# jkulhanek/viewformer

Measured on AMD Instinct MI355X. Metric: novel views/sec (encode->AR transformer->decode), 128px 6-ctx, higher is better.
Workload: dtype bf16

## Files before the change

### include/vf_hip.h

```cpp
#ifndef VF_HIP_H
#define VF_HIP_H

#include <stddef.h>
#include <stdint.h>

#ifdef __cplusplus
extern "C" {
#endif

#define VF_OK 0
#define VF_ERR_BAD_ARG (-1)
#define VF_ERR_UNSUPPORTED (-2)

int vf_abi_version(void);
size_t vf_sizeof_igemm_args(void);
size_t vf_sizeof_pack_desc(void);
const char* vf_build_arch(void);
int vf_build_flags(void);
const char* vf_build_flag_name(int i);
enum { VF_SEL_ATTN_DMA = 0,
       VF_SEL_GEMM_G256 = 1,
       VF_SEL_LN_BWD_TWO_ROWS = 2,
       VF_SEL_ATTN_Q32 = 3,
       VF_SEL_CONV_X3H_K32 = 4,
       VF_SEL_GEMM_TAIL = 5,
       VF_SEL_COUNT = 6 };
int vf_select(int which, int value);
int vf_selected(int which);

enum { VF_MODE_GEMM = 0, VF_MODE_CONV3_S1 = 1, VF_MODE_CONV3_S2PAD = 2, VF_MODE_CONV3_UP2 = 3 };
enum { VF_EPI_NONE = 0, VF_EPI_GELU_ERF = 1,
       VF_EPI_GELU_BWD = 2,
       VF_EPI_GELU_DUAL = 3 };

typedef struct vf_igemm_args {
    const float* x;
    const float* w_packed;
    const float* bias;
    const float* res;
    float* out;
    const float* pro_mean;
    const float* pro_scale;
    const float* pro_beta;
    int32_t pro_swish;
    int32_t pro_rows_per_img;
    int32_t mode;
    int32_t epilogue;
    int32_t M;
    int32_t Cin, Cout;
    int32_t Hin, Win, Hout, Wout;
    int32_t lda, ldc, ldr;
    int32_t batch;
    int64_t stride_x, stride_w, stride_out, stride_res;
    float* gn_part;
    int32_t gn_slots;
    int32_t reserved0;
    void* out_aux;
    float drop_rate;
    uint32_t drop_seed, drop_site;
    int32_t drop_row0;
} vf_igemm_args;

size_t vf_igemm_packed_floats(int K, int N, int taps);
int vf_igemm_pack_f32(const float* src, float* dst, int K, int N, int taps,
                      int64_t sk, int64_t sn, int64_t st, int batch, int64_t src_bstride, void* stream);
int vf_igemm_f32(const vf_igemm_args* args , void* stream);

int vf_conv_in_u8_f32(const uint8_t* img_u8, const float* img_f32, const float* w_oihw, const float* bias,
                      float* out, int n_img, int H, int W, int Cout, void* stream);
size_t vf_conv_in_x3h_packed_elems(int Cout);
int vf_conv_in_x3h_pack(const float* w_oihw, void* dst, int Cout, void* stream);
int vf_conv_in_x3h(const uint8_t* img_u8, const float* img_f32, const void* w_packed, const float* bias, float* out, float* gn_part,
                   int gn_slots, int n_img, int H, int W, int Cout, void* stream);

int vf_conv3_small_cout_f32(const float* x, const float* w_oihw, const float* bias, const float* pro_mean,
                            const float* pro_scale, const float* pro_beta, int pro_swish, float* out, int n_img, int H, int W,
                            int Cin, int Cout, int x_bf16, void* stream);

size_t vf_groupnorm_workspace_bytes(int n_img, int HW, int C);
int vf_groupnorm_stats_f32(const float* x, const float* gamma, int n_img, int HW, int C, int groups, float eps,
                           float* mean_c, float* scale_c, void* ws, void* stream);
int vf_groupnorm_finalize_f32(const float* part, const float* gamma, int n_img, int HW, int C, int groups, int nslots,
                              float eps, float* mean_c, float* scale_c, void* stream);
int vf_groupnorm_apply_f32(const float* x, const float* mean_c, const float* scale_c, const float* beta,
                           float* out, int n_img, int HW, int C, int swish, void* stream);

size_t vf_vq_packed_floats(int D, int Kc);
int vf_vq_pack_codebook_f32(const float* E , float* dst, int D, int Kc, void* stream);
int vf_colsumsq_f32(const float* E , float* e_sq , int D, int Kc, void* stream);
int vf_vq_argmin_f32(const float* z, const float* E_packed, const float* e_sq, int64_t M, int D, int Kc,
                     int64_t* idx, void* stream);
size_t vf_vq_filter_packed_bytes(int D, int Kc);
int vf_vq_filter_pack(const float* E , void* dst, int D, int Kc, void* stream);
int vf_vq_argmin_filtered_f32(const float* z, const void* packed, int64_t M, int D, int Kc, int64_t* idx, uint32_t* stats4,
                              void* stream);
int vf_codebook_gather_f32(const float* E , const int64_t* idx, float* out ,
                           int64_t M, int D, int Kc, void* stream);

int vf_attn_blockcausal_f32(const float* q, const float* k, const float* v, float* out,
                            int B, int H, int T, int L, int ldq, int ldk, int ldv, int ldo,
                            float scale, int skip_masked, int twin_view, void* stream);
int vf_attn_blockcausal_bf16_v2(const void* q, const void* k, const void* v, int in_bf16, void* out, int out_bf16, int B, int H, int T, int L,
                                int ldq, int ldk, int ldv, int ldo, float scale, int skip_masked, int twin_view, void* stream);
int vf_attn_blockcausal_fp8(const void* q, const void* k, const void* v, int in_bf16, void* out, int out_bf16, int B, int H, int T, int L,
                            int ldq, int ldk, int ldv, int ldo, float scale, int skip_masked, int twin_view, void* stream);
int vf_attn_blockcausal_x6(const float* q, const float* k, const float* v, float* out,
                           int B, int H, int T, int L, int ldq, int ldk, int ldv, int ldo,
                           float scale, int skip_masked, int twin_view, void* stream);
int vf_attn_prefix_bf16(const void* q, const void* k, const void* v, const void* kp, const void* vp, int in_bf16, void* out, int out_bf16,
                        int B, int H, int C, int N, int L, int dh, int ldq, int ldk, int ldv, int ldkp, int ldvp, int64_t prefix_stride,
                        int ldo, void* stream);
int vf_attn_prefix_f32eq(const float* q, const float* k, const float* v, const float* kp, const float* vp, float* out,
                         int B, int H, int C, int N, int L, int dh, int ldq, int ldk, int ldv, int ldkp, int ldvp, int64_t prefix_stride,
                         int ldo, void* stream);
int vf_attn_prefix_var_bf16(const void* q, const void* k, const void* v, const void* kp, const void* vp, int in_bf16, void* out, int out_bf16,
                            int B, int H, int C, int N, int L, int dh, int ldq, int ldk, int ldv, int ldkp, int ldvp, int64_t prefix_stride,
                            int ldo, const int32_t* ctx_len, void* stream);
int vf_attn_prefix_var_f32eq(const float* q, const float* k, const float* v, const float* kp, const float* vp, float* out,
                             int B, int H, int C, int N, int L, int dh, int ldq, int ldk, int ldv, int ldkp, int ldvp, int64_t prefix_stride,
                             int ldo, const int32_t* ctx_len, void* stream);
int vf_attn_prefix_fork_bf16(const void* q, const void* k, const void* v, const void* kp, const void* vp, int in_bf16, void* out, int out_bf16,
                             int B, int H, int C, int N, int L, int dh, int ldq, int ldk, int ldv, int ldkp, int ldvp, int64_t prefix_stride,
                             int ldo, const int32_t* ctx_len, const void* kp2, const void* vp2, int C2, int ldkp2, int ldvp2,
                             int64_t prefix_stride2, const int32_t* split, int share, void* stream);
int vf_attn_prefix_fork_f32eq(const float* q, const float* k, const float* v, const float* kp, const float* vp, float* out,
                              int B, int H, int C, int N, int L, int dh, int ldq, int ldk, int ldv, int ldkp, int ldvp, int64_t prefix_stride,
                              int ldo, const int32_t* ctx_len, const float* kp2, const float* vp2, int C2, int ldkp2, int ldvp2,
                              int64_t prefix_stride2, const int32_t* split, int share, void* stream);
int vf_attn_prefix_bwd_f32(const void* q, const void* k, const void* v, const void* kp, const void* vp, int in_bf16, const float* dout,
                           float* dqkv, int B, int H, int C, int N, int L, int dh, int ldq, int ldk, int ldv, int ldkp, int ldvp,
                           int64_t prefix_stride, int lddo, int lddqkv, const int32_t* ctx_len, void* stream);
int vf_kv_append(const void* qkv, void* cache, int elem_bytes, int B, int K, int L, int d, int ld_src, int ld_dst, int64_t cache_stride,
                 int capacity, const int32_t* pos, void* stream);
int vf_kv_append_split(const void* qkv, void* k, void* v, int elem_bytes, int B, int K, int L, int d, int ld_src, int ld_k, int ld_v,
                       int64_t k_stride, int64_t v_stride, int capacity, const int32_t* pos, void* stream);
int vf_kv_pack_e4m3(const void* cache, int elem_bytes, void* kq, void* vq, float* kscale, float* vscale, int B, int C, int H, int L,
                    int ld_src, int64_t cache_stride, int64_t q_view_stride, int64_t q_scene_stride, int64_t s_view_stride,
                    int64_t s_scene_stride, const int32_t* lengths, void* stream);
int vf_kv_append_e4m3(const void* qkv, int elem_bytes, void* kq, void* vq, float* kscale, float* vscale, int B, int K, int H, int L,
                      int ld_src, int64_t q_view_stride, int64_t q_scene_stride, int64_t s_view_stride, int64_t s_scene_stride,
                      int capacity, const int32_t* pos, void* stream);
int vf_attn_prefix_q8_bf16(const void* q, const void* k, const void* v, const void* kq, const void* vq, const float* kscale, const float* vscale,
                           int in_bf16, void* out, int out_bf16, int B, int H, int C, int N, int L, int dh, int ldq, int ldk, int ldv,
                           int64_t q_view_stride, int64_t q_scene_stride, int64_t s_view_stride, int64_t s_scene_stride, int ldo,
                           const int32_t* ctx_len, void* stream);
int vf_attn_spatial_f32(const float* qkv, float* out, int n_img, int HW, int C, int64_t ld, int64_t ldo, float scale, void* stream);
int vf_attn_spatial_x3h(const float* qkv, float* out, int n_img, int HW, int C, int64_t ld, int64_t ldo, float scale, void* stream);
int vf_softmax_rows_f32(float* x, int64_t rows, int n, float scale, void* stream);

int vf_layernorm_f32(const float* x, const float* gamma, const float* beta, float* out,
                     int64_t rows, int d, float eps, void* stream);
int vf_layernorm_bf16out_f32(const float* x, const float* gamma, const float* beta, void* out_bf16, int64_t rows, int d, float eps,
                             void* stream);
int vf_embed_sum_f32(const int32_t* ids, const float* wte, const float* wpe, const float* add,
                     float* out, int64_t BS, int L, int d, int vocab, void* stream);
int vf_dense_small_k_gelu_f32(const float* x, const float* W, const float* b, float* out,
                              int64_t rows, int K, int N, int gelu, void* stream);
int vf_argmax_rows_f32(const float* x, int64_t rows, int n, int ld, int64_t* idx, void* stream);
int vf_lmhead_argmax_bf16(const void* h, int h_bf16, int64_t ldh, const void* w_packed, int64_t M, int K, int N, int64_t* idx,
                          float* max_logit, void* stream);
int vf_lmhead_score_bf16(const void* h, int h_bf16, int64_t ldh, const void* w_packed, int64_t M, int K, int N, const int32_t* target,
                         int64_t* idx, float* max_logit, float* lse, float* target_logit, float* entropy, void* stream);
int vf_logits_score_f32(const float* logits, int64_t rows, int N, int64_t ld, const int32_t* target, int64_t* idx, float* max_logit,
                        float* lse, float* target_logit, float* entropy, void* stream);
int vf_score_views_f32(const float* target_logit, const float* lse, const float* max_logit, const int64_t* idx, const int32_t* target,
                       int64_t views, int L, float* token_log_prob, float* confidence, float* log_likelihood, float* accuracy, void* stream);
int vf_sample_rows_f32(const float* logits, int64_t rows, int N, int64_t ld, float temperature, int top_k, float top_p, uint32_t seed,
                       const int64_t* row_id, int S, int64_t* idx, float* logp, int32_t* kept, float* thr, void* stream);
int vf_sample_views_f32(const float* logp, int64_t views, int L, int S, float* log_likelihood, void* stream);
uint32_t vf_crc32c(const void* data, size_t n, uint32_t crc);
int vf_postprocess_u8(const float* x, uint8_t* out, int64_t n, void* stream);
int vf_resize_u8(const uint8_t* src, uint8_t* dst, int n_img, int Hin, int Win, int Hout, int Wout, int C, int bilinear, void* stream);
size_t vf_image_metrics_workspace_bytes(int n_img, int H, int W, int C);
int vf_image_metrics_u8(const uint8_t* a, const uint8_t* b, int n_img, int H, int W, int C, int64_t* sums, double* ssim, void* workspace,
                        void* stream);
size_t vf_camera_knn_workspace_bytes(int64_t N, int Q, int k);
int vf_camera_knn_f32(const float* db, int64_t N, const float* queries, int Q, int k, float pos_weight, int32_t* idx, float* dist,
                      void* workspace, void* stream);
int vf_codebook_dist_table_f32(const float* E, int D, int K, int64_t ldE, float* table, void* stream);
size_t vf_code_knn_workspace_bytes(int64_t N, int Q, int k);
int vf_code_knn_f32(const int32_t* db, int64_t N, int64_t ld_db, const int32_t* queries, int Q, int64_t ld_q, int t, const float* table,
                    int K, int window, const int32_t* exclude, int k, int32_t* idx, float* dist, void* workspace, void* stream);
int vf_pose_tail_f32(const float* x, int64_t ldx, const float* W, const float* b, float position_multiplier, int64_t views, int L, int K,
                     float* raw, float* tokens, float* cameras, void* stream);

size_t vf_gemm_bf16_packed_elems(int K, int N);
int vf_gemm_bf16_pack(const float* src, void* dst, int K, int N, int64_t sk, int64_t sn, int batch,
                      int64_t src_bstride, void* stream);
typedef struct vf_pack_desc {
    const float* src;
    void* dst;
    int32_t K, N;
    int64_t sk, sn;
} vf_pack_desc;
int vf_gemm_bf16_pack_multi(const vf_pack_desc* descs_device, int n, void* stream);
int vf_gemm_bf16(const vf_igemm_args* args , void* stream);
size_t vf_conv3_bf16_packed_elems(int Cin, int Cout);
int vf_conv3_bf16_pack(const float* w_oihw, void* dst, int Cin, int Cout, void* stream);
int vf_conv3_halo_bf16(const vf_igemm_args* args , void* stream);

int vf_conv3_halo_gn_slots(int Hout, int Wout);
size_t vf_conv3_x6_packed_elems(int Cin, int Cout);
int vf_conv3_x6_pack(const float* w_oihw, void* dst, int Cin, int Cout, void* stream);
int vf_conv3_halo_x6(const vf_igemm_args* args , void* stream);
size_t vf_conv3_x3h_packed_elems(int Cin, int Cout);
int vf_conv3_x3h_pack(const float* w_oihw, void* dst, int Cin, int Cout, void* stream);
int vf_conv3_halo_x3h(const vf_igemm_args* args , void* stream);
size_t vf_gemm_x3h_packed_elems(int K, int N);
int vf_gemm_x3h_pack(const float* src, void* dst, int K, int N, int64_t sk, int64_t sn, void* stream);
int vf_gemm_x3h(const vf_igemm_args* args , void* stream);
size_t vf_gemm_x6_packed_elems(int K, int N);
int vf_gemm_x6_pack(const float* src, void* dst, int K, int N, int64_t sk, int64_t sn, void* stream);
int vf_gemm_x6(const vf_igemm_args* args , void* stream);
int vf_sum_slabs_f32(const float* slabs, int nslabs, int64_t stride, int64_t n, float* dst, int accumulate, void* stream);

int vf_vq_ema_accumulate_f32(const float* z, const int64_t* idx, int64_t M, int D, int Kc, float* counts, float* embed_sum,
                             void* stream);
int vf_vq_ema_update_f32(const float* counts, const float* embed_sum, float* cluster_size_hidden, float* dw_hidden,
                         float* embeddings, int D, int Kc, float decay, float eps, float corr, void* stream);

int vf_gather_transpose_f32(const float* src, float* dst, int n_img, int Hin, int Win, int C, int Hout, int Wout, int stride, int oy,
                            int ox, int64_t ld_dst, void* stream);
size_t vf_conv3_wgrad_x6_rows(int Cin);
int vf_conv3_wgrad_x6(const float* x, const void* dy_packed, float* slabs, int n_img, int Hin, int Win, int Cin, int Hout, int Wout,
                      int Cout, int mode, int splits, void* stream);
int vf_upsample2_bwd_f32(const float* du, float* dx, int n_img, int H, int W, int C, void* stream);
size_t vf_groupnorm_bwd_workspace_bytes(int n_img, int HW, int C, int groups);
int vf_groupnorm_bwd_f32(const float* x, const float* da, const float* mean_c, const float* scale_c, const float* gamma,
                         const float* beta, float* dx, float* chan_sums, int n_img, int HW, int C, int groups, float eps, int swish,
                         int accumulate, void* ws, void* stream);
int vf_softmax_rows_bwd_f32(const float* p, float* dp, int64_t rows, int n, float scale, void* stream);
int vf_l1_loss_partials(int64_t n);
int vf_l1_loss_f32(const float* x, const float* y, float* dy, float* part, int64_t n, float grad_weight, void* stream);

int vf_lpips_scaling_f32(const float* x, float* y, int64_t npix, const float* shift3, const float* scale3, int backward, void* stream);
int vf_relu_f32(float* x, int64_t n, void* stream);
int vf_relu_bwd_f32(float* dy, const float* y, int64_t n, void* stream);
int vf_maxpool2_f32(const float* x, float* y, int n_img, int Hout, int Wout, int C, void* stream);
int vf_maxpool2_bwd_f32(const float* x, const float* dy, float* dx, int n_img, int Hout, int Wout, int C, void* stream);
int vf_lpips_head_blocks(int HW);
int vf_lpips_head_f32(const float* f0, const float* f1, const float* w, float* part, int n_img, int HW, int C, void* stream);
int vf_lpips_head_bwd_f32(const float* f0, const float* f1, const float* w, float* df1, int64_t npix, int C, float gscale,
                          int accumulate, void* stream);

int vf_attn_blockcausal_lse_f32(const float* q, const float* k, const float* v, float* out, float* lse,
                                int B, int H, int T, int L, int ldq, int ldk, int ldv, int ldo,
                                float scale, int skip_masked, int twin_view, float drop_rate, uint32_t drop_seed,
                                uint32_t drop_site, uint32_t drop_plane0, void* stream);
int vf_attn_bwd_prep_f32(const float* dout, const float* out, float* D, int B, int H, int T, int lddo, int ldo, void* stream);
int vf_attn_bwd_f32(const float* q, const float* k, const float* v, const float* dout, const float* lse, const float* D,
                    float* dq, float* dk, float* dv, int B, int H, int T, int L, int ldq, int ldk, int ldv, int lddo,
                    int lddq, int lddk, int lddv, float scale, int twin_view, float drop_rate, uint32_t drop_seed,
                    uint32_t drop_site, uint32_t drop_plane0, void* stream);
int vf_gemm_tn_bf16(const void* x_bf16, int ldx, const void* dy, int dy_is_bf16, int ldy, int M, int K, int N, int splits, float* w_slabs,
                    float* b_slabs, int64_t slab_stride, void* stream);
int vf_attn_blockcausal_bf16_lse(const void* q, const void* k, const void* v, void* out, float* lse, int B, int H, int T, int L,
                                 int ldq, int ldk, int ldv, int ldo, float scale, int twin_view, float drop_rate, uint32_t drop_seed,
                                 uint32_t drop_site, uint32_t drop_plane0, void* stream);
int vf_attn_bwd_prep_bf16(const void* dout, const void* out, float* D, int B, int H, int T, int lddo, int ldo, void* stream);
int vf_attn_bwd_bf16(const void* q, const void* k, const void* v, const void* dout, const float* lse, const float* D, void* dq, void* dk,
                     void* dv, int out_bf16 , int B, int H, int T, int L,
                     int ldq, int ldk, int ldv, int lddo, int lddq, int lddk, int lddv, float scale, int twin_view, float drop_rate,
                     uint32_t drop_seed, uint32_t drop_site, uint32_t drop_plane0, void* stream);
int vf_dropout_add_f32(const float* x, const float* res, float* out, int64_t rows, int cols, int64_t row0, float rate, uint32_t seed, uint32_t site,
                       void* stream);

int vf_transpose_f32(const float* src, float* dst, int rows, int cols, int64_t ld_src, int64_t ld_dst, int batch,
                     int64_t bs_src, int64_t bs_dst, void* stream);
int vf_transpose_bf16_f32(const void* src_bf16, float* dst, int rows, int cols, int64_t ld_src, int64_t ld_dst, int batch,
                          int64_t bs_src, int64_t bs_dst, void* stream);
size_t vf_colsum_workspace_bytes(int N);
int vf_colsum_f32(const float* x, float* out, int64_t M, int N, int64_t ld, int accumulate, void* ws, void* stream);
size_t vf_layernorm_bwd_workspace_bytes(int64_t rows, int d);
int vf_layernorm_bwd_f32(const float* dy, const float* x, const float* gamma, float* dx, float* dgamma, float* dbeta,
                         int64_t rows, int d, float eps, int accumulate, const float* res ,
                         void* dx_bf16 ,
                         float drop_rate, uint32_t drop_seed, uint32_t drop_site, int64_t drop_row0 , void* ws, void* stream);
int vf_gelu_f32(const float* u, float* f, int64_t n, void* stream);
int vf_gelu_bf16out_f32(const float* u, void* f_bf16, int64_t n, void* stream);
int vf_gelu_bwd_f32(const float* u, const float* df, float* du, int64_t n, void* stream);
int vf_gelu_bwd_bf16out_f32(const float* u, const float* df, void* du_bf16, int64_t n, void* stream);
int vf_softmax_mask_f32(float* s, int64_t batch, int T, int L, int mask_spec, float scale, void* stream);
int vf_softmax_mask_bwd_f32(const float* p, float* dp, int64_t batch, int T, int L, int mask_spec, float scale, void* stream);
int vf_softmax_ce_f32(const float* logits, const int32_t* target, const float* row_weight, float* loss, float* dlogits,
                      int64_t rows, int V, float label_smoothing, void* stream);
int vf_pose_mse_f32(const float* raw, const float* gt, const float* w_pos, const float* w_ori, const float* xyz_div, float* pos_loss,
                    float* ori_loss, float* draw, int64_t rows, int L, float position_multiplier, void* stream);
size_t vf_embed_bwd_workspace_bytes(int d, int vocab);
int vf_embed_bwd_f32(const float* dh, const int32_t* ids, float* dwte, float* dwpe, float* dadd, int64_t BS, int L, int d,
                     int vocab, void* workspace, void* stream);
int vf_dense_small_k_bwd_f32(const float* x, const float* dy, float* dW, float* db, int64_t rows, int K, int N, void* stream);
int vf_dense_small_n_f32(const float* x, const float* W, const float* b, float* out, int64_t rows, int K, int N, int64_t ldx, void* stream);
int vf_dense_small_n_wgrad_slabs(int64_t rows);
int vf_dense_small_n_wgrad_f32(const float* x, const float* dy, float* dW, float* ws, int64_t rows, int K, int N, int64_t ldx, int accumulate,
                               void* stream);
int vf_adamw_f32(float* param, const float* grad, float* m, float* v, int64_t n, float lr_decay, float lr_adam, float beta1,
                 float beta2, float eps, void* stream);
int vf_adamw_flat_f32(float* param, const float* grad, float* m, float* v, int64_t n, const int64_t* nodecay_ranges, int nranges,
                      float lr_decay, float lr_adam, float beta1, float beta2, float eps, void* stream);
typedef struct vf_adamw_pack_desc {
    int64_t offset;
    void* dst_kn;
    void* dst_nk;
    int32_t rows, cols;
    int32_t nodecay;
    int32_t reserved;
} vf_adamw_pack_desc;
size_t vf_sizeof_adamw_pack_desc(void);
int vf_adamw_pack_check(const vf_adamw_pack_desc* descs_host, int ndesc, int64_t n);
int vf_adamw_flat_pack_f32(float* param, const float* grad, float* m, float* v, int64_t n, const int64_t* nodecay_ranges, int nranges,
                           float lr_decay, float lr_adam, float beta1, float beta2, float eps, const vf_adamw_pack_desc* descs_device, int ndesc,
                           void* stream);
int vf_add_inplace_f32(float* a, const float* b, int64_t n, void* stream);
int vf_axpby_f32(float a, const float* x, float b, const float* y, float* out, int64_t n, void* stream);
int vf_clip_scratch_floats(void);
int vf_clip_by_norm_f32(float* x, int64_t n, float clip, float* scratch, void* stream);
int vf_clip_grad_norm_f32(float* x, int64_t n, float max_norm, float* scratch, void* stream);

#ifdef __cplusplus
}
#endif
#endif
```

### viewformer_amd/_lib.py

```python
import ctypes
import os
from ctypes import c_int, c_int32, c_int64, c_float, c_void_p, c_size_t, c_char_p, POINTER

HERE = os.path.dirname(os.path.abspath(__file__))
LIB_PATH = os.environ.get('VF_HIP_LIB') or os.path.join(HERE, 'libvf_hip.so')


class VfIgemmArgs(ctypes.Structure):
    _fields_ = [
        ('x', c_void_p), ('w_packed', c_void_p), ('bias', c_void_p), ('res', c_void_p), ('out', c_void_p),
        ('pro_mean', c_void_p), ('pro_scale', c_void_p), ('pro_beta', c_void_p),
        ('pro_swish', c_int32), ('pro_rows_per_img', c_int32), ('mode', c_int32), ('epilogue', c_int32),
        ('M', c_int32), ('Cin', c_int32), ('Cout', c_int32),
        ('Hin', c_int32), ('Win', c_int32), ('Hout', c_int32), ('Wout', c_int32),
        ('lda', c_int32), ('ldc', c_int32), ('ldr', c_int32), ('batch', c_int32),
        ('stride_x', c_int64), ('stride_w', c_int64), ('stride_out', c_int64), ('stride_res', c_int64),
        ('gn_part', c_void_p), ('gn_slots', c_int32), ('reserved0', c_int32),
        ('out_aux', c_void_p),
        ('drop_rate', c_float), ('drop_seed', ctypes.c_uint32), ('drop_site', ctypes.c_uint32), ('drop_row0', c_int32),
    ]


SEL_ATTN_DMA, SEL_GEMM_G256, SEL_LN_BWD_TWO_ROWS, SEL_ATTN_Q32 = 0, 1, 2, 3
SEL_CONV_X3H_K32 = 4
SEL_GEMM_TAIL = 5
_ENV_SELECT = {'VF_ATTN_DMA': SEL_ATTN_DMA, 'VF_GEMM_G256': SEL_GEMM_G256, 'VF_LN_BWD_TWO_ROWS': SEL_LN_BWD_TWO_ROWS, 'VF_ATTN_Q32': SEL_ATTN_Q32,
               'VF_CONV_X3H_K32': SEL_CONV_X3H_K32, 'VF_GEMM_TAIL': SEL_GEMM_TAIL}

ADAMW_PACK_DESC_BYTES = 40
PACK_DESC_BYTES = 40
P = c_void_p
EXPORTS = {
    'vf_abi_version': (c_int, []),
    'vf_sizeof_igemm_args': (c_size_t, []),
    'vf_sizeof_pack_desc': (c_size_t, []),
    'vf_build_arch': (c_char_p, []),
    'vf_build_flags': (c_int, []),
    'vf_build_flag_name': (c_char_p, [c_int]),
    'vf_select': (c_int, [c_int, c_int]),
    'vf_selected': (c_int, [c_int]),
    'vf_igemm_packed_floats': (c_size_t, [c_int, c_int, c_int]),
    'vf_igemm_pack_f32': (c_int, [P, P, c_int, c_int, c_int, c_int64, c_int64, c_int64, c_int, c_int64, P]),
    'vf_igemm_f32': (c_int, [POINTER(VfIgemmArgs), P]),
    'vf_conv_in_u8_f32': (c_int, [P, P, P, P, P, c_int, c_int, c_int, c_int, P]),
    'vf_conv_in_x3h_packed_elems': (c_size_t, [c_int]),
    'vf_conv_in_x3h_pack': (c_int, [P, P, c_int, P]),
    'vf_conv_in_x3h': (c_int, [P, P, P, P, P, P, c_int, c_int, c_int, c_int, c_int, P]),
    'vf_crc32c': (ctypes.c_uint32, [P, c_size_t, ctypes.c_uint32]),
    'vf_conv3_small_cout_f32': (c_int, [P, P, P, P, P, P, c_int, P, c_int, c_int, c_int, c_int, c_int, c_int, P]),
    'vf_groupnorm_workspace_bytes': (c_size_t, [c_int, c_int, c_int]),
    'vf_groupnorm_stats_f32': (c_int, [P, P, c_int, c_int, c_int, c_int, c_float, P, P, P, P]),
    'vf_groupnorm_finalize_f32': (c_int, [P, P, c_int, c_int, c_int, c_int, c_int, c_float, P, P, P]),
    'vf_conv3_halo_gn_slots': (c_int, [c_int, c_int]),
    'vf_groupnorm_apply_f32': (c_int, [P, P, P, P, P, c_int, c_int, c_int, c_int, P]),
    'vf_vq_packed_floats': (c_size_t, [c_int, c_int]),
    'vf_vq_pack_codebook_f32': (c_int, [P, P, c_int, c_int, P]),
    'vf_colsumsq_f32': (c_int, [P, P, c_int, c_int, P]),
    'vf_vq_argmin_f32': (c_int, [P, P, P, c_int64, c_int, c_int, P, P]),
    'vf_vq_filter_packed_bytes': (c_size_t, [c_int, c_int]),
    'vf_vq_filter_pack': (c_int, [P, P, c_int, c_int, P]),
    'vf_vq_argmin_filtered_f32': (c_int, [P, P, c_int64, c_int, c_int, P, P, P]),
    'vf_gather_transpose_f32': (c_int, [P, P, c_int, c_int, c_int, c_int, c_int, c_int, c_int, c_int, c_int, c_int64, P]),
    'vf_upsample2_bwd_f32': (c_int, [P, P, c_int, c_int, c_int, c_int, P]),
    'vf_groupnorm_bwd_workspace_bytes': (c_size_t, [c_int, c_int, c_int, c_int]),
    'vf_groupnorm_bwd_f32': (c_int, [P, P, P, P, P, P, P, P, c_int, c_int, c_int, c_int, c_float, c_int, c_int, P, P]),
    'vf_softmax_rows_bwd_f32': (c_int, [P, P, c_int64, c_int, c_float, P]),
    'vf_l1_loss_partials': (c_int, [c_int64]),
    'vf_l1_loss_f32': (c_int, [P, P, P, P, c_int64, c_float, P]),
    'vf_conv3_wgrad_x6_rows': (c_size_t, [c_int]),
    'vf_conv3_wgrad_x6': (c_int, [P, P, P, c_int, c_int, c_int, c_int, c_int, c_int, c_int, c_int, c_int, P]),
    'vf_lpips_scaling_f32': (c_int, [P, P, c_int64, P, P, c_int, P]),
    'vf_relu_f32': (c_int, [P, c_int64, P]),
    'vf_relu_bwd_f32': (c_int, [P, P, c_int64, P]),
    'vf_maxpool2_f32': (c_int, [P, P, c_int, c_int, c_int, c_int, P]),
    'vf_maxpool2_bwd_f32': (c_int, [P, P, P, c_int, c_int, c_int, c_int, P]),
    'vf_lpips_head_blocks': (c_int, [c_int]),
    'vf_lpips_head_f32': (c_int, [P, P, P, P, c_int, c_int, c_int, P]),
    'vf_lpips_head_bwd_f32': (c_int, [P, P, P, P, c_int64, c_int, c_float, c_int, P]),
    'vf_vq_ema_accumulate_f32': (c_int, [P, P, c_int64, c_int, c_int, P, P, P]),
    'vf_vq_ema_update_f32': (c_int, [P, P, P, P, P, c_int, c_int, c_float, c_float, c_float, P]),
    'vf_codebook_gather_f32': (c_int, [P, P, P, c_int64, c_int, c_int, P]),
    'vf_attn_blockcausal_f32': (c_int, [P, P, P, P, c_int, c_int, c_int, c_int, c_int, c_int, c_int, c_int,
                                        c_float, c_int, c_int, P]),
    'vf_attn_blockcausal_bf16_v2': (c_int, [P, P, P, c_int, P, c_int] + [c_int] * 8 + [c_float, c_int, c_int, P]),
    'vf_attn_blockcausal_fp8': (c_int, [P, P, P, c_int, P, c_int] + [c_int] * 8 + [c_float, c_int, c_int, P]),
    'vf_attn_blockcausal_x6': (c_int, [P, P, P, P, c_int, c_int, c_int, c_int, c_int, c_int, c_int, c_int,
                                       c_float, c_int, c_int, P]),
    'vf_attn_prefix_bf16': (c_int, [P, P, P, P, P, c_int, P, c_int] + [c_int] * 11 + [c_int64, c_int, P]),
    'vf_attn_prefix_f32eq': (c_int, [P, P, P, P, P, P] + [c_int] * 11 + [c_int64, c_int, P]),
    'vf_attn_prefix_var_bf16': (c_int, [P, P, P, P, P, c_int, P, c_int] + [c_int] * 11 + [c_int64, c_int, P, P]),
    'vf_attn_prefix_var_f32eq': (c_int, [P, P, P, P, P, P] + [c_int] * 11 + [c_int64, c_int, P, P]),
    'vf_attn_prefix_fork_bf16': (c_int, [P, P, P, P, P, c_int, P, c_int] + [c_int] * 11 + [c_int64, c_int, P,
                                         P, P, c_int, c_int, c_int, c_int64, P, c_int, P]),
    'vf_attn_prefix_fork_f32eq': (c_int, [P, P, P, P, P, P] + [c_int] * 11 + [c_int64, c_int, P, P, P, c_int, c_int, c_int, c_int64, P, c_int, P]),
    'vf_attn_prefix_bwd_f32': (c_int, [P, P, P, P, P, c_int, P, P] + [c_int] * 11 + [c_int64, c_int, c_int, P, P]),
    'vf_kv_append': (c_int, [P, P, c_int, c_int, c_int, c_int, c_int, c_int, c_int, c_int64, c_int, P, P]),
    'vf_kv_append_split': (c_int, [P, P, P] + [c_int] * 8 + [c_int64, c_int64, c_int, P, P]),
    'vf_kv_pack_e4m3': (c_int, [P, c_int, P, P, P, P] + [c_int] * 5 + [c_int64] * 5 + [P, P]),
    'vf_kv_append_e4m3': (c_int, [P, c_int, P, P, P, P] + [c_int] * 5 + [c_int64] * 4 + [c_int, P, P]),
    'vf_attn_prefix_q8_bf16': (c_int, [P] * 7 + [c_int, P, c_int] + [c_int] * 9 + [c_int64] * 4 + [c_int, P, P]),
    'vf_attn_blockcausal_lse_f32': (c_int, [P, P, P, P, P, c_int, c_int, c_int, c_int, c_int, c_int, c_int, c_int,
                                            c_float, c_int, c_int, c_float, ctypes.c_uint32, ctypes.c_uint32, ctypes.c_uint32, P]),
    'vf_dropout_add_f32': (c_int, [P, P, P, c_int64, c_int, c_int64, c_float, ctypes.c_uint32, ctypes.c_uint32, P]),
    'vf_attn_bwd_prep_f32': (c_int, [P, P, P, c_int, c_int, c_int, c_int, c_int, P]),
    'vf_attn_bwd_f32': (c_int, [P, P, P, P, P, P, P, P, P, c_int, c_int, c_int, c_int, c_int, c_int, c_int, c_int, c_int,
                                c_int, c_int, c_float, c_int, c_float, ctypes.c_uint32, ctypes.c_uint32, ctypes.c_uint32, P]),
    'vf_gemm_tn_bf16': (c_int, [P, c_int, P, c_int, c_int, c_int, c_int, c_int, c_int, P, P, c_int64, P]),
    'vf_attn_blockcausal_bf16_lse': (c_int, [P, P, P, P, P, c_int, c_int, c_int, c_int, c_int, c_int, c_int, c_int, c_float, c_int,
                                             c_float, ctypes.c_uint32, ctypes.c_uint32, ctypes.c_uint32, P]),
    'vf_attn_bwd_prep_bf16': (c_int, [P, P, P, c_int, c_int, c_int, c_int, c_int, P]),
    'vf_attn_bwd_bf16': (c_int, [P, P, P, P, P, P, P, P, P, c_int, c_int, c_int, c_int, c_int, c_int, c_int, c_int, c_int, c_int, c_int, c_int,
                                 c_float, c_int, c_float, ctypes.c_uint32, ctypes.c_uint32, ctypes.c_uint32, P]),
    'vf_attn_spatial_f32': (c_int, [P, P, c_int, c_int, c_int, c_int64, c_int64, c_float, P]),
    'vf_attn_spatial_x3h': (c_int, [P, P, c_int, c_int, c_int, c_int64, c_int64, c_float, P]),
    'vf_softmax_rows_f32': (c_int, [P, c_int64, c_int, c_float, P]),
    'vf_layernorm_f32': (c_int, [P, P, P, P, c_int64, c_int, c_float, P]),
    'vf_layernorm_bf16out_f32': (c_int, [P, P, P, P, c_int64, c_int, c_float, P]),
    'vf_embed_sum_f32': (c_int, [P, P, P, P, P, c_int64, c_int, c_int, c_int, P]),
    'vf_dense_small_k_gelu_f32': (c_int, [P, P, P, P, c_int64, c_int, c_int, c_int, P]),
    'vf_lmhead_argmax_bf16': (c_int, [P, c_int, c_int64, P, c_int64, c_int, c_int, P, P, P]),
    'vf_lmhead_score_bf16': (c_int, [P, c_int, c_int64, P, c_int64, c_int, c_int, P, P, P, P, P, P, P]),
    'vf_logits_score_f32': (c_int, [P, c_int64, c_int, c_int64, P, P, P, P, P, P, P]),
    'vf_score_views_f32': (c_int, [P, P, P, P, P, c_int64, c_int, P, P, P, P, P]),
    'vf_sample_rows_f32': (c_int, [P, c_int64, c_int, c_int64, c_float, c_int, c_float, ctypes.c_uint32, P, c_int, P, P, P, P, P]),
    'vf_sample_views_f32': (c_int, [P, c_int64, c_int, c_int, P, P]),
    'vf_argmax_rows_f32': (c_int, [P, c_int64, c_int, c_int, P, P]),
    'vf_postprocess_u8': (c_int, [P, P, c_int64, P]),
    'vf_resize_u8': (c_int, [P, P, c_int, c_int, c_int, c_int, c_int, c_int, c_int, P]),
    'vf_image_metrics_workspace_bytes': (c_size_t, [c_int, c_int, c_int, c_int]),
    'vf_image_metrics_u8': (c_int, [P, P, c_int, c_int, c_int, c_int, P, P, P, P]),
    'vf_camera_knn_workspace_bytes': (c_size_t, [c_int64, c_int, c_int]),
    'vf_camera_knn_f32': (c_int, [P, c_int64, P, c_int, c_int, c_float, P, P, P, P]),
    'vf_codebook_dist_table_f32': (c_int, [P, c_int, c_int, c_int64, P, P]),
    'vf_code_knn_workspace_bytes': (c_size_t, [c_int64, c_int, c_int]),
    'vf_code_knn_f32': (c_int, [P, c_int64, c_int64, P, c_int, c_int64, c_int, P, c_int, c_int, P, c_int, P, P, P, P]),
    'vf_pose_tail_f32': (c_int, [P, c_int64, P, P, c_float, c_int64, c_int, c_int, P, P, P, P]),
    'vf_gemm_bf16_packed_elems': (c_size_t, [c_int, c_int]),
    'vf_gemm_bf16_pack': (c_int, [P, P, c_int, c_int, c_int64, c_int64, c_int, c_int64, P]),
    'vf_gemm_bf16_pack_multi': (c_int, [P, c_int, P]),
    'vf_gemm_bf16': (c_int, [POINTER(VfIgemmArgs), P]),
    'vf_conv3_bf16_packed_elems': (c_size_t, [c_int, c_int]),
    'vf_conv3_bf16_pack': (c_int, [P, P, c_int, c_int, P]),
    'vf_conv3_halo_bf16': (c_int, [POINTER(VfIgemmArgs), P]),
    'vf_conv3_x6_packed_elems': (c_size_t, [c_int, c_int]),
    'vf_conv3_x6_pack': (c_int, [P, P, c_int, c_int, P]),
    'vf_conv3_halo_x6': (c_int, [POINTER(VfIgemmArgs), P]),
    'vf_conv3_x3h_packed_elems': (c_size_t, [c_int, c_int]),
    'vf_conv3_x3h_pack': (c_int, [P, P, c_int, c_int, P]),
    'vf_conv3_halo_x3h': (c_int, [POINTER(VfIgemmArgs), P]),
    'vf_gemm_x3h_packed_elems': (c_size_t, [c_int, c_int]),
    'vf_gemm_x3h_pack': (c_int, [P, P, c_int, c_int, c_int64, c_int64, P]),
    'vf_gemm_x3h': (c_int, [POINTER(VfIgemmArgs), P]),
    'vf_gemm_x6_packed_elems': (c_size_t, [c_int, c_int]),
    'vf_gemm_x6_pack': (c_int, [P, P, c_int, c_int, c_int64, c_int64, P]),
    'vf_gemm_x6': (c_int, [POINTER(VfIgemmArgs), P]),
    'vf_sum_slabs_f32': (c_int, [P, c_int, c_int64, c_int64, P, c_int, P]),
    'vf_transpose_f32': (c_int, [P, P, c_int, c_int, c_int64, c_int64, c_int, c_int64, c_int64, P]),
    'vf_transpose_bf16_f32': (c_int, [P, P, c_int, c_int, c_int64, c_int64, c_int, c_int64, c_int64, P]),
    'vf_colsum_workspace_bytes': (c_size_t, [c_int]),
    'vf_colsum_f32': (c_int, [P, P, c_int64, c_int, c_int64, c_int, P, P]),
    'vf_layernorm_bwd_workspace_bytes': (c_size_t, [c_int64, c_int]),
    'vf_layernorm_bwd_f32': (c_int, [P, P, P, P, P, P, c_int64, c_int, c_float, c_int, P, P, c_float, ctypes.c_uint32, ctypes.c_uint32, c_int64, P, P]),
    'vf_gelu_f32': (c_int, [P, P, c_int64, P]),
    'vf_gelu_bf16out_f32': (c_int, [P, P, c_int64, P]),
    'vf_gelu_bwd_bf16out_f32': (c_int, [P, P, P, c_int64, P]),
    'vf_gelu_bwd_f32': (c_int, [P, P, P, c_int64, P]),
    'vf_softmax_mask_f32': (c_int, [P, c_int64, c_int, c_int, c_int, c_float, P]),
    'vf_softmax_mask_bwd_f32': (c_int, [P, P, c_int64, c_int, c_int, c_int, c_float, P]),
    'vf_softmax_ce_f32': (c_int, [P, P, P, P, P, c_int64, c_int, c_float, P]),
    'vf_pose_mse_f32': (c_int, [P, P, P, P, P, P, P, P, c_int64, c_int, c_float, P]),
    'vf_embed_bwd_workspace_bytes': (c_size_t, [c_int, c_int]),
    'vf_embed_bwd_f32': (c_int, [P, P, P, P, P, c_int64, c_int, c_int, c_int, P, P]),
    'vf_dense_small_k_bwd_f32': (c_int, [P, P, P, P, c_int64, c_int, c_int, P]),
    'vf_dense_small_n_f32': (c_int, [P, P, P, P, c_int64, c_int, c_int, c_int64, P]),
    'vf_dense_small_n_wgrad_slabs': (c_int, [c_int64]),
    'vf_dense_small_n_wgrad_f32': (c_int, [P, P, P, P, c_int64, c_int, c_int, c_int64, c_int, P]),
    'vf_adamw_f32': (c_int, [P, P, P, P, c_int64, c_float, c_float, c_float, c_float, c_float, P]),
    'vf_adamw_flat_f32': (c_int, [P, P, P, P, c_int64, P, c_int, c_float, c_float, c_float, c_float, c_float, P]),
    'vf_sizeof_adamw_pack_desc': (c_size_t, []),
    'vf_adamw_pack_check': (c_int, [P, c_int, c_int64]),
    'vf_adamw_flat_pack_f32': (c_int, [P, P, P, P, c_int64, P, c_int, c_float, c_float, c_float, c_float, c_float, P, c_int, P]),
    'vf_axpby_f32': (c_int, [c_float, P, c_float, P, P, c_int64, P]),
    'vf_add_inplace_f32': (c_int, [P, P, c_int64, P]),
    'vf_clip_scratch_floats': (c_int, []),
    'vf_clip_by_norm_f32': (c_int, [P, c_int64, c_float, P, P]),
    'vf_clip_grad_norm_f32': (c_int, [P, c_int64, c_float, P, P]),
}

_lib = None


class VfError(RuntimeError):
    pass


def _bind(path):
    lib = ctypes.CDLL(path)
    for name, (res, args) in EXPORTS.items():
        fn = getattr(lib, name)
        fn.restype = res
        fn.argtypes = args
    return lib


def load_variant(path):
    return _bind(os.path.abspath(path))


class use:

    def __init__(self, handle):
        self.handle = handle

    def __enter__(self):
        global _lib
        load()
        self.prev, _lib = _lib, self.handle
        return self.handle

    def __exit__(self, *exc):
        global _lib
        _lib = self.prev
        return False


def load():
    global _lib
    if _lib is not None:
        return _lib
    if not os.path.exists(LIB_PATH):
        raise VfError(f'{LIB_PATH} not found — run `python -m viewformer_amd.build` (hipcc --offload-arch=gfx950). '
                      'There is no CPU/PyTorch fallback for the hot path.')
    lib = _bind(LIB_PATH)
    if int(lib.vf_sizeof_igemm_args()) != ctypes.sizeof(VfIgemmArgs):
        raise VfError(f'vf_igemm_args is {int(lib.vf_sizeof_igemm_args())} bytes in {LIB_PATH} and {ctypes.sizeof(VfIgemmArgs)} in '
                      'viewformer_amd/_lib.py: rebuild the library or update the mirror')
    if int(lib.vf_sizeof_pack_desc()) != PACK_DESC_BYTES:
        raise VfError(f'vf_pack_desc is {int(lib.vf_sizeof_pack_desc())} bytes in {LIB_PATH}, {PACK_DESC_BYTES} expected')
    if int(lib.vf_sizeof_adamw_pack_desc()) != ADAMW_PACK_DESC_BYTES:
        raise VfError(f'vf_adamw_pack_desc is {int(lib.vf_sizeof_adamw_pack_desc())} bytes in {LIB_PATH}, {ADAMW_PACK_DESC_BYTES} expected')
    for env, which in _ENV_SELECT.items():
        if os.environ.get(env) in ('0', '1'):
            lib.vf_select(which, int(os.environ[env]))
    _lib = lib
    return lib


def select(which, value):
    prev = load().vf_select(int(which), 1 if value else 0)
    if prev < 0:
        raise VfError(f'vf_select({which}, {value}): bad argument')
    return prev


def check(status: int, what: str):
    if status == 0:
        return
    if status < 0:
        msg = {-1: 'bad argument', -2: 'unsupported shape'}.get(status, 'error')
        raise VfError(f'{what}: {msg} ({status})')
    raise VfError(f'{what}: HIP error {status}')
```

### viewformer_amd/csrc/conv3_halo_x3h.hip

```cpp
#include <type_traits>
#include "halo_common.h"

namespace {

typedef _Float16 f16x8 __attribute__((ext_vector_type(8)));
typedef _Float16 f16x4 __attribute__((ext_vector_type(4)));

typedef unsigned u32x4_t __attribute__((ext_vector_type(4)));
__device__ __forceinline__ f16x8 wbuf_load(__amdgpu_buffer_rsrc_t r, unsigned voff, unsigned soff) {
    return __builtin_bit_cast(f16x8, __builtin_amdgcn_raw_buffer_load_b128(r, voff, soff, 0));
}

constexpr int CK = 32;
constexpr int P_LDB = 144;
constexpr int TH = 8, TW = 16;
constexpr int BN = 128;
constexpr int PLANE_BYTES = 2 * BN * 16;
constexpr int KS_BYTES = 2 * PLANE_BYTES;
constexpr int TAP_BYTES = 2 * KS_BYTES;
constexpr int TAIL_BYTES = 16;

template <bool UP2, bool PAIR = false>
struct Geo {
    static constexpr int PH = UP2 ? (TH / 2 + 2) : (TH + 2);
    static constexpr int PW = PAIR ? 20 : (UP2 ? (TW / 2 + 2) : (TW + 2));
    static constexpr int NPIX = PH * PW;
    static constexpr int SLOTS = (NPIX * 8 + 255) / 256;
    static constexpr int BUF = (NPIX + 1) * P_LDB;
};

__device__ __forceinline__ void split2(float x, _Float16& h, _Float16& l) {
    h = (_Float16)x;
    l = (_Float16)((x - (float)h) * 2048.f);
}

template <bool UP2, bool PRO, bool SWISH, bool PAIR = false>
__global__ __launch_bounds__(256, 2) void conv3_halo_x3h_kernel(vf_igemm_args p) {
    using G = Geo<UP2, PAIR>;
    extern __shared__ __attribute__((aligned(16))) unsigned char smem_h[];

    const int tid = threadIdx.x;
    const int lane = tid & 63;
    const int wave = __builtin_amdgcn_readfirstlane(tid >> 6);
    constexpr int MI = 4, NJ = 1;
    const int wave_m = 0, wave_n = wave;
    const int half = lane >> 5, l31 = lane & 31;

    const int nb = p.Cout / BN;
    const int tilesX = p.Wout / TW, tilesY = p.Hout / TH;
    int bid = (int)vf_xcd_bid();
    const int nblk = bid % nb; bid /= nb;
    int tx = 0, ty = 0, img;
    if (PAIR) { img = bid * 2; }
    else { tx = bid % tilesX; bid /= tilesX; ty = bid % tilesY; img = bid / tilesY; }
    const int n_img_total = p.M / (p.Hout * p.Wout);
    const int img1 = PAIR ? min(img + 1, n_img_total - 1) : img;
    const int pair_pix = (img1 - img) * p.Hin * p.Win;
    const int y0 = ty * TH, x0 = tx * TW;
    const int sy0 = UP2 ? (y0 / 2 - 1) : (y0 - 1);
    const int sx0 = UP2 ? (x0 / 2 - 1) : (x0 - 1);

    const float* __restrict__ X = p.x + (size_t)img * p.Hin * p.Win * p.Cin;
    const int nchunks = p.Cin / CK;
    const int last_stage = nchunks * 9 - 1;

    const int c4 = tid & 7;
    int s_off[G::SLOTS];
    unsigned ok_mask = 0, sel_mask = 0;
    const int lds0 = (tid >> 3) * P_LDB + c4 * 8;
    int lds_last = 0;
#pragma unroll
    for (int q = 0; q < G::SLOTS; ++q) {
        const int pix = (tid >> 3) + 32 * q;
        const int pixc = pix < G::NPIX ? pix : G::NPIX;
        const int pr = pixc / G::PW, pc0 = pixc - pr * G::PW;
        const int sel = PAIR ? (pc0 >= 10) : 0;
        const int pc = pc0 - 10 * sel;
        sel_mask |= (unsigned)sel << q;
        const int sy = sy0 + pr, sx = sx0 + pc;
        const bool ok = pix < G::NPIX && sy >= 0 && sy < p.Hin && sx >= 0 && sx < p.Win;
        ok_mask |= (unsigned)ok << q;
        s_off[q] = ok ? (sel * pair_pix + sy * p.Win + sx) * p.Cin + c4 * 4 : c4 * 4;
        if (q == G::SLOTS - 1) lds_last = pixc * P_LDB + c4 * 8;
    }

    f32x4 preg[G::SLOTS];
    f32x4 pmean, pscale, pbeta, pmean1, pscale1;
    const __amdgpu_buffer_rsrc_t x_rs = __builtin_amdgcn_make_buffer_rsrc(const_cast<float*>(X), 0, 0x7fffffff, 0x00020000);
    auto patch_load = [&](int chunk) {
#pragma unroll
        for (int q = 0; q < G::SLOTS; ++q)
            preg[q] = __builtin_bit_cast(f32x4, __builtin_amdgcn_raw_buffer_load_b128(x_rs, (unsigned)s_off[q] * 4u, (unsigned)(chunk * CK * 4), 0));
        if (PRO) {
            pmean = *reinterpret_cast<const f32x4*>(p.pro_mean + (size_t)img * p.Cin + chunk * CK + c4 * 4);
            pscale = *reinterpret_cast<const f32x4*>(p.pro_scale + (size_t)img * p.Cin + chunk * CK + c4 * 4);
            pbeta = *reinterpret_cast<const f32x4*>(p.pro_beta + chunk * CK + c4 * 4);
            if (PAIR) {
                pmean1 = *reinterpret_cast<const f32x4*>(p.pro_mean + (size_t)img1 * p.Cin + chunk * CK + c4 * 4);
                pscale1 = *reinterpret_cast<const f32x4*>(p.pro_scale + (size_t)img1 * p.Cin + chunk * CK + c4 * 4);
            }
        }
    };
    auto patch_store_slot = [&](int buf, int q) {
        unsigned char* dst = smem_h + buf * G::BUF + (q == G::SLOTS - 1 ? lds_last : lds0 + q * 32 * P_LDB);
        f16x4 oh, ol;
#pragma unroll
        for (int e = 0; e < 4; ++e) {
            float t = preg[q][e];
            if (PRO) {
                const float mu = (PAIR && ((sel_mask >> q) & 1u)) ? pmean1[e] : pmean[e];
                const float sc = (PAIR && ((sel_mask >> q) & 1u)) ? pscale1[e] : pscale[e];
                t = (t - mu) * sc + pbeta[e];
                if (SWISH) t = vf_swish_1ulp(t);
            }
            _Float16 h, l;
            split2(((ok_mask >> q) & 1u) ? t : 0.f, h, l);
            oh[e] = h; ol[e] = l;
        }
        *reinterpret_cast<f16x4*>(dst) = oh;
        *reinterpret_cast<f16x4*>(dst + 64) = ol;
    };

    const int trow = vf_perm_row(l31), tpx = vf_perm_px(l31);
    int a_base[MI], a_r[MI];
#pragma unroll
    for (int mi = 0; mi < MI; ++mi) {
        const int a0 = wave_m * 4 + mi * 2 + trow;
        a_r[mi] = a0;
        const int tcol = PAIR ? (tpx >> 3) * 10 + (tpx & 7) : tpx;
        a_base[mi] = (a0 * G::PW + tcol) * P_LDB + half * 16;
    }

    const unsigned char* __restrict__ Wb = reinterpret_cast<const unsigned char*>(p.w_packed) + (size_t)nblk * TAP_BYTES;
    const size_t tap_stride = (size_t)nb * TAP_BYTES;
    const int b_lane = (half * BN + wave_n * (32 * NJ) + l31) * 16;
    constexpr int BD = 2, RING = BD + 1;
    static_assert(18 % RING == 0, "ring indices must repeat per chunk");
    f16x8 bring[RING][2][NJ];
    f16x8 aring[2][MI][2];
    const int last_g = nchunks * 18 - 1;
    const __amdgpu_buffer_rsrc_t w_rs = __builtin_amdgcn_make_buffer_rsrc(const_cast<unsigned char*>(Wb), 0, 0x7fffffff, 0x00020000);
    auto b_load = [&](f16x8 (&dst)[2][NJ], int g) {
        g = min(g, last_g);
        const unsigned soff = (unsigned)((size_t)(g >> 1) * tap_stride + (g & 1) * KS_BYTES);
#pragma unroll
        for (int pl = 0; pl < 2; ++pl)
#pragma unroll
            for (int j = 0; j < NJ; ++j) dst[pl][j] = wbuf_load(w_rs, (unsigned)(b_lane + pl * PLANE_BYTES + j * 32 * 16), soff);
    };
    auto a_load = [&](f16x8 (&dst)[MI][2], const unsigned char* patch, int s) {
        const int tap = s >> 1, ks = s & 1;
        const int dy = tap / 3, dx = tap % 3;
#pragma unroll
        for (int mi = 0; mi < MI; ++mi) {
            int aoff;
            if (UP2) {
                const int pr = (a_r[mi] + dy + 1) >> 1, pc = (tpx + dx + 1) >> 1;
                aoff = (pr * G::PW + pc) * P_LDB + half * 16;
            } else {
                aoff = a_base[mi] + (dy * G::PW + dx) * P_LDB;
            }
#pragma unroll
            for (int pl = 0; pl < 2; ++pl) dst[mi][pl] = *reinterpret_cast<const f16x8*>(patch + aoff + pl * 64 + ks * 32);
        }
    };

    f32x16 acc[MI][NJ], accx[MI][NJ];
#pragma unroll
    for (int i = 0; i < MI; ++i)
#pragma unroll
        for (int j = 0; j < NJ; ++j)
#pragma unroll
            for (int r = 0; r < 16; ++r) { acc[i][j][r] = 0.f; accx[i][j][r] = 0.f; }

    patch_load(0);
#pragma unroll
    for (int g = 0; g < BD; ++g) b_load(bring[g], g);
#pragma unroll
    for (int q = 0; q < G::SLOTS; ++q) patch_store_slot(0, q);
    __syncthreads();

    for (int chunk = 0; chunk < nchunks; ++chunk) {
        const unsigned char* patch = smem_h + (chunk & 1) * G::BUF;
        b_load(bring[BD % RING], chunk * 18 + BD);
        const bool more = UP2 || PAIR || chunk + 1 < nchunks;
        if (more) patch_load(min(chunk + 1, nchunks - 1));
        a_load(aring[0], patch, 0);
#pragma unroll
        for (int s = 0; s < 18; ++s) {
            if (s > 0) b_load(bring[(s + BD) % RING], chunk * 18 + s + BD);
            if (s + 1 < 18) a_load(aring[(s + 1) & 1], patch, s + 1);
#pragma unroll
            for (int t = 0; t < 3; ++t) {
#pragma unroll
                for (int mi = 0; mi < MI; ++mi)
#pragma unroll
                    for (int j = 0; j < NJ; ++j) {
                        if (t == 0) accx[mi][j] = __builtin_amdgcn_mfma_f32_32x32x16_f16(aring[s & 1][mi][1], bring[s % RING][0][j], accx[mi][j], 0, 0, 0);
                        else if (t == 1) accx[mi][j] = __builtin_amdgcn_mfma_f32_32x32x16_f16(aring[s & 1][mi][0], bring[s % RING][1][j], accx[mi][j], 0, 0, 0);
                        else acc[mi][j] = __builtin_amdgcn_mfma_f32_32x32x16_f16(aring[s & 1][mi][0], bring[s % RING][0][j], acc[mi][j], 0, 0, 0);
                    }
            }
            __builtin_amdgcn_sched_barrier(0);
            if ((s & 1) && (s >> 1) < G::SLOTS && more) patch_store_slot((chunk + 1) & 1, s >> 1);
        }
        __syncthreads();
    }

    const float inv_s = *reinterpret_cast<const float*>(reinterpret_cast<const unsigned char*>(p.w_packed) + (size_t)nchunks * 9 * nb * TAP_BYTES);
#pragma unroll
    for (int i = 0; i < MI; ++i)
#pragma unroll
        for (int j = 0; j < NJ; ++j)
#pragma unroll
            for (int r = 0; r < 16; ++r) acc[i][j][r] = __builtin_fmaf(accx[i][j][r], 4.8828125e-4f, acc[i][j][r]) * inv_s;
    vf_halo_epilogue_t<PAIR, MI, NJ>(p, acc, img, img1, y0, x0, PAIR ? 0 : (ty * tilesX + tx) * 2, nblk, wave_m, wave_n, half, l31);
}


constexpr int S2_PH = 2 * TH + 1, S2_PW = 2 * TW + 1;
constexpr int S2_NPIX = S2_PH * S2_PW;
constexpr int S2_LDB = 80;
constexpr int S2_SLOTS = (S2_NPIX * 4 + 255) / 256;
constexpr int S2_BUF = (S2_NPIX + 1) * S2_LDB;

template <bool P8>
__global__ __launch_bounds__(256, 2) void conv3_s2_x3h_kernel(vf_igemm_args p) {
    extern __shared__ __attribute__((aligned(16))) unsigned char smem_h[];
    constexpr int PW = P8 ? 34 : S2_PW;
    constexpr int NPIX = S2_PH * PW;
    constexpr int SLOTS = (NPIX * 4 + 255) / 256;
    const int tid = threadIdx.x;
    const int lane = tid & 63;
    const int wave = __builtin_amdgcn_readfirstlane(tid >> 6);
    constexpr int MI = 4, NJ = 1;
    const int wave_m = 0, wave_n = wave;
    const int half = lane >> 5, l31 = lane & 31;

    const int nb = p.Cout / BN;
    const int tilesX = P8 ? 1 : p.Wout / TW, tilesY = P8 ? 1 : p.Hout / TH;
    int bid = (int)vf_xcd_bid();
    const int nblk = bid % nb; bid /= nb;
    const int tx = bid % tilesX; bid /= tilesX;
    const int ty = bid % tilesY;
    const int img = P8 ? (bid / tilesY) * 2 : bid / tilesY;
    const int n_img_total = p.M / (p.Hout * p.Wout);
    const int img1 = P8 ? min(img + 1, n_img_total - 1) : img;
    const int pair_pix = (img1 - img) * p.Hin * p.Win;
    const int y0 = ty * TH, x0 = tx * TW;
    const float* __restrict__ X = p.x + (size_t)img * p.Hin * p.Win * p.Cin;
    const int nchunks = p.Cin / 16;

    const int c4 = tid & 3;
    int s_off[SLOTS], s_lds[SLOTS];
    bool s_ok[SLOTS];
#pragma unroll
    for (int q = 0; q < SLOTS; ++q) {
        const int pix = (tid >> 2) + 64 * q;
        const int pixc = pix < NPIX ? pix : 0;
        const int pr = pixc / PW, pc0 = pixc - pr * PW;
        const int sel = P8 ? (pc0 >= 17) : 0;
        const int pc = pc0 - 17 * sel;
        const int sy = 2 * y0 + pr, sx = 2 * x0 + pc;
        const bool ok = pix < NPIX && sy < p.Hin && sx < p.Win;
        s_ok[q] = ok;
        s_off[q] = ok ? (sel * pair_pix + sy * p.Win + sx) * p.Cin + c4 * 4 : c4 * 4;
        int slot;
        if (P8) slot = pr * PW + ((pc & 1) ? 18 + sel * 8 + (pc >> 1) : sel * 9 + (pc >> 1));
        else slot = pr * PW + (pc & 1) * (TW + 1) + (pc >> 1);
        s_lds[q] = (pix < NPIX ? slot : NPIX) * S2_LDB + c4 * 8;
    }
    f32x4 preg[SLOTS];
    auto patch_load = [&](int chunk) {
#pragma unroll
        for (int q = 0; q < SLOTS; ++q) preg[q] = *reinterpret_cast<const f32x4*>(X + chunk * 16 + s_off[q]);
    };
    auto patch_park = [&]() {
#pragma unroll
        for (int q = 0; q < SLOTS; ++q) {
            f16x4 oh, ol;
#pragma unroll
            for (int e = 0; e < 4; ++e) {
                _Float16 h, l;
                split2(s_ok[q] ? preg[q][e] : 0.f, h, l);
                oh[e] = h; ol[e] = l;
            }
            unsigned char* dst = smem_h + s_lds[q];
            *reinterpret_cast<f16x4*>(dst) = oh;
            *reinterpret_cast<f16x4*>(dst + 32) = ol;
        }
    };

    const int trow = vf_perm_row(l31), tpx = vf_perm_px(l31);
    int a_base[MI], a_base_o[MI];
#pragma unroll
    for (int mi = 0; mi < MI; ++mi) {
        const int row2 = 2 * (wave_m * 4 + mi * 2 + trow) * PW;
        if (P8) {
            a_base[mi] = (row2 + (tpx >> 3) * 9 + (tpx & 7)) * S2_LDB + half * 16;
            a_base_o[mi] = (row2 + 18 + (tpx >> 3) * 8 + (tpx & 7)) * S2_LDB + half * 16;
        } else {
            a_base[mi] = (row2 + tpx) * S2_LDB + half * 16;
            a_base_o[mi] = a_base[mi] + (TW + 1) * S2_LDB;
        }
    }

    const unsigned char* __restrict__ Wb = reinterpret_cast<const unsigned char*>(p.w_packed) + (size_t)nblk * TAP_BYTES;
    const size_t tap_stride = (size_t)nb * TAP_BYTES;
    const int b_lane = (half * BN + wave_n * (32 * NJ) + l31) * 16;
    const int last_g = nchunks * 9 - 1;
    constexpr int S2_BR = 3;
    f16x8 bring[S2_BR][2][NJ];
    f16x8 aring[2][MI][2];
    auto b_load = [&](f16x8 (&dst)[2][NJ], int g) {
        g = min(g, last_g);
        const int c = g / 9, tap = g - c * 9;
        const unsigned char* src = Wb + (size_t)((c >> 1) * 9 + tap) * tap_stride + (c & 1) * KS_BYTES + b_lane;
#pragma unroll
        for (int pl = 0; pl < 2; ++pl)
#pragma unroll
            for (int j = 0; j < NJ; ++j) dst[pl][j] = *reinterpret_cast<const f16x8*>(src + pl * PLANE_BYTES + j * 32 * 16);
    };
    auto a_load = [&](f16x8 (&dst)[MI][2], int tap) {
        const int dy = tap / 3, dx = tap % 3;
        const int off = (dy * PW + (dx >> 1)) * S2_LDB;
#pragma unroll
        for (int mi = 0; mi < MI; ++mi)
#pragma unroll
            for (int pl = 0; pl < 2; ++pl) dst[mi][pl] = *reinterpret_cast<const f16x8*>(smem_h + ((dx & 1) ? a_base_o[mi] : a_base[mi]) + off + pl * 32);
    };

    f32x16 acc[MI][NJ], accx[MI][NJ];
#pragma unroll
    for (int i = 0; i < MI; ++i)
#pragma unroll
        for (int j = 0; j < NJ; ++j)
#pragma unroll
            for (int r = 0; r < 16; ++r) { acc[i][j][r] = 0.f; accx[i][j][r] = 0.f; }

    patch_load(0);
    b_load(bring[0], 0);
    if (S2_BR > 2) b_load(bring[1], 1);
    for (int chunk = 0; chunk < nchunks; ++chunk) {
        __syncthreads();
        patch_park();
        b_load(bring[(S2_BR - 1) % S2_BR], chunk * 9 + S2_BR - 1);
        if (chunk + 1 < nchunks) patch_load(min(chunk + 1, nchunks - 1));
        __syncthreads();
        a_load(aring[0], 0);
#pragma unroll
        for (int t = 0; t < 9; ++t) {
            if (t > 0) b_load(bring[(t + S2_BR - 1) % S2_BR], chunk * 9 + t + S2_BR - 1);
            if (t + 1 < 9) a_load(aring[(t + 1) & 1], t + 1);
#pragma unroll
            for (int mi = 0; mi < MI; ++mi)
#pragma unroll
                for (int j = 0; j < NJ; ++j) accx[mi][j] = __builtin_amdgcn_mfma_f32_32x32x16_f16(aring[t & 1][mi][1], bring[t % S2_BR][0][j], accx[mi][j], 0, 0, 0);
#pragma unroll
            for (int mi = 0; mi < MI; ++mi)
#pragma unroll
                for (int j = 0; j < NJ; ++j) accx[mi][j] = __builtin_amdgcn_mfma_f32_32x32x16_f16(aring[t & 1][mi][0], bring[t % S2_BR][1][j], accx[mi][j], 0, 0, 0);
#pragma unroll
            for (int mi = 0; mi < MI; ++mi)
#pragma unroll
                for (int j = 0; j < NJ; ++j) acc[mi][j] = __builtin_amdgcn_mfma_f32_32x32x16_f16(aring[t & 1][mi][0], bring[t % S2_BR][0][j], acc[mi][j], 0, 0, 0);
            __builtin_amdgcn_sched_barrier(0);
        }
    }
    const float inv_s = *reinterpret_cast<const float*>(reinterpret_cast<const unsigned char*>(p.w_packed) + (size_t)(p.Cin / CK) * 9 * nb * TAP_BYTES);
#pragma unroll
    for (int i = 0; i < MI; ++i)
// ... 143 lines not shown
    for (int q = 0; q < G::SLOTS; ++q) patch_store_slot(0, q);
    __syncthreads();

    auto chunk_body = [&](int chunk, auto parity) {
        constexpr int P0 = decltype(parity)::value;
        const unsigned char* patch = smem_h + P0 * G::BUF;
        const bool more = chunk + 1 < nchunks;
        b_load(bring[(P0 + 1) & 1], chunk * 9 + 1);
        unsigned pad[G::SLOTS];
#pragma unroll
        for (int q = 0; q < G::SLOTS; ++q) pad[q] = __builtin_amdgcn_raw_buffer_load_b32(w_rs, (unsigned)(q * 256), 0u, 0);
        if (more) patch_load(chunk + 1);
#pragma unroll
        for (int i = 0; i < AR - 1; ++i) a_load(aring[i], patch, i);
#pragma unroll
        for (int t = 0; t < 9; ++t) {
            if (t > 0) b_load(bring[(P0 + t + 1) & 1], chunk * 9 + t + 1);
            if (t == 2) {
#pragma unroll
                for (int q = 0; q < G::SLOTS; ++q) asm volatile("" :: "v"(pad[q]));
            }
            const f16x8 (&B)[4] = bring[(P0 + t) & 1];
#pragma unroll
            for (int rt = 0; rt < RT; ++rt) {
                const int step = t * 8 + rt;
                if (step + AR - 1 < 72) a_load(aring[(step + AR - 1) % AR], patch, step + AR - 1);
                const f16x8 ah = aring[step % AR][0], al = aring[step % AR][1];
                accx[rt][0] = __builtin_amdgcn_mfma_f32_16x16x32_f16(al, B[0], accx[rt][0], 0, 0, 0);
                accx[rt][1] = __builtin_amdgcn_mfma_f32_16x16x32_f16(al, B[1], accx[rt][1], 0, 0, 0);
                acc[rt][0] = __builtin_amdgcn_mfma_f32_16x16x32_f16(ah, B[0], acc[rt][0], 0, 0, 0);
                acc[rt][1] = __builtin_amdgcn_mfma_f32_16x16x32_f16(ah, B[1], acc[rt][1], 0, 0, 0);
                accx[rt][0] = __builtin_amdgcn_mfma_f32_16x16x32_f16(ah, B[2], accx[rt][0], 0, 0, 0);
                accx[rt][1] = __builtin_amdgcn_mfma_f32_16x16x32_f16(ah, B[3], accx[rt][1], 0, 0, 0);
                __builtin_amdgcn_sched_barrier(0);
            }
            if (t >= 1 && t <= G::SLOTS && more) {
                if (t == 1) asm volatile("s_waitcnt vmcnt(8)" ::: "memory");
                patch_store_slot((P0 + 1) & 1, t - 1);
            }
        }
        __syncthreads();
    };
    for (int chunk = 0; chunk < nchunks; chunk += 2) {
        chunk_body(chunk, std::integral_constant<int, 0>{});
        chunk_body(chunk + 1, std::integral_constant<int, 1>{});
    }

    const float inv_s = *reinterpret_cast<const float*>(reinterpret_cast<const unsigned char*>(p.w_packed) + (size_t)nchunks * 9 * nb * TAP_BYTES);
    const __amdgpu_buffer_rsrc_t o_rs = __builtin_amdgcn_make_buffer_rsrc(p.out + (size_t)img * p.Hout * p.Wout * p.ldc, 0, 0x7fffffff, 0x00020000);
    const __amdgpu_buffer_rsrc_t r_rs = __builtin_amdgcn_make_buffer_rsrc(const_cast<float*>(p.res ? p.res + (size_t)img * p.Hout * p.Wout * p.ldr : p.out), 0, 0x7fffffff, 0x00020000);
    const bool Res = p.res != nullptr;
    const bool stats = p.gn_part != nullptr;
    const int cg = p.Cout >> 5;
    const int tile_slot = (ty * tilesX + tx) * 2;
    const int pbase = lg == 0 ? 0 : lg == 1 ? 1 : lg == 2 ? 9 : 8;
    auto spix = [&](int rt, int r) { return (y0 + rt) * p.Wout + x0 + 2 * r; };
#pragma unroll
    for (int rt = 0; rt < RT; ++rt)
#pragma unroll
        for (int ct = 0; ct < CT; ++ct)
#pragma unroll
            for (int r = 0; r < 4; ++r) acc[rt][ct][r] = __builtin_fmaf(accx[rt][ct][r], 4.8828125e-4f, acc[rt][ct][r]) * inv_s;
    __builtin_amdgcn_sched_barrier(0);
    float rr[CT][RT][4];
    if (Res) {
#pragma unroll
        for (int ct = 0; ct < CT; ++ct) {
            const int n = nblk * BN + wave * 32 + ct * 16 + lm;
            const unsigned rv = (unsigned)(pbase * p.ldr + n) * 4u;
#pragma unroll
            for (int rt = 0; rt < RT; ++rt)
#pragma unroll
                for (int r = 0; r < 4; ++r)
                    rr[ct][rt][r] = __builtin_bit_cast(float, __builtin_amdgcn_raw_buffer_load_b32(r_rs, rv, (unsigned)(spix(rt, r) * p.ldr) * 4u, 0));
        }
    }
#pragma unroll
    for (int ct = 0; ct < CT; ++ct) {
        const int n = nblk * BN + wave * 32 + ct * 16 + lm;
        const float bias = p.bias ? p.bias[n] : 0.f;
        const unsigned ov = (unsigned)(pbase * p.ldc + n) * 4u;
#pragma unroll
        for (int sl = 0; sl < 2; ++sl) {
            float s32 = 0.f, q32 = 0.f;
#pragma unroll
            for (int k = 0; k < 4; ++k) {
                const int rt = sl * 4 + k;
#pragma unroll
                for (int r = 0; r < 4; ++r) {
                    float v = acc[rt][ct][r] + bias;
                    if (Res) v += rr[ct][rt][r];
                    __builtin_amdgcn_raw_buffer_store_b32(__builtin_bit_cast(unsigned, v), o_rs, ov, (unsigned)(spix(rt, r) * p.ldc) * 4u, 0);
                    s32 += v;
                    q32 = __builtin_fmaf(v, v, q32);
                }
            }
            if (stats) {
                vf_gn_acc_t s = (vf_gn_acc_t)s32, q = (vf_gn_acc_t)q32;
                for (int o = 1; o < cg; o <<= 1) { s += __shfl_xor(s, o, 64); q += __shfl_xor(q, o, 64); }
                s += __shfl_xor(s, 16, 64); q += __shfl_xor(q, 16, 64);
                s += __shfl_xor(s, 32, 64); q += __shfl_xor(q, 32, 64);
                if (lg == 0 && (lm & (cg - 1)) == 0) {
                    float* dst = p.gn_part + ((((size_t)img * p.gn_slots) + tile_slot + sl) * 32 + n / cg) * 2;
                    dst[0] = (float)s;
                    dst[1] = (float)q;
                }
            }
        }
    }
}

__global__ void absmax_kernel(const float* __restrict__ w, long long n, unsigned* __restrict__ out) {
    float m = 0.f;
    for (long long i = blockIdx.x * (long long)blockDim.x + threadIdx.x; i < n; i += (long long)gridDim.x * blockDim.x) m = fmaxf(m, fabsf(w[i]));
    vf_block_max_atomic(m, out);
}

__global__ void pack_conv_x3h_kernel(const float* __restrict__ w, _Float16* __restrict__ dst, int Cin, int Cout, int nb, int nchunks,
                                     unsigned char* __restrict__ tail) {
    const float amax = __uint_as_float(*reinterpret_cast<const unsigned*>(tail + 4));
    const int ex = amax > 0.f ? ilogbf(amax) : 13;
    const float S = ldexpf(1.f, 13 - ex);
    if (blockIdx.x == 0 && threadIdx.x == 0) *reinterpret_cast<float*>(tail) = ldexpf(1.f, ex - 13);
    const long long total = (long long)nchunks * 9 * nb * CK * BN;
    for (long long idx = blockIdx.x * (long long)blockDim.x + threadIdx.x; idx < total; idx += (long long)gridDim.x * blockDim.x) {
        const int e = (int)(idx & 7);
        long long t = idx >> 3;
        const int nl = (int)(t % BN); t /= BN;
        const int half = (int)(t & 1);
        const int ks = (int)((t >> 1) & 1);
        t >>= 2;
        const int nblk = (int)(t % nb); t /= nb;
        const int tap = (int)(t % 9);
        const int chunk = (int)(t / 9);
        const int c = chunk * CK + ks * 16 + half * 8 + e;
        const int n = nblk * BN + nl;
        float v = 0.f;
        if (c < Cin && n < Cout) v = w[((size_t)n * Cin + c) * 9 + tap] * S;
        _Float16 h, l;
        split2(v, h, l);
        const size_t base = ((((size_t)(chunk * 9 + tap) * nb + nblk) * 2 + ks) * 2) * (2 * BN * 8) + ((size_t)half * BN + nl) * 8 + e;
        dst[base] = h;
        dst[base + 2 * BN * 8] = l;
    }
}

template <bool UP2, bool PRO, bool SWISH, bool PAIR>
int launch_halo(const vf_igemm_args& a, hipStream_t stream) {
    using G = Geo<UP2, PAIR>;
    const size_t smem = (size_t)2 * G::BUF;
    const int n_img = a.M / (a.Hout * a.Wout);
    const long long blocks = PAIR ? (long long)((n_img + 1) / 2) * (a.Cout / BN)
                                  : (long long)n_img * (a.Hout / TH) * (a.Wout / TW) * (a.Cout / BN);
    hipLaunchKernelGGL((conv3_halo_x3h_kernel<UP2, PRO, SWISH, PAIR>), dim3((unsigned)blocks), dim3(256), smem, stream, a);
    return vf_last_status();
}

static inline size_t vf_x3h16_lds_bytes(int pro_cin) { return (size_t)2 * Geo<false, false>::BUF + Geo<false, false>::SLOTS * 4096 - 1024 + (size_t)3 * pro_cin * 4; }

template <bool PRO, bool SWISH>
int launch_halo16(const vf_igemm_args& a, hipStream_t stream) {
    using G = Geo<false, false>;
    const int n_img = a.M / (a.Hout * a.Wout);
    const long long blocks = (long long)n_img * (a.Hout / TH) * (a.Wout / TW) * (a.Cout / BN);
    const size_t smem = vf_x3h16_lds_bytes(PRO ? a.Cin : 0);
    static unsigned long long attr_devs = 0;
    if (vf_attr_needed(&attr_devs)) {
        const hipError_t e = hipFuncSetAttribute(reinterpret_cast<const void*>(conv3_halo_x3h16_kernel<PRO, SWISH>), hipFuncAttributeMaxDynamicSharedMemorySize, 80 * 1024);
        if (e != hipSuccess) return (int)e;
        vf_attr_done(&attr_devs);
    }
    hipLaunchKernelGGL((conv3_halo_x3h16_kernel<PRO, SWISH>), dim3((unsigned)blocks), dim3(256), smem, stream, a);
    return vf_last_status();
}

template <bool UP2, bool PAIR>
int dispatch_pro(const vf_igemm_args& a, hipStream_t s) {
    if (!UP2 && !PAIR && (a.Cin / CK) % 2 == 0 && (!a.gn_part || a.Cout / 32 <= 16) && vf_x3h16_lds_bytes(a.pro_mean ? a.Cin : 0) <= 80 * 1024 &&
        vf_selected(VF_SEL_CONV_X3H_K32)) {
        if (!a.pro_mean) return launch_halo16<false, false>(a, s);
        return a.pro_swish ? launch_halo16<true, true>(a, s) : launch_halo16<true, false>(a, s);
    }
    if (!a.pro_mean) return launch_halo<UP2, false, false, PAIR>(a, s);
    return a.pro_swish ? launch_halo<UP2, true, true, PAIR>(a, s) : launch_halo<UP2, true, false, PAIR>(a, s);
}

}

extern "C" {

size_t vf_conv3_x3h_packed_elems(int Cin, int Cout) {
    if (Cin <= 0 || Cout <= 0) return 0;
    return (size_t)((Cin + CK - 1) / CK) * 9 * ((Cout + BN - 1) / BN) * CK * BN * 2 + TAIL_BYTES / 2;
}

int vf_conv3_x3h_pack(const float* w_oihw, void* dst, int Cin, int Cout, void* stream) {
    if (!w_oihw || !dst || Cin <= 0 || Cout <= 0) return VF_ERR_BAD_ARG;
    const int nb = (Cout + BN - 1) / BN, nchunks = (Cin + CK - 1) / CK;
    const long long total = (long long)nchunks * 9 * nb * CK * BN;
    unsigned char* tail = reinterpret_cast<unsigned char*>(dst) + (size_t)total * 2 * sizeof(_Float16);
    hipStream_t s = (hipStream_t)stream;
    if (hipMemsetAsync(tail, 0, TAIL_BYTES, s) != hipSuccess) return vf_last_status();
    const long long nw = (long long)Cout * Cin * 9;
    hipLaunchKernelGGL(absmax_kernel, dim3((unsigned)((nw + 2047) / 2048 > 128 ? 128 : (nw + 2047) / 2048)), dim3(256), 0, s, w_oihw, nw,
                       reinterpret_cast<unsigned*>(tail + 4));
    const int blocks = (int)((total + 255) / 256 > 4096 ? 4096 : (total + 255) / 256);
    hipLaunchKernelGGL(pack_conv_x3h_kernel, dim3(blocks), dim3(256), 0, s, w_oihw, (_Float16*)dst, Cin, Cout, nb, nchunks, tail);
    return vf_last_status();
}

int vf_conv3_halo_x3h(const vf_igemm_args* args, void* stream) {
    if (!args) return VF_ERR_BAD_ARG;
    const vf_igemm_args& a = *args;
    if (!a.x || !a.w_packed || !a.out || a.M <= 0) return VF_ERR_BAD_ARG;
    if (a.drop_rate != 0.f || a.out_aux) return VF_ERR_UNSUPPORTED;
    if (a.mode == VF_MODE_CONV3_S2PAD) {
        const bool p8 = a.Hout == 8 && a.Wout == 8;
        if (a.Cout % BN != 0 || a.Cin % CK != 0 || (!p8 && (a.Hout % TH != 0 || a.Wout % TW != 0)) || a.pro_mean) return VF_ERR_UNSUPPORTED;
        if (a.Hin != a.Hout * 2 || a.Win != a.Wout * 2 || a.M % (a.Hout * a.Wout) != 0) return VF_ERR_BAD_ARG;
        if (a.batch > 1 || a.epilogue != VF_EPI_NONE || a.ldc < a.Cout || (a.res && a.ldr < a.Cout)) return VF_ERR_BAD_ARG;
        if ((long long)a.Hin * a.Win * a.Cin >= (1ll << 31)) return VF_ERR_UNSUPPORTED;
        if (int st = vf_halo_gn_check(a)) return st;
        if (p8) {
            const long long blocks = (long long)((a.M / 64 + 1) / 2) * (a.Cout / BN);
            hipLaunchKernelGGL(conv3_s2_x3h_kernel<true>, dim3((unsigned)blocks), dim3(256), (size_t)(S2_PH * 34 + 1) * S2_LDB, (hipStream_t)stream, a);
            return vf_last_status();
        }
        const long long blocks = (long long)(a.M / (a.Hout * a.Wout)) * (a.Hout / TH) * (a.Wout / TW) * (a.Cout / BN);
        hipLaunchKernelGGL(conv3_s2_x3h_kernel<false>, dim3((unsigned)blocks), dim3(256), (size_t)S2_BUF, (hipStream_t)stream, a);
        return vf_last_status();
    }
    if (a.mode != VF_MODE_CONV3_S1 && a.mode != VF_MODE_CONV3_UP2) return VF_ERR_UNSUPPORTED;
    const bool pair = a.mode == VF_MODE_CONV3_S1 && a.Hout == 8 && a.Wout == 8;
    if (a.Cout % BN != 0 || a.Cin % CK != 0 || (!pair && (a.Hout % TH != 0 || a.Wout % TW != 0))) return VF_ERR_UNSUPPORTED;
    if (a.Hin <= 0 || a.Win <= 0 || a.M % (a.Hout * a.Wout) != 0) return VF_ERR_BAD_ARG;
    if (a.mode == VF_MODE_CONV3_S1 && (a.Hout != a.Hin || a.Wout != a.Win)) return VF_ERR_BAD_ARG;
    if (a.mode == VF_MODE_CONV3_UP2 && (a.Hout != a.Hin * 2 || a.Wout != a.Win * 2)) return VF_ERR_BAD_ARG;
    if (a.batch > 1 || a.epilogue != VF_EPI_NONE || a.ldc < a.Cout || (a.res && a.ldr < a.Cout)) return VF_ERR_BAD_ARG;
    if ((a.pro_mean || a.pro_scale || a.pro_beta) && !(a.pro_mean && a.pro_scale && a.pro_beta)) return VF_ERR_BAD_ARG;
    if ((long long)a.Hin * a.Win * a.Cin >= (1ll << 31)) return VF_ERR_UNSUPPORTED;
    if (int st = vf_halo_gn_check(a)) return st;
    hipStream_t s = (hipStream_t)stream;
    if (pair) return dispatch_pro<false, true>(a, s);
    return (a.mode == VF_MODE_CONV3_UP2) ? dispatch_pro<true, false>(a, s) : dispatch_pro<false, false>(a, s);
}

}
```

### viewformer_amd/csrc/gemm_bf16.hip

```cpp
#include "vf_common.h"
#include "epilogue.h"
#include "../../include/vf_hip.h"

namespace {

typedef __bf16 bf16x8 __attribute__((ext_vector_type(8)));
typedef __bf16 bf16x4 __attribute__((ext_vector_type(4)));

constexpr int CK = 64;
constexpr int BM = 128, BN = 128;
constexpr int A_LDB = 144;
constexpr int A_BYTES = BM * A_LDB;
constexpr int B_BYTES = CK * BN * 2;

__global__ __launch_bounds__(256, 2) void gemm_bf16_kernel(vf_igemm_args p) {
    extern __shared__ __attribute__((aligned(16))) unsigned char smem_b[];
    unsigned char* As = smem_b;
    unsigned char* Bs = smem_b + 2 * A_BYTES;

    const int tid = threadIdx.x;
    const int lane = tid & 63;
    const int wave = __builtin_amdgcn_readfirstlane(tid >> 6);
    const int wave_m = wave >> 1, wave_n = wave & 1;
    const int half = lane >> 5, l31 = lane & 31;
// ... 213 lines not shown
        typedef __bf16 bf16x2_t __attribute__((ext_vector_type(2)));
        const bool gelu16 = p.epilogue == VF_EPI_GELU_ERF;
        const bool gbwd = p.epilogue == VF_EPI_GELU_BWD;
        __bf16* __restrict__ O = reinterpret_cast<__bf16*>(p.out);
        const bool pairs = (p.ldc & 1) == 0 && (p.Cout & 1) == 0;
        const int odd = l31 & 1;
#pragma unroll
        for (int j = 0; j < NJ; ++j) {
            const int n = nblk * BN + wave_n * (32 * NJ) + j * 32 + l31;
            const float bias = (n < p.Cout && p.bias) ? p.bias[n] : 0.f;
#pragma unroll
            for (int i = 0; i < MI; ++i) {
                const int m0 = mtile * BM + wave_m * 64 + i * 32 + 4 * half;
                float t[16];
                if (gbwd) {
                    float uu[16];
#pragma unroll
                    for (int r = 0; r < 16; ++r) {
                        const int m = m0 + (r & 3) + 8 * (r >> 2);
                        uu[r] = p.res[(size_t)(m < p.M ? m : 0) * p.ldr + (n < p.Cout ? n : 0)];
                    }
#pragma unroll
                    for (int r = 0; r < 16; ++r) t[r] = __fmul_rn(__fadd_rn(acc[i][j][r], bias), vf_gelu_grad_fast(uu[r]));
                } else {
#pragma unroll
                    for (int r = 0; r < 16; ++r) {
                        t[r] = acc[i][j][r] + bias;
                        if (gelu16) t[r] = vf_gelu_erf_fast(t[r]);
                    }
                }
                if (pairs) {
#pragma unroll
                    for (int r = 0; r < 16; r += 2) {
                        const float give = odd ? t[r] : t[r + 1];
                        const float got = vf_lane_xor1(give);
                        const int m = m0 + ((r + odd) & 3) + 8 * ((r + odd) >> 2);
                        bf16x2_t v;
                        v[0] = (__bf16)(odd ? got : t[r]);
                        v[1] = (__bf16)(odd ? t[r + 1] : got);
                        const int n0 = n - odd;
                        if (m < p.M && n0 < p.Cout) *reinterpret_cast<bf16x2_t*>(O + (size_t)m * p.ldc + n0) = v;
                    }
                } else {
#pragma unroll
                    for (int r = 0; r < 16; ++r) {
                        const int m = m0 + (r & 3) + 8 * (r >> 2);
                        if (m < p.M && n < p.Cout) O[(size_t)m * p.ldc + n] = (__bf16)t[r];
                    }
                }
            }
        }
        return;
    }
    float* __restrict__ Out = p.out;
    const float* __restrict__ Res = p.res;
    const bool full = (mtile * BM + BM <= p.M) && (nblk * BN + BN <= p.Cout);
    const long long ldc = p.ldc, ldr = p.ldr;
    const bool gelu = p.epilogue == VF_EPI_GELU_ERF;
#pragma unroll
    for (int j = 0; j < NJ; ++j) {
        const int n = nblk * BN + wave_n * (32 * NJ) + j * 32 + l31;
        const bool nok = n < p.Cout;
        const float bias = (nok && p.bias) ? p.bias[n] : 0.f;
#pragma unroll
        for (int i = 0; i < MI; ++i) {
            const int m0 = mtile * BM + wave_m * 64 + i * 32 + 4 * half;
            const int nn = nok ? n : 0;
            float* o = Out + (size_t)(m0 < p.M ? m0 : 0) * ldc + nn;
            const float* rs = Res ? Res + (size_t)(m0 < p.M ? m0 : 0) * ldr + nn : nullptr;
            const int rows_left = nok ? p.M - m0 : 0;
            if (full) {
                auto oo = [&](int r) { return (long long)((r & 3) + 8 * (r >> 2)) * ldc; };
                auto ro = [&](int r) { return (long long)((r & 3) + 8 * (r >> 2)) * ldr; };
                if (gelu) {
                    if (Res) vf_store_tile<2, true>(acc[i][j], bias, o, rs, oo, ro);
                    else vf_store_tile<2, false>(acc[i][j], bias, o, rs, oo, ro);
                } else {
                    if (Res) vf_store_tile<0, true>(acc[i][j], bias, o, rs, oo, ro);
                    else vf_store_tile<0, false>(acc[i][j], bias, o, rs, oo, ro);
                }
            } else if (gelu) {
                if (Res) vf_store_tile_ragged<2, true>(acc[i][j], bias, o, rs, ldc, ldr, rows_left);
                else vf_store_tile_ragged<2, false>(acc[i][j], bias, o, rs, ldc, ldr, rows_left);
            } else {
                if (Res) vf_store_tile_ragged<0, true>(acc[i][j], bias, o, rs, ldc, ldr, rows_left);
                else vf_store_tile_ragged<0, false>(acc[i][j], bias, o, rs, ldc, ldr, rows_left);
            }
        }
    }
}

__global__ void pack_bf16_kernel(const float* __restrict__ src, __bf16* __restrict__ dst, int K, int N, long long sk,
                                 long long sn, int nb, int nchunks, long long src_bstride, long long dst_bstride) {
    const long long total = (long long)nchunks * nb * CK * BN;
    const int bz = blockIdx.y;
    for (long long idx = blockIdx.x * (long long)blockDim.x + threadIdx.x; idx < total; idx += (long long)gridDim.x * blockDim.x) {
        const int e = (int)(idx & 7);
        long long t = idx >> 3;
        const int nl = (int)(t % BN); t /= BN;
        const int half = (int)(t & 1);
        const int ks = (int)((t >> 1) & 3);
        t >>= 3;
        const int nblk = (int)(t % nb);
        const int chunk = (int)(t / nb);
        const int k = chunk * CK + ks * 16 + half * 8 + e;
        const int n = nblk * BN + nl;
        float v = 0.f;
        if (k < K && n < N) v = src[(size_t)bz * src_bstride + k * sk + n * sn];
        dst[(size_t)bz * dst_bstride + idx] = (__bf16)v;
    }
}

__global__ void pack_bf16_multi_kernel(const vf_pack_desc* __restrict__ descs) {
    const vf_pack_desc d = descs[blockIdx.y];
    const int nb = (d.N + BN - 1) / BN, nchunks = (d.K + CK - 1) / CK;
    const long long groups = (long long)nchunks * nb * (CK * BN / 8);
    __bf16* __restrict__ dst = reinterpret_cast<__bf16*>(d.dst);
    typedef __bf16 bf16x8_t __attribute__((ext_vector_type(8)));
    for (long long gi = blockIdx.x * (long long)blockDim.x + threadIdx.x; gi < groups; gi += (long long)gridDim.x * blockDim.x) {
        long long t = gi;
        const int nl = (int)(t % BN); t /= BN;
        const int half = (int)(t & 1);
        const int ks = (int)((t >> 1) & 3);
        t >>= 3;
        const int nblk = (int)(t % nb);
        const int chunk = (int)(t / nb);
        const int k0 = chunk * CK + ks * 16 + half * 8;
        const int n = nblk * BN + nl;
        float v[8];
#pragma unroll
        for (int e = 0; e < 8; ++e) v[e] = 0.f;
        if (n < d.N) {
            const float* sp = d.src + (long long)k0 * d.sk + (long long)n * d.sn;
            if (d.sk == 1 && k0 + 8 <= d.K && ((reinterpret_cast<uintptr_t>(sp) & 15) == 0)) {
                const f32x4 a = *reinterpret_cast<const f32x4*>(sp), b = *reinterpret_cast<const f32x4*>(sp + 4);
#pragma unroll
                for (int e = 0; e < 4; ++e) { v[e] = a[e]; v[4 + e] = b[e]; }
            } else {
#pragma unroll
                for (int e = 0; e < 8; ++e)
                    if (k0 + e < d.K) v[e] = sp[(long long)e * d.sk];
            }
        }
        bf16x8_t o;
#pragma unroll
        for (int e = 0; e < 8; ++e) o[e] = (__bf16)v[e];
        *reinterpret_cast<bf16x8_t*>(dst + gi * 8) = o;
    }
}

}

int vf_gemm_bf16_g256_launch(const vf_igemm_args& a, hipStream_t stream);

extern "C" {

size_t vf_gemm_bf16_packed_elems(int K, int N) {
    if (K <= 0 || N <= 0) return 0;
    return (size_t)((K + CK - 1) / CK) * ((N + BN - 1) / BN) * CK * BN;
}

int vf_gemm_bf16_pack(const float* src, void* dst, int K, int N, int64_t sk, int64_t sn, int batch, int64_t src_bstride,
                      void* stream) {
    if (!src || !dst || K <= 0 || N <= 0 || batch < 1) return VF_ERR_BAD_ARG;
    const int nb = (N + BN - 1) / BN, nchunks = (K + CK - 1) / CK;
    const long long total = (long long)nchunks * nb * CK * BN;
    const int blocks = (int)((total + 255) / 256 > 4096 ? 4096 : (total + 255) / 256);
    hipLaunchKernelGGL(pack_bf16_kernel, dim3(blocks, batch), dim3(256), 0, (hipStream_t)stream, src, (__bf16*)dst, K, N,
                       (long long)sk, (long long)sn, nb, nchunks, (long long)src_bstride, total);
    return vf_last_status();
}

int vf_gemm_bf16_pack_multi(const vf_pack_desc* descs_device, int n, void* stream) {
    if (!descs_device || n <= 0) return VF_ERR_BAD_ARG;
    hipLaunchKernelGGL(pack_bf16_multi_kernel, dim3(128, (unsigned)n), dim3(256), 0, (hipStream_t)stream, descs_device);
    return vf_last_status();
}

int vf_gemm_bf16(const vf_igemm_args* args, void* stream) {
    if (!args) return VF_ERR_BAD_ARG;
    const vf_igemm_args& a = *args;
    if (!a.x || !a.w_packed || !a.out || a.M <= 0 || a.Cin <= 0 || a.Cout <= 0) return VF_ERR_BAD_ARG;
    if (a.gn_part) return VF_ERR_UNSUPPORTED;
    if (a.mode != VF_MODE_GEMM || a.pro_mean) return VF_ERR_UNSUPPORTED;
    if (a.Cin % CK != 0) return VF_ERR_UNSUPPORTED;
    if (a.epilogue == VF_EPI_GELU_BWD && !(a.reserved0 & 2)) return VF_ERR_UNSUPPORTED;
    if ((a.epilogue == VF_EPI_GELU_DUAL) != (a.out_aux != nullptr)) return VF_ERR_BAD_ARG;
    if (a.lda < a.Cin || (a.lda & 3) || a.ldc < a.Cout || (a.res && a.ldr < a.Cout)) return VF_ERR_BAD_ARG;
    if (a.epilogue == VF_EPI_GELU_DUAL) {
        if (!(a.reserved0 & 1) || a.batch > 1 || a.Cin % (2 * CK) != 0) return VF_ERR_UNSUPPORTED;
        const int rc = vf_gemm_bf16_g256_launch(a, (hipStream_t)stream);
        return rc;
    }
    if (a.drop_rate != 0.f) {
        if (!(a.reserved0 & 1) || (a.reserved0 & 2) || a.batch > 1 || a.Cin % (2 * CK) != 0) return VF_ERR_UNSUPPORTED;
        return vf_gemm_bf16_g256_launch(a, (hipStream_t)stream);
    }
    const size_t smem = (size_t)2 * (A_BYTES + B_BYTES);
    static unsigned long long attr_devs = 0;
    if (vf_attr_needed(&attr_devs)) {
        hipError_t e = hipFuncSetAttribute(reinterpret_cast<const void*>(gemm_bf16_kernel),
                                           hipFuncAttributeMaxDynamicSharedMemorySize, (int)smem);
        if (e != hipSuccess) return (int)e;
        vf_attr_done(&attr_devs);
    }
    const int nb = (a.Cout + BN - 1) / BN, mt = (a.M + BM - 1) / BM;
    const bool a16 = a.reserved0 & 1, o16 = a.reserved0 & 2;
    if (a16 || o16) {
        if (a.Cin % (2 * CK) != 0 || a.batch > 1) return VF_ERR_UNSUPPORTED;
        if ((a16 && (a.lda & 7)) || (o16 && a.res && a.epilogue != VF_EPI_GELU_BWD)) return VF_ERR_BAD_ARG;
        if (a.epilogue == VF_EPI_GELU_BWD && !(o16 && a.res && a.ldr >= a.Cout)) return VF_ERR_BAD_ARG;
        if (a.reserved0 & 4) {
            if (a.epilogue != VF_EPI_GELU_BWD) return VF_ERR_BAD_ARG;
            return vf_gemm_bf16_g256_launch(a, (hipStream_t)stream);
        }
        if (vf_selected(VF_SEL_GEMM_G256)) {
            const int rc = vf_gemm_bf16_g256_launch(a, (hipStream_t)stream);
            if (rc != VF_ERR_UNSUPPORTED) return rc;
        }
        const dim3 g((unsigned)(mt * nb));
        hipStream_t st = (hipStream_t)stream;
        if (a16 && o16) hipLaunchKernelGGL((gemm_bf16_direct_kernel<true, true>), g, dim3(256), (size_t)2 * A_BYTES, st, a);
        else if (a16) hipLaunchKernelGGL((gemm_bf16_direct_kernel<true, false>), g, dim3(256), (size_t)2 * A_BYTES, st, a);
        else hipLaunchKernelGGL((gemm_bf16_direct_kernel<false, true>), g, dim3(256), (size_t)2 * A_BYTES, st, a);
        return vf_last_status();
    }
    if (a.Cin % (2 * CK) == 0 && a.batch <= 1) {
        hipLaunchKernelGGL((gemm_bf16_direct_kernel<false, false>), dim3((unsigned)(mt * nb)), dim3(256), (size_t)2 * A_BYTES, (hipStream_t)stream, a);
        return vf_last_status();
    }
    dim3 grid((unsigned)(mt * nb), 1, (unsigned)(a.batch > 0 ? a.batch : 1));
    hipLaunchKernelGGL(gemm_bf16_kernel, grid, dim3(256), smem, (hipStream_t)stream, a);
    return vf_last_status();
}

}
```

### viewformer_amd/csrc/gemm_bf16_g256.hip

```cpp
#include "vf_common.h"
#include "epilogue.h"
#include "../../include/vf_hip.h"

namespace {

typedef __bf16 bf16x8 __attribute__((ext_vector_type(8)));
typedef __bf16 bf16x2_t __attribute__((ext_vector_type(2)));

constexpr int GM = 256, GN = 256, GK = 64;
constexpr int GA_BYTES = GM * GK * 2;
constexpr int GB_BYTES = GN * GK * 2;
constexpr int GSTAGE = GA_BYTES + GB_BYTES;

__device__ __forceinline__ void bufds16(__amdgpu_buffer_rsrc_t r, void* l, unsigned voff, unsigned soff) {
    __builtin_amdgcn_raw_ptr_buffer_load_lds(r, (__attribute__((address_space(3))) void*)l, 16, voff, soff, 0, 0);
}

template <bool DROP, int IC>
__device__ __forceinline__ void g256_store_f32(const vf_igemm_args& p, const f32x16 (&acc)[IC][2], int m_tile0, int n_tile0, int wrow0,
                                               int wave_n, int half, int l31, bool full, bool gelu) {
    const long long ldc = p.ldc, ldr = p.ldr;
    const bool has_res = p.res != nullptr;
    const bool dual = p.epilogue == VF_EPI_GELU_DUAL;
    const int odd = l31 & 1;
// ... 4 lines not shown
        const int n = n_tile0 + wave_n * 64 + j * 32 + l31;
        const float bias = p.bias ? p.bias[n] : 0.f;
#pragma unroll
        for (int i = 0; i < IC; ++i) {
            int m0 = m_tile0 + wrow0 + i * 32 + 4 * half;
            if constexpr (DROP) asm volatile("" : "+v"(m0) :: "memory");
            const int rows_left = p.M - m0;
            float* o = p.out + (size_t)(rows_left > 0 ? m0 : 0) * ldc + n;
            float v[16];
#pragma unroll
            for (int r = 0; r < 16; ++r) v[r] = acc[i][j][r] + bias;
            if (gelu) {
#pragma unroll
                for (int r = 0; r < 16; ++r) v[r] = vf_gelu_erf_fast(v[r]);
            }
            if constexpr (DROP) {
#pragma unroll
                for (int g = 0; g < 4; ++g) {
                    const uint32_t w = vf_dropout_word(drop_key, (uint32_t)(((m0 + p.drop_row0) >> 2) + 2 * g) * (uint32_t)p.Cout + (uint32_t)n);
#pragma unroll
                    for (int e = 0; e < 4; ++e) v[4 * g + e] = vf_dropout_keep(w, e, drop_thresh) ? v[4 * g + e] * drop_scale : 0.f;
                }
            }
            if (has_res) {
                const float* rs = p.res + (size_t)(rows_left > 0 ? m0 : 0) * ldr + n;
                float rr[16];
#pragma unroll
                for (int r = 0; r < 16; ++r) {
                    const int row = (r & 3) + 8 * (r >> 2);
                    rr[r] = rs[(long long)(full || row < rows_left ? row : 0) * ldr];
                }
#pragma unroll
                for (int r = 0; r < 16; ++r) v[r] += rr[r];
            }
            if (full) {
#pragma unroll
                for (int r = 0; r < 16; ++r) o[(long long)((r & 3) + 8 * (r >> 2)) * ldc] = v[r];
            } else if (rows_left > 0) {
#pragma unroll
                for (int r = 0; r < 16; ++r) {
                    const int row = (r & 3) + 8 * (r >> 2);
                    if (row < rows_left) o[(long long)row * ldc] = v[r];
                }
            }
            if (dual) {
                __builtin_amdgcn_sched_barrier(0);
                __bf16* o16 = reinterpret_cast<__bf16*>(p.out_aux) + (size_t)(rows_left > 0 ? m0 : 0) * ldc + (n - odd);
#pragma unroll
                for (int r = 0; r < 16; ++r) v[r] = vf_gelu_erf_fast(v[r]);
#pragma unroll
                for (int r = 0; r < 16; r += 2) {
                    const float give = odd ? v[r] : v[r + 1];
                    const float got = vf_lane_xor1(give);
                    const int row = ((r + odd) & 3) + 8 * ((r + odd) >> 2);
                    bf16x2_t h;
                    h[0] = (__bf16)(odd ? got : v[r]);
                    h[1] = (__bf16)(odd ? v[r + 1] : got);
                    if (full || row < rows_left) *reinterpret_cast<bf16x2_t*>(o16 + (long long)row * ldc) = h;
                }
            }
            __builtin_amdgcn_sched_barrier(0);
        }
    }
}

template <int EPI, bool FULL, int IC>
__device__ __forceinline__ void g256_store_bf16(const vf_igemm_args& p, const f32x16 (&acc)[IC][2], int m_tile0, int n_tile0, int wrow0,
                                                int wave_n, int half, int l31) {
    __bf16* __restrict__ O = reinterpret_cast<__bf16*>(p.out);
    const int odd = l31 & 1;
#pragma unroll
    for (int j = 0; j < 2; ++j) {
        const int n = n_tile0 + wave_n * 64 + j * 32 + l31;
        const float bias = p.bias ? p.bias[n] : 0.f;
#pragma unroll
        for (int i = 0; i < IC; ++i) {
            const int m0 = m_tile0 + wrow0 + i * 32 + 4 * half;
            float t[16];
            if (EPI == 2 || EPI == 4) {
                const bool u16 = p.reserved0 & 4;
                const unsigned esz = u16 ? 2u : 4u;
                const __amdgpu_buffer_rsrc_t u_rs = __builtin_amdgcn_make_buffer_rsrc(
                    const_cast<unsigned char*>(reinterpret_cast<const unsigned char*>(p.res) + (size_t)m_tile0 * p.ldr * esz), 0,
                    (int)min((long long)0x7fffffff, (long long)(p.M - m_tile0) * p.ldr * esz), 0x00020000);
                float uu[16];
                if (u16) {
                    const unsigned voff = ((unsigned)(m0 - m_tile0) * (unsigned)p.ldr + (unsigned)(n - odd)) * 2u;
                    unsigned w[8];
#pragma unroll
                    for (int r = 0; r < 16; r += 2) {
                        const int row = ((r + odd) & 3) + 8 * ((r + odd) >> 2);
                        w[r >> 1] = __builtin_amdgcn_raw_buffer_load_b32(u_rs, voff + (unsigned)row * (unsigned)p.ldr * 2u, 0, 0);
                    }
#pragma unroll
                    for (int r = 0; r < 16; r += 2) {
                        const unsigned mine = w[r >> 1];
                        const unsigned give = odd ? (mine << 16) : (mine & 0xffff0000u);
                        const unsigned got = vf_lane_xor1(give);
                        uu[r] = __builtin_bit_cast(float, odd ? got : (mine << 16));
                        uu[r + 1] = __builtin_bit_cast(float, odd ? (mine & 0xffff0000u) : got);
                    }
                } else {
                    const unsigned voff = ((unsigned)(m0 - m_tile0) * (unsigned)p.ldr + (unsigned)n) * 4u;
#pragma unroll
                    for (int r = 0; r < 16; ++r) {
                        const unsigned soff = (unsigned)((r & 3) + 8 * (r >> 2)) * (unsigned)p.ldr * 4u;
                        uu[r] = __builtin_bit_cast(float, __builtin_amdgcn_raw_buffer_load_b32(u_rs, voff, soff, 0));
                    }
                }
                __builtin_amdgcn_sched_barrier(0);
#pragma unroll
                for (int q = 0; q < 4; ++q) {
#pragma unroll
                    for (int e = 0; e < 4; ++e)
                        t[4 * q + e] = __fmul_rn(__fadd_rn(acc[i][j][4 * q + e], bias), EPI == 4 ? uu[4 * q + e] : vf_gelu_grad_fast(uu[4 * q + e]));
                    __builtin_amdgcn_sched_barrier(0);
                }
            } else {
#pragma unroll
                for (int r = 0; r < 16; ++r) {
                    t[r] = acc[i][j][r] + bias;
                    if (EPI == 1) t[r] = vf_gelu_erf_fast(t[r]);
                }
            }
            float gq[EPI == 5 ? 16 : 1];
            if (EPI == 5) {
#pragma unroll
                for (int r = 0; r < 16; ++r) { float f, g; vf_gelu_and_grad_fast(t[r], f, g); t[r] = f; gq[r] = g; }
            }
#pragma unroll
            for (int pass = 0; pass < ((EPI == 3 || EPI == 5) ? 2 : 1); ++pass) {
                __bf16* __restrict__ dst = pass == 0 ? O : reinterpret_cast<__bf16*>(p.out_aux);
                if (EPI == 3 && pass == 1) {
                    __builtin_amdgcn_sched_barrier(0);
#pragma unroll
                    for (int r = 0; r < 16; ++r) t[r] = vf_gelu_erf_fast(t[r]);
                }
#pragma unroll
                for (int r = 0; r < 16; r += 2) {
                    const float lo = (EPI == 5 && pass == 0) ? gq[r] : t[r], hi = (EPI == 5 && pass == 0) ? gq[r + 1] : t[r + 1];
                    const float give = odd ? lo : hi;
                    const float got = vf_lane_xor1(give);
                    const int m = m0 + ((r + odd) & 3) + 8 * ((r + odd) >> 2);
                    bf16x2_t v;
                    v[0] = (__bf16)(odd ? got : lo);
                    v[1] = (__bf16)(odd ? hi : got);
                    if (FULL || m < p.M) *reinterpret_cast<bf16x2_t*>(dst + (size_t)m * p.ldc + (n - odd)) = v;
                }
            }
        }
    }
}

template <bool O16, bool DROP, int IC>
__device__ __forceinline__ void g256_tile(const vf_igemm_args& p, unsigned char* smem_b, int m_tile0, int nblk, int tid) {
    constexpr int TROWS = 2 * IC * 32;
    const int lane = tid & 63;
    const int wave = __builtin_amdgcn_readfirstlane(tid >> 6);
    const int wave_m = wave >> 2, wave_n = wave & 3;
    const int half = lane >> 5, l31 = lane & 31;
    const int wrow0 = wave_m * (IC * 32);
    const int n_tile0 = nblk * GN;
    const int nstages = p.Cin / GK;

    const bool a_mover = wave * 32 < TROWS;
    const __amdgpu_buffer_rsrc_t a_rsrc = __builtin_amdgcn_make_buffer_rsrc(const_cast<float*>(p.x), 0, 0x7fffffff, 0x00020000);
    const __amdgpu_buffer_rsrc_t w_rsrc = __builtin_amdgcn_make_buffer_rsrc(const_cast<float*>(p.w_packed), 0, 0x7fffffff, 0x00020000);
    unsigned avoff[4];
#pragma unroll
    for (int q = 0; q < 4; ++q) {
        const int r = wave * 32 + q * 8 + (lane >> 3);
        const int c = (lane & 7) ^ ((r >> 1) & 7);
        int m = m_tile0 + r;
        m = m < p.M ? m : p.M - 1;
        avoff[q] = (unsigned)(((size_t)m * p.lda) * 2 + c * 16);
    }
    const unsigned wvoff = (unsigned)((size_t)nblk * GB_BYTES + wave * 4096 + lane * 16);
    const size_t w_stage_stride = (size_t)(p.Cout / 128) * (GK * 128 * 2);
    auto issue = [&](int s) {
        unsigned char* dst = smem_b + (s & 1) * GSTAGE;
        if (IC == 4 || a_mover) {
#pragma unroll
            for (int q = 0; q < 4; ++q) bufds16(a_rsrc, dst + (wave * 32 + q * 8) * 128, avoff[q], (unsigned)(s * (GK * 2)));
        }
#pragma unroll
        for (int q = 0; q < 4; ++q) bufds16(w_rsrc, dst + GA_BYTES + wave * 4096 + q * 1024, wvoff + q * 1024, (unsigned)((size_t)s * w_stage_stride));
    };

    const unsigned a_row_off = (unsigned)((wrow0 + l31) * 128);
    const unsigned a_swz = (unsigned)((l31 >> 1) & 7);
    unsigned a_off[4];
#pragma unroll
    for (int ks = 0; ks < 4; ++ks) a_off[ks] = a_row_off + ((((unsigned)(ks * 2 + half)) ^ a_swz) << 4);
    const unsigned b_off = (unsigned)(GA_BYTES + (wave_n >> 1) * (GK * 128 * 2) + ((half * 128) + (wave_n & 1) * 64 + l31) * 16);

    f32x16 acc[IC][2];
#pragma unroll
    for (int i = 0; i < IC; ++i)
#pragma unroll
        for (int j = 0; j < 2; ++j)
#pragma unroll
            for (int r = 0; r < 16; ++r) acc[i][j][r] = 0.f;

    issue(0);
    for (int s = 0; s < nstages; ++s) {
        asm volatile("s_waitcnt vmcnt(0) lgkmcnt(0)" ::: "memory");
        __builtin_amdgcn_s_barrier();
        if (s + 1 < nstages) issue(s + 1);
        const unsigned char* buf = smem_b + (s & 1) * GSTAGE;
        bf16x8 a[2][IC], b[2][2];
        auto frags = [&](int ks, bf16x8 (&af)[IC], bf16x8 (&bf)[2]) {
#pragma unroll
            for (int j = 0; j < 2; ++j) bf[j] = *reinterpret_cast<const bf16x8*>(buf + b_off + (ks * 2 * 128 + j * 32) * 16);
#pragma unroll
            for (int i = 0; i < IC; ++i) af[i] = *reinterpret_cast<const bf16x8*>(buf + a_off[ks] + i * (32 * 128));
        };
        frags(0, a[0], b[0]);
#pragma unroll
        for (int ks = 0; ks < 4; ++ks) {
            if (ks < 3) frags(ks + 1, a[(ks + 1) & 1], b[(ks + 1) & 1]);
            __builtin_amdgcn_sched_barrier(0);
#pragma unroll
            for (int i = 0; i < IC; ++i)
#pragma unroll
                for (int j = 0; j < 2; ++j)
                    acc[i][j] = __builtin_amdgcn_mfma_f32_32x32x16_bf16(a[ks & 1][i], b[ks & 1][j], acc[i][j], 0, 0, 0);
            __builtin_amdgcn_sched_barrier(0);
        }
    }

    const bool full = m_tile0 + TROWS <= p.M;
    const bool gelu = p.epilogue == VF_EPI_GELU_ERF;
    if (O16) {
        const bool gbwd = p.epilogue == VF_EPI_GELU_BWD;
        const bool dual16 = p.epilogue == VF_EPI_GELU_DUAL;
        const bool deriv = p.reserved0 & 8;
        if (dual16 && deriv) {
            if (full) g256_store_bf16<5, true, IC>(p, acc, m_tile0, n_tile0, wrow0, wave_n, half, l31);
            else g256_store_bf16<5, false, IC>(p, acc, m_tile0, n_tile0, wrow0, wave_n, half, l31);
        } else if (gbwd && deriv) {
            if (full) g256_store_bf16<4, true, IC>(p, acc, m_tile0, n_tile0, wrow0, wave_n, half, l31);
            else g256_store_bf16<4, false, IC>(p, acc, m_tile0, n_tile0, wrow0, wave_n, half, l31);
        } else if (dual16) {
            if (full) g256_store_bf16<3, true, IC>(p, acc, m_tile0, n_tile0, wrow0, wave_n, half, l31);
            else g256_store_bf16<3, false, IC>(p, acc, m_tile0, n_tile0, wrow0, wave_n, half, l31);
        } else if (full) {
            if (gbwd) g256_store_bf16<2, true, IC>(p, acc, m_tile0, n_tile0, wrow0, wave_n, half, l31);
            else if (gelu) g256_store_bf16<1, true, IC>(p, acc, m_tile0, n_tile0, wrow0, wave_n, half, l31);
            else g256_store_bf16<0, true, IC>(p, acc, m_tile0, n_tile0, wrow0, wave_n, half, l31);
        } else {
            if (gbwd) g256_store_bf16<2, false, IC>(p, acc, m_tile0, n_tile0, wrow0, wave_n, half, l31);
            else if (gelu) g256_store_bf16<1, false, IC>(p, acc, m_tile0, n_tile0, wrow0, wave_n, half, l31);
            else g256_store_bf16<0, false, IC>(p, acc, m_tile0, n_tile0, wrow0, wave_n, half, l31);
        }
    } else {
        g256_store_f32<DROP, IC>(p, acc, m_tile0, n_tile0, wrow0, wave_n, half, l31, full, gelu);
    }
}

__device__ __forceinline__ void g256_panel_order(unsigned lbid, int mt, int nb, int& mtile, int& nblk) {
    constexpr int PANEL = 4;
    const int sn = nb <= PANEL ? nb : nb % PANEL == 0 ? PANEL : nb % 3 == 0 ? 3 : nb % 2 == 0 ? 2 : 1;
    const int per_panel = mt * sn;
    const int panel = (int)(lbid / (unsigned)per_panel);
    const int in_panel = (int)(lbid - (unsigned)panel * per_panel);
    nblk = panel * sn + in_panel % sn;
    mtile = in_panel / sn;
}

template <bool O16, bool DROP = false, bool TAIL = false>
__global__ __launch_bounds__(512, 1) void gemm_bf16_g256_kernel(vf_igemm_args p, int f_rows, int h_rows, int tail_ic) {
    extern __shared__ __attribute__((aligned(16))) unsigned char smem_b[];
    const int tid = threadIdx.x;
    const int nb = p.Cout / GN;
    int mtile, nblk;
    if constexpr (!TAIL) {
        g256_panel_order(vf_xcd_bid(), (p.M + GM - 1) / GM, nb, mtile, nblk);
        g256_tile<O16, DROP, 4>(p, smem_b, mtile * GM, nblk, tid);
    } else {
        const unsigned F = (unsigned)(f_rows * nb), tot = gridDim.x;
        const unsigned x = blockIdx.x & 7u, i = blockIdx.x >> 3;
        const unsigned nF = F / 8u + (x < (F & 7u) ? 1u : 0u);
        const unsigned baseF = x * (F / 8u) + (x < (F & 7u) ? x : (F & 7u));
        if (i < nF) {
            g256_panel_order(baseF + i, f_rows, nb, mtile, nblk);
            g256_tile<O16, DROP, 4>(p, smem_b, mtile * GM, nblk, tid);
            return;
        }
        const unsigned baseT = x * (tot / 8u) + (x < (tot & 7u) ? x : (tot & 7u));
        g256_panel_order(baseT - baseF + (i - nF), h_rows, nb, mtile, nblk);
        const int m_tile0 = f_rows * GM + mtile * (tail_ic * 64);
        if (tail_ic == 3) g256_tile<O16, DROP, 3>(p, smem_b, m_tile0, nblk, tid);
        else g256_tile<O16, DROP, 2>(p, smem_b, m_tile0, nblk, tid);
    }
}

}

struct G256Tail { int f_rows, h_rows, ic; };
static G256Tail g256_tail_policy(int M, int nb) {
    const int mt = (M + GM - 1) / GM;
    const long long ntiles = (long long)mt * nb;
    constexpr int CUS = 256;
    G256Tail none{0, 0, 0};
    if (ntiles <= CUS || !vf_selected(VF_SEL_GEMM_TAIL)) return none;
    const int last = (int)(ntiles % CUS);
    if (last == 0 || last > (CUS * 3) / 4 - 8 || last < 16) return none;
    const int f_rows = (int)((ntiles / CUS) * CUS / nb);
    if (f_rows <= 0 || f_rows >= mt) return none;
    const int rem_blocks = (M - f_rows * GM + 31) / 32;
    for (int ic = 2; ic <= 3; ++ic) {
        const int h_rows = (rem_blocks + 2 * ic - 1) / (2 * ic);
        if ((long long)h_rows * nb <= CUS) return G256Tail{f_rows, h_rows, ic};
    }
    return none;
}

int vf_gemm_bf16_g256_launch(const vf_igemm_args& a, hipStream_t stream) {
    const bool a16 = a.reserved0 & 1, o16 = a.reserved0 & 2;
    if (!a16 || a.batch > 1 || a.Cout % GN != 0 || a.Cin % GK != 0 || a.M < GM || (a.lda & 7)) return VF_ERR_UNSUPPORTED;
    if (o16 && ((a.res && a.epilogue != VF_EPI_GELU_BWD) || (a.ldc & 1))) return VF_ERR_UNSUPPORTED;
    if (a.epilogue == VF_EPI_GELU_BWD && !(o16 && a.res)) return VF_ERR_UNSUPPORTED;
    if (a.epilogue == VF_EPI_GELU_DUAL && (a.res || !a.out_aux || (a.ldc & 1))) return VF_ERR_UNSUPPORTED;
    if ((a.reserved0 & 4) && a.epilogue != VF_EPI_GELU_BWD) return VF_ERR_BAD_ARG;
    if (a.reserved0 & 8) {
        if (a.epilogue == VF_EPI_GELU_BWD ? !(a.reserved0 & 4) : !(a.epilogue == VF_EPI_GELU_DUAL && o16)) return VF_ERR_BAD_ARG;
    }
    if (a.res && a.epilogue == VF_EPI_GELU_ERF) return VF_ERR_UNSUPPORTED;
    if (a.drop_rate != 0.f && (!(a.drop_rate > 0.f && a.drop_rate < 1.f) || o16 || a.epilogue != VF_EPI_NONE || a.drop_row0 < 0 || (a.drop_row0 & 3) ||
                               (((unsigned long long)a.M + (unsigned long long)a.drop_row0 + 3) / 4) * (unsigned long long)a.Cout >= (1ull << 32)))
        return VF_ERR_UNSUPPORTED;
    if ((size_t)a.M * a.lda * 2 >= (1ull << 31) || (size_t)a.Cin * a.Cout * 2 >= (1ull << 31)) return VF_ERR_UNSUPPORTED;
    const int mt = (a.M + GM - 1) / GM, nb = a.Cout / GN;
    const G256Tail t = g256_tail_policy(a.M, nb);
    const dim3 g((unsigned)(t.f_rows ? (t.f_rows + t.h_rows) * nb : mt * nb));
    auto launch = [&](auto kernel, unsigned long long* devs) -> int {
        if (vf_attr_needed(devs)) {
            const hipError_t e = hipFuncSetAttribute(reinterpret_cast<const void*>(kernel), hipFuncAttributeMaxDynamicSharedMemorySize, 2 * GSTAGE);
            if (e != hipSuccess) return (int)e;
            vf_attr_done(devs);
        }
        hipLaunchKernelGGL(kernel, g, dim3(512), (size_t)2 * GSTAGE, stream, a, t.f_rows, t.h_rows, t.ic);
        return vf_last_status();
    };
    static unsigned long long d0 = 0, d1 = 0, d2 = 0, d3 = 0, d4 = 0, d5 = 0;
    const bool drop = a.drop_rate > 0.f;
    if (t.f_rows) {
        if (o16) return launch(gemm_bf16_g256_kernel<true, false, true>, &d3);
        return drop ? launch(gemm_bf16_g256_kernel<false, true, true>, &d5) : launch(gemm_bf16_g256_kernel<false, false, true>, &d4);
    }
    if (o16) return launch(gemm_bf16_g256_kernel<true, false, false>, &d0);
    return drop ? launch(gemm_bf16_g256_kernel<false, true, false>, &d2) : launch(gemm_bf16_g256_kernel<false, false, false>, &d1);
}
```

### viewformer_amd/csrc/igemm_f32.hip

```cpp
#include "vf_common.h"
#include "epilogue.h"
#include "../../include/vf_hip.h"
#include <stdlib.h>

int vf_conv3_halo_try(const vf_igemm_args& a, hipStream_t stream, int* status);

namespace {

constexpr int CK = 32;
constexpr int A_LD = 36;

__host__ __device__ inline int bn_for(int N) { return N > 64 ? 128 : (N > 32 ? 64 : 32); }

struct RowInfo {
    int pix_base;
    int oy, ox;
    int img;
    int valid;
};

template <int WAVES_M, int WAVES_N, int WM_T, int WN_T, int PBN = WAVES_N * WN_T * 32>
__global__ __launch_bounds__(256, 2) void igemm_f32_kernel(vf_igemm_args p) {
    constexpr int BN = WAVES_N * WN_T * 32;
    constexpr int BM = WAVES_M * WM_T * 32;
// ... 110 lines not shown
#pragma unroll
        for (int q = 0; q < AP; ++q) {
            f32x4 v = areg[q];
            if (has_pro) {
#pragma unroll
                for (int e = 0; e < 4; ++e) {
                    float t = (v[e] - pmean[q][e]) * pscale[q][e] + pbeta[e];
                    if (p.pro_swish) t = vf_swish(t);
                    v[e] = aok[q] ? t : 0.f;
                }
            }
            *reinterpret_cast<f32x4*>(a_dst + (a_row0 + 32 * q) * A_LD + a_col4 * 4) = v;
        }
        float* b_dst = Bs + buf * (CK * BN);
#pragma unroll
        for (int q = 0; q < B_F4; ++q)
            *reinterpret_cast<f32x4*>(b_dst + (size_t)(tid + 256 * q) * 4) = breg[q];
    };

    f32x16 acc[WM_T][WN_T];
#pragma unroll
    for (int i = 0; i < WM_T; ++i)
#pragma unroll
        for (int j = 0; j < WN_T; ++j)
#pragma unroll
            for (int r = 0; r < 16; ++r) acc[i][j][r] = 0.f;

    int chunk = 0, tap = 0;
    load_stage(0, 0);
    store_stage(0);
    __syncthreads();

    for (int s = 0; s < nstages; ++s) {
        int nchunk = chunk, ntap = tap + 1;
        if (ntap == taps) { ntap = 0; nchunk = chunk + 1; }
        const bool more = (s + 1) < nstages;
        if (more) load_stage(nchunk, ntap);

        const float* a_src = As + (s & 1) * (BM * A_LD) + (wave_m * WM_T * 32 + l31) * A_LD + half * 4;
        const float* b_src = Bs + (s & 1) * (CK * BN) + (half * BN + wave_n * WN_T * 32 + l31) * 4;
#pragma unroll
        for (int g = 0; g < 4; ++g) {
            f32x4 a[WM_T], b[WN_T];
#pragma unroll
            for (int i = 0; i < WM_T; ++i) a[i] = *reinterpret_cast<const f32x4*>(a_src + i * 32 * A_LD + g * 8);
#pragma unroll
            for (int j = 0; j < WN_T; ++j) b[j] = *reinterpret_cast<const f32x4*>(b_src + (g * 2 * BN + j * 32) * 4);
#pragma unroll
            for (int e = 0; e < 4; ++e)
#pragma unroll
                for (int i = 0; i < WM_T; ++i)
#pragma unroll
                    for (int j = 0; j < WN_T; ++j)
                        acc[i][j] = __builtin_amdgcn_mfma_f32_32x32x2f32(a[i][e], b[j][e], acc[i][j], 0, 0, 0);
        }
        if (more) store_stage((s + 1) & 1);
        __syncthreads();
        chunk = nchunk; tap = ntap;
    }

#pragma unroll
    for (int j = 0; j < WN_T; ++j) {
        const int n = nblk * BN + (wave_n * WN_T + j) * 32 + l31;
        const bool nok = n < p.Cout;
        const float bias = (nok && p.bias) ? p.bias[n] : 0.f;
        const long long ldc = p.ldc, ldr = p.ldr;
        const bool gelu = p.epilogue == VF_EPI_GELU_ERF;
#pragma unroll
        for (int i = 0; i < WM_T; ++i) {
            const int m0 = mtile * BM + (wave_m * WM_T + i) * 32 + 4 * half;
            const int nn = nok ? n : 0;
            float* o = Out + (size_t)(m0 < p.M ? m0 : 0) * ldc + nn;
            const float* rs = Res ? Res + (size_t)(m0 < p.M ? m0 : 0) * ldr + nn : nullptr;
            const int rows_left = nok ? p.M - m0 : 0;
            const bool full = (mtile * BM + BM <= p.M) && (nblk * BN + BN <= p.Cout);
            if (full) {
                auto oo = [&](int r) { return (long long)((r & 3) + 8 * (r >> 2)) * ldc; };
                auto ro = [&](int r) { return (long long)((r & 3) + 8 * (r >> 2)) * ldr; };
                if (gelu) {
                    if (Res) vf_store_tile<1, true>(acc[i][j], bias, o, rs, oo, ro);
                    else vf_store_tile<1, false>(acc[i][j], bias, o, rs, oo, ro);
                } else {
                    if (Res) vf_store_tile<0, true>(acc[i][j], bias, o, rs, oo, ro);
                    else vf_store_tile<0, false>(acc[i][j], bias, o, rs, oo, ro);
                }
            } else if (gelu) {
                if (Res) vf_store_tile_ragged<1, true>(acc[i][j], bias, o, rs, ldc, ldr, rows_left);
                else vf_store_tile_ragged<1, false>(acc[i][j], bias, o, rs, ldc, ldr, rows_left);
            } else {
                if (Res) vf_store_tile_ragged<0, true>(acc[i][j], bias, o, rs, ldc, ldr, rows_left);
                else vf_store_tile_ragged<0, false>(acc[i][j], bias, o, rs, ldc, ldr, rows_left);
            }
        }
    }
}

__global__ void pack_b_kernel(const float* __restrict__ src, float* __restrict__ dst, int K, int N, int taps,
                              long long sk, long long sn, long long st, int BN, int nb, int nchunks,
                              long long src_bstride, long long dst_bstride) {
    const long long total = (long long)nchunks * taps * nb * CK * BN;
    const int bz = blockIdx.y;
    for (long long idx = blockIdx.x * (long long)blockDim.x + threadIdx.x; idx < total;
         idx += (long long)gridDim.x * blockDim.x) {
        const int e = (int)(idx & 3);
        long long t = idx >> 2;
        const int nl = (int)(t % BN); t /= BN;
        const int half = (int)(t & 1);
        const int g = (int)((t >> 1) & 3);
        t >>= 3;
        const int nblk = (int)(t % nb); t /= nb;
        const int tap = (int)(t % taps);
        const int chunk = (int)(t / taps);
        const int k = chunk * CK + g * 8 + half * 4 + e;
        const int n = nblk * BN + nl;
        float v = 0.f;
        if (k < K && n < N) v = src[(size_t)bz * src_bstride + k * sk + n * sn + tap * st];
        dst[(size_t)bz * dst_bstride + idx] = v;
    }
}

template <int WAVES_M, int WAVES_N, int WM_T, int WN_T, int PBN = WAVES_N * WN_T * 32>
int launch_igemm(const vf_igemm_args& a, hipStream_t stream) {
    constexpr int BN = WAVES_N * WN_T * 32;
    constexpr int BM = WAVES_M * WM_T * 32;
    const size_t smem = (size_t)(2 * BM * A_LD + 2 * CK * BN) * sizeof(float);
    auto kern = igemm_f32_kernel<WAVES_M, WAVES_N, WM_T, WN_T, PBN>;
    static unsigned long long attr_devs = 0;
    if (vf_attr_needed(&attr_devs)) {
        hipError_t e = hipFuncSetAttribute(reinterpret_cast<const void*>(kern),
                                           hipFuncAttributeMaxDynamicSharedMemorySize, (int)smem);
        if (e != hipSuccess) return (int)e;
        vf_attr_done(&attr_devs);
    }
    const int nb = (a.Cout + BN - 1) / BN;
    const int mt = (a.M + BM - 1) / BM;
    dim3 grid((unsigned)(mt * nb), 1, (unsigned)(a.batch > 0 ? a.batch : 1));
    hipLaunchKernelGGL(kern, grid, dim3(256), smem, stream, a);
    return vf_last_status();
}

}

int vf_pack_b_impl(const float* src, float* dst, int K, int N, int taps, long long sk, long long sn, long long st,
                   int BN, int batch, long long src_bstride, hipStream_t stream) {
    const int nb = (N + BN - 1) / BN;
    const int nchunks = (K + CK - 1) / CK;
    const long long total = (long long)nchunks * taps * nb * CK * BN;
    const int blocks = (int)((total + 255) / 256 > 4096 ? 4096 : (total + 255) / 256);
    hipLaunchKernelGGL(pack_b_kernel, dim3(blocks, batch), dim3(256), 0, stream, src, dst, K, N, taps, sk, sn, st, BN,
                       nb, nchunks, src_bstride, total);
    return vf_last_status();
}

extern "C" {

int vf_abi_version(void) { return 20; }

static int g_vf_select[VF_SEL_COUNT] = {1, 1, 1, 1, 1, 0};
int vf_select(int which, int value) {
    if (which < 0 || which >= VF_SEL_COUNT || (value != 0 && value != 1)) return VF_ERR_BAD_ARG;
    return __atomic_exchange_n(&g_vf_select[which], value, __ATOMIC_RELAXED);
}
int vf_selected(int which) {
    if (which < 0 || which >= VF_SEL_COUNT) return VF_ERR_BAD_ARG;
    return __atomic_load_n(&g_vf_select[which], __ATOMIC_RELAXED);
}
size_t vf_sizeof_igemm_args(void) { return sizeof(vf_igemm_args); }
size_t vf_sizeof_pack_desc(void) { return sizeof(vf_pack_desc); }
const char* vf_build_arch(void) { return "gfx950"; }

size_t vf_igemm_packed_floats(int K, int N, int taps) {
    if (K <= 0 || N <= 0 || taps <= 0) return 0;
    const int BN = bn_for(N);
    const size_t nb = (size_t)(N + BN - 1) / BN;
    const size_t nchunks = (size_t)(K + CK - 1) / CK;
    return nchunks * taps * nb * CK * BN;
}

int vf_igemm_pack_f32(const float* src, float* dst, int K, int N, int taps, int64_t sk, int64_t sn, int64_t st,
                      int batch, int64_t src_bstride, void* stream) {
    if (!src || !dst || K <= 0 || N <= 0 || (taps != 1 && taps != 9) || batch < 1) return VF_ERR_BAD_ARG;
    return vf_pack_b_impl(src, dst, K, N, taps, sk, sn, st, bn_for(N), batch, src_bstride, (hipStream_t)stream);
}

int vf_igemm_f32(const vf_igemm_args* args, void* stream) {
    if (!args) return VF_ERR_BAD_ARG;
    const vf_igemm_args& a = *args;
    if (!a.x || !a.w_packed || !a.out || a.M <= 0 || a.Cin <= 0 || a.Cout <= 0) return VF_ERR_BAD_ARG;
    if (a.epilogue != VF_EPI_NONE && a.epilogue != VF_EPI_GELU_ERF) return VF_ERR_UNSUPPORTED;
    if (a.gn_part) return VF_ERR_UNSUPPORTED;
    if (a.drop_rate != 0.f || a.out_aux) return VF_ERR_UNSUPPORTED;
    if (a.Cin % CK != 0) return VF_ERR_UNSUPPORTED;
    if (a.mode < VF_MODE_GEMM || a.mode > VF_MODE_CONV3_UP2) return VF_ERR_BAD_ARG;
    if (a.mode != VF_MODE_GEMM) {
        if (a.Hin <= 0 || a.Win <= 0 || a.Hout <= 0 || a.Wout <= 0) return VF_ERR_BAD_ARG;
        if (a.M % (a.Hout * a.Wout) != 0) return VF_ERR_BAD_ARG;
        if (a.mode == VF_MODE_CONV3_S1 && (a.Hout != a.Hin || a.Wout != a.Win)) return VF_ERR_BAD_ARG;
        if (a.mode == VF_MODE_CONV3_S2PAD && (a.Hout != a.Hin / 2 || a.Wout != a.Win / 2)) return VF_ERR_BAD_ARG;
        if (a.mode == VF_MODE_CONV3_UP2 && (a.Hout != a.Hin * 2 || a.Wout != a.Win * 2)) return VF_ERR_BAD_ARG;
    } else {
        if (a.lda < a.Cin || (a.lda & 3)) return VF_ERR_BAD_ARG;
    }
    if (a.ldc < a.Cout || (a.res && a.ldr < a.Cout)) return VF_ERR_BAD_ARG;
    const bool pro = a.pro_mean || a.pro_scale || a.pro_beta;
    if (pro && !(a.pro_mean && a.pro_scale && a.pro_beta)) return VF_ERR_BAD_ARG;
    if (pro && a.mode == VF_MODE_GEMM && a.pro_rows_per_img <= 0) return VF_ERR_BAD_ARG;
    hipStream_t s = (hipStream_t)stream;
    {
        int st = 0;
        if (vf_conv3_halo_try(a, s, &st) == 0) return st;
    }
    const int BN = bn_for(a.Cout);
    if (BN == 128) {
        const long long tiles128 = (long long)((a.M + 127) / 128) * ((a.Cout + 127) / 128) * (a.batch > 0 ? a.batch : 1);
        if (tiles128 < 384 && a.Cout % 64 == 0) return launch_igemm<2, 2, 1, 1, 128>(a, s);
        return launch_igemm<2, 2, 2, 2>(a, s);
    }
    if (BN == 64) return launch_igemm<4, 1, 1, 2>(a, s);
    return launch_igemm<4, 1, 1, 1>(a, s);
}

}
```

### viewformer_amd/csrc/vf_common.h

```cpp
#pragma once
#include <hip/hip_runtime.h>
#include <stdint.h>

typedef float f32x4 __attribute__((ext_vector_type(4)));
typedef float f32x16 __attribute__((ext_vector_type(16)));

#define VF_OK 0
#define VF_ERR_BAD_ARG (-1)
#define VF_ERR_UNSUPPORTED (-2)

#define VF_WAVE 64

static inline int vf_last_status() {
    hipError_t e = hipGetLastError();
    return e == hipSuccess ? VF_OK : (int)e;
}

static inline bool vf_attr_needed(unsigned long long* mask) {
    int d = 0;
    (void)hipGetDevice(&d);
    return !((__atomic_load_n(mask, __ATOMIC_RELAXED) >> (d & 63)) & 1ull);
}
static inline void vf_attr_done(unsigned long long* mask) {
    int d = 0;
    (void)hipGetDevice(&d);
    __atomic_fetch_or(mask, 1ull << (d & 63), __ATOMIC_RELAXED);
}

__device__ __forceinline__ float vf_swish(float v) {
    return v / (1.0f + expf(-v));
}

__device__ __forceinline__ float vf_swish_1ulp(float v) {
    const float LH = -1.4426950408889634f, LL = -1.9259629911266175e-8f;
    float th = v * LH;
    const float tl = __builtin_fmaf(v, LH, -th) + v * LL;
    th = fminf(th, 126.0f);
    const float e0 = __builtin_amdgcn_exp2f(th);
    const float d = 1.0f + __builtin_fmaf(e0 * tl, 0.6931471805599453f, e0);
    float r = __builtin_amdgcn_rcpf(d);
    r = __builtin_fmaf(__builtin_fmaf(-d, r, 1.0f), r, r);
    return v * r;
}

__device__ __forceinline__ float vf_exp_neg(float d) {
    const float LH = 1.4426950408889634f, LL = 1.9259629911266175e-8f;
    const float th = __fmul_rn(d, LH);
    const float tl = __builtin_fmaf(d, LH, -th) + d * LL;
    const float e0 = __builtin_amdgcn_exp2f(th);
    return __builtin_fmaf(e0 * tl, 0.6931471805599453f, e0);
}

__device__ __forceinline__ float vf_gelu_erf(float v) {
    return 0.5f * v * (1.0f + erff(v * 0.70710678118654752440f));
}

__device__ __forceinline__ float vf_gelu_grad(float x) {
    const float cdf = __fmul_rn(0.5f, __fadd_rn(1.0f, erff(__fmul_rn(x, 0.70710678118654752440f))));
    const float pdf = __fmul_rn(0.39894228040143267794f, expf(__fmul_rn(-0.5f, __fmul_rn(x, x))));
    return __fmaf_rn(x, pdf, cdf);
}

__device__ __forceinline__ float vf_gelu_grad_fast(float x) {
    const float z = __fmul_rn(fabsf(x), 0.70710678118654752440f);
    const float t = __builtin_amdgcn_rcpf(__fmaf_rn(0.3275911f, z, 1.0f));
    float p = __fmaf_rn(1.061405429f, t, -1.453152027f);
    p = __fmaf_rn(p, t, 1.421413741f);
    p = __fmaf_rn(p, t, -0.284496736f);
    p = __fmaf_rn(p, t, 0.254829592f);
    const float e = __builtin_amdgcn_exp2f(__fmul_rn(-1.4426950408889634f, __fmul_rn(z, z)));
    const float erf_abs = __fmaf_rn(-__fmul_rn(p, t), e, 1.0f);
    const float cdf = __fmul_rn(0.5f, __fadd_rn(1.0f, copysignf(erf_abs, x)));
    return __fmaf_rn(x, __fmul_rn(0.39894228040143267794f, e), cdf);
}

__device__ __forceinline__ float vf_gelu_erf_fast(float v) {
    const float z = fabsf(v) * 0.70710678118654752440f;
    float t = __builtin_amdgcn_rcpf(__builtin_fmaf(0.3275911f, z, 1.0f));
    float p = __builtin_fmaf(1.061405429f, t, -1.453152027f);
    p = __builtin_fmaf(p, t, 1.421413741f);
    p = __builtin_fmaf(p, t, -0.284496736f);
    p = __builtin_fmaf(p, t, 0.254829592f);
    const float e = __builtin_amdgcn_exp2f(-1.4426950408889634f * z * z);
    const float erf_abs = __builtin_fmaf(-p * t, e, 1.0f);
    return 0.5f * v * (1.0f + copysignf(erf_abs, v));
}

__device__ __forceinline__ void vf_gelu_and_grad_fast(float v, float& f, float& g) {
    const float z = fabsf(v) * 0.70710678118654752440f;
    float t = __builtin_amdgcn_rcpf(__builtin_fmaf(0.3275911f, z, 1.0f));
    float p = __builtin_fmaf(1.061405429f, t, -1.453152027f);
    p = __builtin_fmaf(p, t, 1.421413741f);
    p = __builtin_fmaf(p, t, -0.284496736f);
    p = __builtin_fmaf(p, t, 0.254829592f);
    const float e = __builtin_amdgcn_exp2f(-1.4426950408889634f * z * z);
    const float erf_abs = __builtin_fmaf(-p * t, e, 1.0f);
    const float one_plus = 1.0f + copysignf(erf_abs, v);
    f = 0.5f * v * one_plus;
    g = __builtin_fmaf(v, 0.39894228040143267794f * e, 0.5f * one_plus);
}

__device__ __forceinline__ int vf_lane_xor1(int v) { return __builtin_amdgcn_mov_dpp(v, 0xB1, 0xF, 0xF, true); }
__device__ __forceinline__ unsigned vf_lane_xor1(unsigned v) { return (unsigned)__builtin_amdgcn_mov_dpp((int)v, 0xB1, 0xF, 0xF, true); }
__device__ __forceinline__ float vf_lane_xor1(float v) { return __int_as_float(__builtin_amdgcn_mov_dpp(__float_as_int(v), 0xB1, 0xF, 0xF, true)); }

__device__ __forceinline__ float vf_wave_sum(float v) {
#pragma unroll
    for (int o = 32; o > 0; o >>= 1) v += __shfl_xor(v, o, 64);
    return v;
}

__device__ __forceinline__ float vf_wave_sum_dpp(float v) {
#define VF_DPP_ADD(ctrl, rmask) v += __int_as_float(__builtin_amdgcn_update_dpp(0, __float_as_int(v), ctrl, rmask, 0xF, false))
    VF_DPP_ADD(0x111, 0xF);
    VF_DPP_ADD(0x112, 0xF);
    VF_DPP_ADD(0x114, 0xF);
    VF_DPP_ADD(0x118, 0xF);
    VF_DPP_ADD(0x142, 0xA);
    VF_DPP_ADD(0x143, 0xC);
#undef VF_DPP_ADD
    return __int_as_float(__builtin_amdgcn_readlane(__float_as_int(v), 63));
}

__device__ __forceinline__ float vf_wave_max(float v) {
#pragma unroll
    for (int o = 32; o > 0; o >>= 1) v = fmaxf(v, __shfl_xor(v, o, 64));
    return v;
}

__device__ __forceinline__ void vf_block_max_atomic(float m, unsigned* out) {
    __shared__ float vf_bm_red[4];
    m = vf_wave_max(m);
    if ((threadIdx.x & 63) == 0) vf_bm_red[threadIdx.x >> 6] = m;
    __syncthreads();
    if (threadIdx.x == 0) atomicMax(out, __float_as_uint(fmaxf(fmaxf(vf_bm_red[0], vf_bm_red[1]), fmaxf(vf_bm_red[2], vf_bm_red[3]))));
}

__host__ __device__ __forceinline__ uint32_t vf_dropout_hash(uint32_t seed, uint32_t site, uint64_t idx) {
    uint32_t h = seed ^ (site * 0x9E3779B9u);
    h ^= (uint32_t)idx;
    h *= 0x85EBCA6Bu;
    h ^= h >> 13;
    h += (uint32_t)(idx >> 32) * 0xC2B2AE35u + 0x27D4EB2Fu;
    h ^= h >> 16;
    h *= 0x165667B1u;
    h ^= h >> 15;
    h *= 0xD3A2646Cu;
    h ^= h >> 16;
    return h;
}
__host__ __device__ __forceinline__ uint32_t vf_lowbias32(uint32_t x) {
    x ^= x >> 16;
    x *= 0x7FEB352Du;
    x ^= x >> 15;
    x *= 0x846CA68Bu;
    x ^= x >> 16;
    return x;
}
__host__ __device__ __forceinline__ uint32_t vf_dropout_key(uint32_t seed, uint32_t site, uint32_t hi) { return vf_dropout_hash(seed, site, (uint64_t)hi); }
__host__ __device__ __forceinline__ uint32_t vf_dropout_word(uint32_t key, uint32_t lo) { return vf_lowbias32(lo ^ key); }
__host__ __device__ __forceinline__ bool vf_dropout_keep(uint32_t word, int j, uint32_t thresh) {
    const uint32_t s = 8u * ((uint32_t)j & 3u);
    return ((word << s) | (word >> ((32u - s) & 31u))) >= thresh;
}
__device__ __forceinline__ uint32_t vf_dropout_rotr(int j) { return (32u - 8u * ((uint32_t)j & 3u)) & 31u; }
__device__ __forceinline__ bool vf_dropout_keep_rotr(uint32_t word, uint32_t rr, uint32_t thresh) { return __builtin_amdgcn_alignbit(word, word, rr) >= thresh; }
__host__ __device__ __forceinline__ bool vf_dropout_keep_elem(uint32_t seed, uint32_t site, uint64_t m, uint32_t n, uint32_t N, uint32_t thresh) {
    const uint64_t g = (m >> 2) * (uint64_t)N + n;
    return vf_dropout_keep(vf_dropout_word(vf_dropout_key(seed, site, (uint32_t)(g >> 32)), (uint32_t)g), (int)(m & 3), thresh);
}
__host__ __device__ __forceinline__ uint32_t vf_dropout_thresh(float rate) { return (uint32_t)((double)rate * 4294967296.0); }

__device__ __forceinline__ unsigned vf_xcd_bid() {
    const unsigned n = gridDim.x, b = blockIdx.x;
    const unsigned q = n >> 3, r = n & 7u, x = b & 7u, i = b >> 3;
    return x * q + (x < r ? x : r) + i;
}

__device__ __forceinline__ float vf_vq_sq4(const f32x4 v) {
    return __builtin_fmaf(v[0], v[0], v[1] * v[1]) + __builtin_fmaf(v[2], v[2], v[3] * v[3]);
// ... 107 lines not shown
```

### viewformer_amd/ops.py

```python
import ctypes
import os

import torch

from . import _lib
from ._lib import VfIgemmArgs, check

MODE_GEMM, MODE_CONV3_S1, MODE_CONV3_S2PAD, MODE_CONV3_UP2 = 0, 1, 2, 3
EPI_NONE, EPI_GELU, EPI_GELU_BWD, EPI_GELU_DUAL = 0, 1, 2, 3


def _stream():
    return ctypes.c_void_p(torch.cuda.current_stream().cuda_stream)


def _p(t):
    if t is None:
        return None
    return ctypes.c_void_p(t.data_ptr())


def _chk(t, dtype=torch.float32, name='tensor'):
    if not t.is_cuda:
        raise _lib.VfError(f'{name} must live on the GPU (no CPU fallback for the hot path)')
# ... 153 lines not shown


ARM_KW = {'f32': {}, 'x6': dict(x6=True), 'x3h': dict(x3h=True), 'bf16': dict(bf16=True)}


def conv3_arm(mode, Cin, Cout, Hout, Wout, activations=False, res=False):
    if not res and conv3_small_cout_supported(mode, Cin, Cout, Hout, Wout):
        return 'small'
    if conv3_x6_supported(mode, Cin, Cout, Hout, Wout):
        return 'x3h' if activations else 'x6'
    return 'f32'


def pack_conv3(arm, w_oihw):
    return {'f32': pack_conv_oihw, 'x6': pack_conv3_x6, 'x3h': pack_conv3_x3h, 'bf16': pack_conv3_bf16}[arm](w_oihw)


def pack_dense_nk_arm(arm, w, n_rows=None):
    return {'f32': pack_dense_nk, 'x6': pack_dense_nk_x6, 'x3h': pack_dense_nk_x3h, 'bf16': pack_dense_nk_bf16}[arm](w, n_rows)


def pack_dense(arm, w, transposed=False, n_rows=None):
    fn = globals()['pack_dense_' + ('nk' if transposed else 'kn') + ('' if arm == 'f32' else '_' + arm)]
    return fn(w) if n_rows is None else fn(w, n_rows=n_rows)


def gemm_bf16_splitk(x, w_packed, M, Cin, Cout, dst, splits, lda=None, accumulate=True):
    lib = _lib.load()
    ks = Cin // splits
    if splits < 1 or ks * splits != Cin or ks % 64:
        raise _lib.VfError(f'gemm_bf16_splitk: Cin = {Cin} does not split into {splits} ranges of whole 64-deep chunks')
    nb = (Cout + 127) // 128
    slabs = torch.empty((splits, M, Cout), dtype=torch.float32, device=x.device)
    igemm(x, w_packed, M, ks, Cout, slabs, lda=Cin if lda is None else lda, bf16=True, batch=splits, stride_x=ks,
          stride_w=(ks // 64) * nb * 64 * 128, stride_out=M * Cout)
    check(lib.vf_sum_slabs_f32(_p(slabs), splits, M * Cout, M * Cout, _p(_f32(dst)), 1 if accumulate else 0, _stream()),
          'vf_sum_slabs_f32')
    return dst


TN_TARGET_WORKGROUPS = 256
TN_TARGET_WORKGROUPS_BESIDE = 192


def gemm_tn_bf16_supported(x, M, K, N):
    return x.dtype == torch.bfloat16 and gemm_tn_bf16_shape_ok(M, K, N)


def gemm_tn_bf16_shape_ok(M, K, N):
    return K % 256 == 0 and N % 256 == 0 and M % 64 == 0 and M * K * 2 < 2 ** 31


def gemm_g256_shape_ok(M, K, N):
    return N % 256 == 0 and K % 64 == 0 and M >= 256 and M * K * 2 < 2 ** 31 and K * N * 2 < 2 ** 31


def gemm_drop_supported(M, K, N, row0=0):
    return gemm_g256_shape_ok(M, K, N) and row0 % 4 == 0 and ((M + row0 + 3) // 4) * N < 2 ** 32


def gemm_tn_bf16(x16, dy, M, K, N, dw, db=None, accumulate=True, beside_another_gemm=False):
    lib = _lib.load()
    _chk(x16, torch.bfloat16, 'x16')
    tiles = (K // 256) * (N // 256)
    target = TN_TARGET_WORKGROUPS_BESIDE if beside_another_gemm else TN_TARGET_WORKGROUPS
    splits = max(1, min(M // 64, target // tiles if tiles <= target else 1))
    rec = K * N + (N if db is not None else 0)
    ws = torch.empty((splits, rec), dtype=torch.float32, device=dy.device)
    y16 = dy.dtype == torch.bfloat16
    check(lib.vf_gemm_tn_bf16(_p(x16), x16.stride(0), _p(dy if y16 else _f32(dy)), 1 if y16 else 0, dy.stride(0), M, K, N, splits, _p(ws),
                              ws.data_ptr() + K * N * 4 if db is not None else None, rec, _stream()), 'vf_gemm_tn_bf16')
    acc = 1 if accumulate else 0
    _f32(dw)
    if db is not None and _f32(db).data_ptr() == dw.data_ptr() + K * N * 4 and dw.is_contiguous():
        check(lib.vf_sum_slabs_f32(_p(ws), splits, rec, rec, _p(dw), acc, _stream()), 'vf_sum_slabs_f32')
    else:
        check(lib.vf_sum_slabs_f32(_p(ws), splits, rec, K * N, _p(dw), acc, _stream()), 'vf_sum_slabs_f32')
        if db is not None:
            check(lib.vf_sum_slabs_f32(ws.data_ptr() + K * N * 4, splits, rec, N, _p(db), acc, _stream()), 'vf_sum_slabs_f32')
    return dw


def igemm(x, w_packed, M, Cin, Cout, out, bias=None, res=None, mode=MODE_GEMM, epilogue=EPI_NONE,
          pro=None, pro_swish=False, pro_rows_per_img=0, Hin=0, Win=0, Hout=0, Wout=0,
          lda=None, ldc=None, ldr=None, batch=1, stride_x=0, stride_w=0, stride_out=0, stride_res=0, bf16=False, x6=False, gn_part=None, split_k=0,
          x3h=False, a16=False, o16=False, out_aux=None, res16=False, drop=None, gelu_grad=False):
    lib = _lib.load()
    if not 0 <= M < 2 ** 31 or max(Cin, Cout, Hin, Win, Hout, Wout, batch) >= 2 ** 31:
        raise _lib.VfError(f'igemm: M = {M} rows do not fit the int32 fields of vf_igemm_args — split the launch '
                           '(VQGAN(max_images_per_call=...))')
    a = VfIgemmArgs()
    a.x = x.data_ptr()
    a.w_packed = w_packed.data_ptr()
    a.bias = bias.data_ptr() if bias is not None else None
    a.res = res.data_ptr() if res is not None else None
    a.out = out.data_ptr()
    if out_aux is not None:
        _chk(out_aux, torch.bfloat16, 'out_aux')
        if out_aux.shape != out.shape or not (out_aux.is_contiguous() or out_aux.stride() == out.stride()):
            raise _lib.VfError('out_aux must have the shape and row stride of out')
        a.out_aux = out_aux.data_ptr()
    if pro is not None:
        mean_c, scale_c, beta = pro
        a.pro_mean, a.pro_scale, a.pro_beta = mean_c.data_ptr(), scale_c.data_ptr(), beta.data_ptr()
    a.pro_swish = 1 if pro_swish else 0
    a.pro_rows_per_img = pro_rows_per_img
    a.mode, a.epilogue = mode, epilogue
    a.M, a.Cin, a.Cout = M, Cin, Cout
    a.Hin, a.Win, a.Hout, a.Wout = Hin, Win, Hout, Wout
    a.lda = Cin if lda is None else lda
    a.ldc = Cout if ldc is None else ldc
    a.ldr = (Cout if ldr is None else ldr)
    a.batch = batch
    a.stride_x, a.stride_w, a.stride_out, a.stride_res = stride_x, stride_w, stride_out, stride_res
    a.reserved0 = split_k
    if gn_part is not None:
        a.gn_part = _f32(gn_part).data_ptr()
        a.gn_slots = gn_part.shape[1]
    conv16 = False
    if a16 or o16:
        if not bf16 or mode not in (MODE_GEMM, MODE_CONV3_S1, MODE_CONV3_UP2):
            raise _lib.VfError('a16 / o16 need bf16=True and a GEMM or 3x3 stride-1 / upsample convolution')
        _chk(x, torch.bfloat16 if a16 else torch.float32, 'x')
        _chk(out, torch.bfloat16 if o16 else torch.float32, 'out')
        a.reserved0 = (1 if a16 else 0) | (2 if o16 else 0)
        conv16 = mode != MODE_GEMM
        if conv16:
            if a16 and not o16:
                raise _lib.VfError('the bf16 convolution takes bf16 activations in only together with bf16 out')
            if res is not None:
                _chk(res, torch.bfloat16 if o16 else torch.float32, 'res')
    if drop is not None and drop[0]:
        if not (bf16 and a16 and not o16 and mode == MODE_GEMM and epilogue == EPI_NONE):
            raise _lib.VfError('drop needs the bf16 GEMM with bf16 x, fp32 out and no epilogue function')
        a.drop_rate, a.drop_seed, a.drop_site = float(drop[0]), int(drop[1]) & 0xFFFFFFFF, int(drop[2])
        a.drop_row0 = int(drop[3]) if len(drop) > 3 else 0
    if res16:
        if not (a16 and o16 and epilogue == EPI_GELU_BWD and res is not None):
            raise _lib.VfError('res16 is the bf16 pre-activation of EPI_GELU_BWD (bf16 in, bf16 out)')
        _chk(res, torch.bfloat16, 'res')
        a.reserved0 |= 4
    if gelu_grad:
        if not ((epilogue == EPI_GELU_DUAL and a16 and o16) or (epilogue == EPI_GELU_BWD and res16)):
            raise _lib.VfError('gelu_grad: EPI_GELU_DUAL with bf16 in / out, or EPI_GELU_BWD with res16')
        a.reserved0 |= 8
    for t in ((None if a16 else x), (None if o16 else out), bias, (None if (res16 or conv16) else res)):
        if t is not None:
            _f32(t)
    if x3h:
        _chk(w_packed, torch.float16, 'w_packed')
        if mode == MODE_GEMM:
            check(lib.vf_gemm_x3h(ctypes.byref(a), _stream()), 'vf_gemm_x3h')
        else:
            check(lib.vf_conv3_halo_x3h(ctypes.byref(a), _stream()), 'vf_conv3_halo_x3h')
        return out
    if x6:
        _chk(w_packed, torch.bfloat16, 'w_packed')
        if mode == MODE_GEMM:
            check(lib.vf_gemm_x6(ctypes.byref(a), _stream()), 'vf_gemm_x6')
        else:
            check(lib.vf_conv3_halo_x6(ctypes.byref(a), _stream()), 'vf_conv3_halo_x6')
        return out
    if bf16:
        _chk(w_packed, torch.bfloat16, 'w_packed')
        if mode == MODE_GEMM:
            check(lib.vf_gemm_bf16(ctypes.byref(a), _stream()), 'vf_gemm_bf16')
        else:
            check(lib.vf_conv3_halo_bf16(ctypes.byref(a), _stream()), 'vf_conv3_halo_bf16')
        return out
    _f32(w_packed)
    check(lib.vf_igemm_f32(ctypes.byref(a), _stream()), 'vf_igemm_f32')
    return out


def conv3_small_cout_supported(mode, Cin, Cout, H, W):
    return mode == MODE_CONV3_S1 and 1 <= Cout <= 4 and Cin % 32 == 0 and Cin // 32 * 4608 <= 96 * 1024 and H % 8 == 0 and W % 32 == 0


def conv3_small_cout(x, w_oihw, bias, n_img, H, W, Cin, Cout, pro=None, pro_swish=True, out=None):
    lib = _lib.load()
    if out is None:
        out = torch.empty((n_img * H * W, Cout), dtype=torch.float32, device=x.device)
    pm, ps, pb = (None, None, None) if pro is None else pro
    x16 = x.dtype == torch.bfloat16
    check(lib.vf_conv3_small_cout_f32(_p(x if x16 else _f32(x)), _p(_f32(w_oihw)), _p(_f32(bias)) if bias is not None else None,
                                      _p(pm) if pm is not None else None, _p(ps) if ps is not None else None,
                                      _p(pb) if pb is not None else None, 1 if pro_swish else 0, _p(out), n_img, H, W, Cin, Cout,
                                      1 if x16 else 0, _stream()), 'vf_conv3_small_cout_f32')
    return out


def pack_conv_in_x3h(w_oihw):
    lib = _lib.load()
    w = _f32(w_oihw).contiguous()
    out = torch.empty(int(lib.vf_conv_in_x3h_packed_elems(w.shape[0])), dtype=torch.float16, device=w.device)
    check(lib.vf_conv_in_x3h_pack(_p(w), _p(out), w.shape[0], _stream()), 'vf_conv_in_x3h_pack')
    return out


def conv_in_x3h_supported(H, W, Cout):
    return H % 8 == 0 and W % 16 == 0 and Cout % 128 == 0


def conv_in(img, w_oihw, bias, n_img, H, W, Cout, out=None, wp3h=None, gn_part=None):
    lib = _lib.load()
    if out is None:
        out = torch.empty((n_img, H, W, Cout), dtype=torch.float32, device=img.device)
    if img.dtype == torch.uint8:
        u8, f32 = _p(_chk(img, torch.uint8)), None
    else:
        u8, f32 = None, _p(_f32(img))
    if wp3h is not None:
        _chk(wp3h, torch.float16, 'wp3h')
        check(lib.vf_conv_in_x3h(u8, f32, _p(wp3h), _p(bias), _p(out), _p(gn_part) if gn_part is not None else None,
                                 gn_part.shape[1] if gn_part is not None else 0, n_img, H, W, Cout, _stream()), 'vf_conv_in_x3h')
        return out
    if gn_part is not None:
        raise _lib.VfError('conv_in: fused GroupNorm statistics need the x3h form (wp3h)')
    check(lib.vf_conv_in_u8_f32(u8, f32, _p(_f32(w_oihw)), _p(bias), _p(out), n_img, H, W, Cout, _stream()),
          'vf_conv_in_u8_f32')
    return out


def groupnorm_stats(x, gamma, n_img, HW, C, groups=32, eps=1e-6):
    lib = _lib.load()
    mean_c = torch.empty((n_img, C), dtype=torch.float32, device=x.device)
    scale_c = torch.empty((n_img, C), dtype=torch.float32, device=x.device)
    ws = torch.empty(int(lib.vf_groupnorm_workspace_bytes(n_img, HW, C)), dtype=torch.uint8, device=x.device)
    check(lib.vf_groupnorm_stats_f32(_p(_f32(x)), _p(_f32(gamma)), n_img, HW, C, groups, eps, _p(mean_c), _p(scale_c),
                                     _p(ws), _stream()), 'vf_groupnorm_stats_f32')
    return mean_c, scale_c


def halo_gn_slots(Hout, Wout):
    return int(_lib.load().vf_conv3_halo_gn_slots(Hout, Wout))


def new_gn_part(n_img, Hout, Wout, device):
    return torch.empty((n_img, halo_gn_slots(Hout, Wout), 32, 2), dtype=torch.float32, device=device)


def groupnorm_finalize(part, gamma, n_img, HW, C, groups=32, eps=1e-6):
    lib = _lib.load()
    mean_c = torch.empty((n_img, C), dtype=torch.float32, device=part.device)
    scale_c = torch.empty((n_img, C), dtype=torch.float32, device=part.device)
    check(lib.vf_groupnorm_finalize_f32(_p(_f32(part)), _p(_f32(gamma)), n_img, HW, C, groups, part.shape[1], eps,
                                        _p(mean_c), _p(scale_c), _stream()), 'vf_groupnorm_finalize_f32')
    return mean_c, scale_c


def groupnorm_apply(x, mean_c, scale_c, beta, n_img, HW, C, swish, out=None):
    lib = _lib.load()
    if out is None:
        out = torch.empty_like(x)
    check(lib.vf_groupnorm_apply_f32(_p(_f32(x)), _p(mean_c), _p(scale_c), _p(_f32(beta)), _p(out), n_img, HW, C,
                                     1 if swish else 0, _stream()), 'vf_groupnorm_apply_f32')
    return out


def vq_pack_codebook(E):
    lib = _lib.load()
    E = _f32(E).contiguous()
    D, Kc = E.shape
    out = torch.empty(int(lib.vf_vq_packed_floats(D, Kc)), dtype=torch.float32, device=E.device)
    check(lib.vf_vq_pack_codebook_f32(_p(E), _p(out), D, Kc, _stream()), 'vf_vq_pack_codebook_f32')
    e_sq = torch.empty(Kc, dtype=torch.float32, device=E.device)
    check(lib.vf_colsumsq_f32(_p(E), _p(e_sq), D, Kc, _stream()), 'vf_colsumsq_f32')
    return out, e_sq


def vq_argmin(z_rows, E_packed, e_sq, D, Kc):
    lib = _lib.load()
    z_rows = _f32(z_rows)
    M = z_rows.numel() // D
    idx = torch.empty(M, dtype=torch.int64, device=z_rows.device)
    check(lib.vf_vq_argmin_f32(_p(z_rows), _p(E_packed), _p(e_sq), M, D, Kc, _p(idx), _stream()), 'vf_vq_argmin_f32')
    return idx


def vq_filter_supported(D, Kc):
    return int(_lib.load().vf_vq_filter_packed_bytes(D, Kc)) > 0


def vq_filter_pack(E):
    lib = _lib.load()
    E = _f32(E).contiguous()
    D, Kc = E.shape
    n = int(lib.vf_vq_filter_packed_bytes(D, Kc))
    if n == 0:
        raise _lib.VfError(f'vq_filter_pack: unsupported codebook shape D={D}, Kc={Kc} (need D == 256, Kc % 32 == 0, Kc <= 1024)')
    out = torch.empty(n, dtype=torch.uint8, device=E.device)
    check(lib.vf_vq_filter_pack(_p(E), _p(out), D, Kc, _stream()), 'vf_vq_filter_pack')
    return out


def vq_argmin_filtered(z_rows, blob, D, Kc, stats=None):
    lib = _lib.load()
    z_rows = _f32(z_rows)
    M = z_rows.numel() // D
    idx = torch.empty(M, dtype=torch.int64, device=z_rows.device)
    check(lib.vf_vq_argmin_filtered_f32(_p(z_rows), _p(_chk(blob, torch.uint8, 'blob')), M, D, Kc, _p(idx),
                                        _p(_chk(stats, torch.int32, 'stats')) if stats is not None else None, _stream()),
          'vf_vq_argmin_filtered_f32')
    return idx


def codebook_gather(E, idx, D, Kc):
    lib = _lib.load()
    idx = _chk(idx, torch.int64, 'codes').contiguous()
    M = idx.numel()
    out = torch.empty((M, D), dtype=torch.float32, device=idx.device)
    check(lib.vf_codebook_gather_f32(_p(_f32(E)), _p(idx), _p(out), M, D, Kc, _stream()), 'vf_codebook_gather_f32')
    return out


def attn_blockcausal(q, k, v, out, B, H, T, L, ldq, ldk, ldv, ldo, scale=1.0, skip_masked=True, twin_view=-1, bf16=False, x6=False,
                     fp8=False):
    lib = _lib.load()
    if fp8:
# ... 467 lines not shown
```

Measured before the change: 1146.

## Add 64-row GEMM tiles and split-K paths for small-M latency-bound launches

Adds a 64-row-tile bf16 GEMM path, on by default, that kicks in when the existing tiling would launch fewer blocks than there are CUs. Two split-K variants are added but default off: one for GEMM with a separate reduce kernel, and one for the paired 8x8 halo conv. Both write partial sums to a workspace that ops.py allocates. The goal is better CU occupancy during the small-batch autoregressive transformer and decoder steps. The cost is extra workspace traffic and an extra reduce launch when split-K is enabled, plus a possible tile-efficiency loss from the smaller tiles.

```diff
diff --git a/include/vf_hip.h b/include/vf_hip.h
--- a/include/vf_hip.h
+++ b/include/vf_hip.h
@@ -27,6 +27,9 @@
        VF_SEL_COUNT = 6 };
 int vf_select(int which, int value);
 int vf_selected(int which);
+enum { VF_LAT_GEMM_ROWS64 = 0, VF_LAT_GEMM_SPLITK = 1, VF_LAT_CONV_SPLITK = 2, VF_LAT_COUNT = 3 };
+int vf_latency_select(int which, int value);
+int vf_latency_selected(int which);
 
 enum { VF_MODE_GEMM = 0, VF_MODE_CONV3_S1 = 1, VF_MODE_CONV3_S2PAD = 2, VF_MODE_CONV3_UP2 = 3 };
 enum { VF_EPI_NONE = 0, VF_EPI_GELU_ERF = 1,
@@ -195,6 +198,8 @@
 } vf_pack_desc;
 int vf_gemm_bf16_pack_multi(const vf_pack_desc* descs_device, int n, void* stream);
 int vf_gemm_bf16(const vf_igemm_args* args , void* stream);
+size_t vf_gemm_bf16_workspace_bytes(const vf_igemm_args* args );
+int vf_gemm_bf16_ws(const vf_igemm_args* args , void* workspace, size_t workspace_bytes, void* stream);
 size_t vf_conv3_bf16_packed_elems(int Cin, int Cout);
 int vf_conv3_bf16_pack(const float* w_oihw, void* dst, int Cin, int Cout, void* stream);
 int vf_conv3_halo_bf16(const vf_igemm_args* args , void* stream);
@@ -206,6 +211,8 @@
 size_t vf_conv3_x3h_packed_elems(int Cin, int Cout);
 int vf_conv3_x3h_pack(const float* w_oihw, void* dst, int Cin, int Cout, void* stream);
 int vf_conv3_halo_x3h(const vf_igemm_args* args , void* stream);
+size_t vf_conv3_halo_x3h_workspace_bytes(const vf_igemm_args* args );
+int vf_conv3_halo_x3h_ws(const vf_igemm_args* args , void* workspace, size_t workspace_bytes, void* stream);
 size_t vf_gemm_x3h_packed_elems(int K, int N);
 int vf_gemm_x3h_pack(const float* src, void* dst, int K, int N, int64_t sk, int64_t sn, void* stream);
 int vf_gemm_x3h(const vf_igemm_args* args , void* stream);
diff --git a/viewformer_amd/_lib.py b/viewformer_amd/_lib.py
--- a/viewformer_amd/_lib.py
+++ b/viewformer_amd/_lib.py
@@ -24,6 +24,8 @@
 SEL_ATTN_DMA, SEL_GEMM_G256, SEL_LN_BWD_TWO_ROWS, SEL_ATTN_Q32 = 0, 1, 2, 3
 SEL_CONV_X3H_K32 = 4
 SEL_GEMM_TAIL = 5
+LAT_GEMM_ROWS64, LAT_GEMM_SPLITK, LAT_CONV_SPLITK = 0, 1, 2
+_ENV_LATENCY = {'VF_LAT_GEMM_ROWS64': LAT_GEMM_ROWS64, 'VF_LAT_GEMM_SPLITK': LAT_GEMM_SPLITK, 'VF_LAT_CONV_SPLITK': LAT_CONV_SPLITK}
 _ENV_SELECT = {'VF_ATTN_DMA': SEL_ATTN_DMA, 'VF_GEMM_G256': SEL_GEMM_G256, 'VF_LN_BWD_TWO_ROWS': SEL_LN_BWD_TWO_ROWS, 'VF_ATTN_Q32': SEL_ATTN_Q32,
                'VF_CONV_X3H_K32': SEL_CONV_X3H_K32, 'VF_GEMM_TAIL': SEL_GEMM_TAIL}
 
@@ -39,6 +41,8 @@
     'vf_build_flag_name': (c_char_p, [c_int]),
     'vf_select': (c_int, [c_int, c_int]),
     'vf_selected': (c_int, [c_int]),
+    'vf_latency_select': (c_int, [c_int, c_int]),
+    'vf_latency_selected': (c_int, [c_int]),
     'vf_igemm_packed_floats': (c_size_t, [c_int, c_int, c_int]),
     'vf_igemm_pack_f32': (c_int, [P, P, c_int, c_int, c_int, c_int64, c_int64, c_int64, c_int, c_int64, P]),
     'vf_igemm_f32': (c_int, [POINTER(VfIgemmArgs), P]),
@@ -139,6 +143,8 @@
     'vf_gemm_bf16_pack': (c_int, [P, P, c_int, c_int, c_int64, c_int64, c_int, c_int64, P]),
     'vf_gemm_bf16_pack_multi': (c_int, [P, c_int, P]),
     'vf_gemm_bf16': (c_int, [POINTER(VfIgemmArgs), P]),
+    'vf_gemm_bf16_workspace_bytes': (c_size_t, [POINTER(VfIgemmArgs)]),
+    'vf_gemm_bf16_ws': (c_int, [POINTER(VfIgemmArgs), P, c_size_t, P]),
     'vf_conv3_bf16_packed_elems': (c_size_t, [c_int, c_int]),
     'vf_conv3_bf16_pack': (c_int, [P, P, c_int, c_int, P]),
     'vf_conv3_halo_bf16': (c_int, [POINTER(VfIgemmArgs), P]),
@@ -148,6 +154,8 @@
     'vf_conv3_x3h_packed_elems': (c_size_t, [c_int, c_int]),
     'vf_conv3_x3h_pack': (c_int, [P, P, c_int, c_int, P]),
     'vf_conv3_halo_x3h': (c_int, [POINTER(VfIgemmArgs), P]),
+    'vf_conv3_halo_x3h_workspace_bytes': (c_size_t, [POINTER(VfIgemmArgs)]),
+    'vf_conv3_halo_x3h_ws': (c_int, [POINTER(VfIgemmArgs), P, c_size_t, P]),
     'vf_gemm_x3h_packed_elems': (c_size_t, [c_int, c_int]),
     'vf_gemm_x3h_pack': (c_int, [P, P, c_int, c_int, c_int64, c_int64, P]),
     'vf_gemm_x3h': (c_int, [POINTER(VfIgemmArgs), P]),
@@ -242,6 +250,9 @@
     for env, which in _ENV_SELECT.items():
         if os.environ.get(env) in ('0', '1'):
             lib.vf_select(which, int(os.environ[env]))
+    for env, which in _ENV_LATENCY.items():
+        if os.environ.get(env) in ('0', '1'):
+            lib.vf_latency_select(which, int(os.environ[env]))
     _lib = lib
     return lib
 
@@ -250,6 +261,13 @@
     prev = load().vf_select(int(which), 1 if value else 0)
     if prev < 0:
         raise VfError(f'vf_select({which}, {value}): bad argument')
+    return prev
+
+
+def latency_select(which, value):
+    prev = load().vf_latency_select(int(which), 1 if value else 0)
+    if prev < 0:
+        raise VfError(f'vf_latency_select({which}, {value}): bad argument')
     return prev
 
 
diff --git a/viewformer_amd/csrc/conv3_halo_x3h.hip b/viewformer_amd/csrc/conv3_halo_x3h.hip
--- a/viewformer_amd/csrc/conv3_halo_x3h.hip
+++ b/viewformer_amd/csrc/conv3_halo_x3h.hip
@@ -34,8 +34,8 @@
     l = (_Float16)((x - (float)h) * 2048.f);
 }
 
-template <bool UP2, bool PRO, bool SWISH, bool PAIR = false>
-__global__ __launch_bounds__(256, 2) void conv3_halo_x3h_kernel(vf_igemm_args p) {
+template <bool UP2, bool PRO, bool SWISH, bool PAIR = false, bool SPLIT = false>
+__global__ __launch_bounds__(256, 2) void conv3_halo_x3h_kernel(vf_igemm_args p, float* __restrict__ ws, int split_chunks) {
     using G = Geo<UP2, PAIR>;
     extern __shared__ __attribute__((aligned(16))) unsigned char smem_h[];
 
@@ -49,6 +49,7 @@
     const int nb = p.Cout / BN;
     const int tilesX = p.Wout / TW, tilesY = p.Hout / TH;
     int bid = (int)vf_xcd_bid();
+    const int tile_id = bid;
     const int nblk = bid % nb; bid /= nb;
     int tx = 0, ty = 0, img;
     if (PAIR) { img = bid * 2; }
@@ -61,8 +62,8 @@
     const int sx0 = UP2 ? (x0 / 2 - 1) : (x0 - 1);
 
     const float* __restrict__ X = p.x + (size_t)img * p.Hin * p.Win * p.Cin;
-    const int nchunks = p.Cin / CK;
-    const int last_stage = nchunks * 9 - 1;
+    const int chunk0 = SPLIT ? (int)blockIdx.y * split_chunks : 0;
+    const int nchunks = SPLIT ? split_chunks : p.Cin / CK;
 
     const int c4 = tid & 7;
     int s_off[G::SLOTS];
@@ -88,6 +89,7 @@
     f32x4 pmean, pscale, pbeta, pmean1, pscale1;
     const __amdgpu_buffer_rsrc_t x_rs = __builtin_amdgcn_make_buffer_rsrc(const_cast<float*>(X), 0, 0x7fffffff, 0x00020000);
     auto patch_load = [&](int chunk) {
+        chunk += chunk0;
 #pragma unroll
         for (int q = 0; q < G::SLOTS; ++q)
             preg[q] = __builtin_bit_cast(f32x4, __builtin_amdgcn_raw_buffer_load_b128(x_rs, (unsigned)s_off[q] * 4u, (unsigned)(chunk * CK * 4), 0));
@@ -141,7 +143,7 @@
     const int last_g = nchunks * 18 - 1;
     const __amdgpu_buffer_rsrc_t w_rs = __builtin_amdgcn_make_buffer_rsrc(const_cast<unsigned char*>(Wb), 0, 0x7fffffff, 0x00020000);
     auto b_load = [&](f16x8 (&dst)[2][NJ], int g) {
-        g = min(g, last_g);
+        g = min(g, last_g) + chunk0 * 18;
         const unsigned soff = (unsigned)((size_t)(g >> 1) * tap_stride + (g & 1) * KS_BYTES);
 #pragma unroll
         for (int pl = 0; pl < 2; ++pl)
@@ -207,6 +209,16 @@
         __syncthreads();
     }
 
+    if constexpr (SPLIT) {
+        float* dst = ws + ((size_t)blockIdx.y * gridDim.x + tile_id) * (MI * NJ * 16 * 256) + tid;
+#pragma unroll
+        for (int i = 0; i < MI; ++i)
+#pragma unroll
+            for (int j = 0; j < NJ; ++j)
+#pragma unroll
+                for (int r = 0; r < 16; ++r) dst[((i * NJ + j) * 16 + r) * 256] = __builtin_fmaf(accx[i][j][r], 4.8828125e-4f, acc[i][j][r]);
+        return;
+    }
     const float inv_s = *reinterpret_cast<const float*>(reinterpret_cast<const unsigned char*>(p.w_packed) + (size_t)nchunks * 9 * nb * TAP_BYTES);
 #pragma unroll
     for (int i = 0; i < MI; ++i)
@@ -217,6 +229,44 @@
     vf_halo_epilogue_t<PAIR, MI, NJ>(p, acc, img, img1, y0, x0, PAIR ? 0 : (ty * tilesX + tx) * 2, nblk, wave_m, wave_n, half, l31);
 }
 
+template <bool PAIR>
+__global__ __launch_bounds__(64) void conv3_x3h_split_reduce_kernel(vf_igemm_args p, const float* __restrict__ ws, int slices) {
+    constexpr int MI = 2, NJ = 1;
+    const int lane = threadIdx.x;
+    const int sub = blockIdx.x & 7;
+    const int wave = sub & 3, wave_m = sub >> 2;
+    const int half = lane >> 5, l31 = lane & 31;
+    const int nb = p.Cout / BN;
+    const int tilesX = p.Wout / TW, tilesY = p.Hout / TH;
+    const int tile_id = (int)(blockIdx.x >> 3);
+    int bid = tile_id;
+    const int nblk = bid % nb; bid /= nb;
+    int tx = 0, ty = 0, img;
+    if (PAIR) { img = bid * 2; }
+    else { tx = bid % tilesX; bid /= tilesX; ty = bid % tilesY; img = bid / tilesY; }
+    const int n_img_total = p.M / (p.Hout * p.Wout);
+    const int img1 = PAIR ? min(img + 1, n_img_total - 1) : img;
+    const float inv_s = *reinterpret_cast<const float*>(reinterpret_cast<const unsigned char*>(p.w_packed) + (size_t)(p.Cin / CK) * 9 * nb * TAP_BYTES);
+    f32x16 acc[MI][NJ];
+    const float* src = ws + (size_t)tile_id * (4 * 16 * 256) + (wave_m * 2 * 16) * 256 + wave * 64 + lane;
+    const size_t slice_stride = (size_t)(gridDim.x >> 3) * (4 * 16 * 256);
+#pragma unroll
+    for (int i = 0; i < MI; ++i)
+#pragma unroll
+        for (int r = 0; r < 16; ++r) acc[i][0][r] = src[(i * 16 + r) * 256];
+    for (int s = 1; s < slices; ++s) {
+        const float* sp = src + s * slice_stride;
+#pragma unroll
+        for (int i = 0; i < MI; ++i)
+#pragma unroll
+            for (int r = 0; r < 16; ++r) acc[i][0][r] = __fadd_rn(acc[i][0][r], sp[(i * 16 + r) * 256]);
+    }
+#pragma unroll
+    for (int i = 0; i < MI; ++i)
+#pragma unroll
+        for (int r = 0; r < 16; ++r) acc[i][0][r] = __fmul_rn(acc[i][0][r], inv_s);
+    vf_halo_epilogue_t<PAIR, MI, NJ>(p, acc, img, img1, ty * TH, tx * TW, PAIR ? 0 : (ty * tilesX + tx) * 2, nblk, wave_m, wave, half, l31);
+}
 
 constexpr int S2_PH = 2 * TH + 1, S2_PW = 2 * TW + 1;
 constexpr int S2_NPIX = S2_PH * S2_PW;
@@ -666,7 +716,36 @@
     const int n_img = a.M / (a.Hout * a.Wout);
     const long long blocks = PAIR ? (long long)((n_img + 1) / 2) * (a.Cout / BN)
                                   : (long long)n_img * (a.Hout / TH) * (a.Wout / TW) * (a.Cout / BN);
-    hipLaunchKernelGGL((conv3_halo_x3h_kernel<UP2, PRO, SWISH, PAIR>), dim3((unsigned)blocks), dim3(256), smem, stream, a);
+    hipLaunchKernelGGL((conv3_halo_x3h_kernel<UP2, PRO, SWISH, PAIR>), dim3((unsigned)blocks), dim3(256), smem, stream, a, (float*)nullptr, 0);
+    return vf_last_status();
+}
+
+constexpr size_t SPLIT_TILE_BYTES = (size_t)4 * 16 * 256 * sizeof(float);
+static inline long long halo_blocks(const vf_igemm_args& a, bool pair) {
+    const int n_img = a.M / (a.Hout * a.Wout);
+    return pair ? (long long)((n_img + 1) / 2) * (a.Cout / BN) : (long long)n_img * (a.Hout / TH) * (a.Wout / TW) * (a.Cout / BN);
+}
+static int halo_split_slices(const vf_igemm_args& a, bool pair, size_t ws_bytes, bool unlimited) {
+    if (!vf_latency_selected(VF_LAT_CONV_SPLITK) || a.mode != VF_MODE_CONV3_S1 || !pair) return 0;
+    const int cus = vf_device_cus();
+    const long long blocks = halo_blocks(a, pair);
+    const int nchunks = a.Cin / CK;
+    if (cus <= 0 || blocks <= 0 || blocks >= cus) return 0;
+    int S = 1;
+    while (blocks * S < cus && S * 2 <= nchunks && nchunks % (S * 2) == 0) S *= 2;
+    if (!unlimited)
+        while (S > 1 && (size_t)S * blocks * SPLIT_TILE_BYTES > ws_bytes) S >>= 1;
+    return S > 1 ? S : 0;
+}
+
+template <bool PRO, bool SWISH, bool PAIR>
+int launch_halo_split(const vf_igemm_args& a, float* ws, int S, hipStream_t stream) {
+    using G = Geo<false, PAIR>;
+    const unsigned blocks = (unsigned)halo_blocks(a, PAIR);
+    hipLaunchKernelGGL((conv3_halo_x3h_kernel<false, PRO, SWISH, PAIR, true>), dim3(blocks, (unsigned)S), dim3(256), (size_t)2 * G::BUF, stream, a, ws,
+                       (a.Cin / CK) / S);
+    if (const int rc = vf_last_status()) return rc;
+    hipLaunchKernelGGL(conv3_x3h_split_reduce_kernel<PAIR>, dim3(blocks * 8), dim3(64), 0, stream, a, (const float*)ws, S);
     return vf_last_status();
 }
 
@@ -689,7 +768,15 @@
 }
 
 template <bool UP2, bool PAIR>
-int dispatch_pro(const vf_igemm_args& a, hipStream_t s) {
+int dispatch_pro(const vf_igemm_args& a, hipStream_t s, void* ws, size_t ws_bytes) {
+    if constexpr (PAIR) {
+        if (ws && !(reinterpret_cast<uintptr_t>(ws) & 15)) {
+            if (const int S = halo_split_slices(a, PAIR, ws_bytes, false)) {
+                if (!a.pro_mean) return launch_halo_split<false, false, PAIR>(a, (float*)ws, S, s);
+                return a.pro_swish ? launch_halo_split<true, true, PAIR>(a, (float*)ws, S, s) : launch_halo_split<true, false, PAIR>(a, (float*)ws, S, s);
+            }
+        }
+    }
     if (!UP2 && !PAIR && (a.Cin / CK) % 2 == 0 && (!a.gn_part || a.Cout / 32 <= 16) && vf_x3h16_lds_bytes(a.pro_mean ? a.Cin : 0) <= 80 * 1024 &&
         vf_selected(VF_SEL_CONV_X3H_K32)) {
         if (!a.pro_mean) return launch_halo16<false, false>(a, s);
@@ -723,7 +810,18 @@
     return vf_last_status();
 }
 
-int vf_conv3_halo_x3h(const vf_igemm_args* args, void* stream) {
+size_t vf_conv3_halo_x3h_workspace_bytes(const vf_igemm_args* args) {
+    if (!args || args->mode != VF_MODE_CONV3_S1 || args->M <= 0 || args->Hout <= 0 || args->Wout <= 0 || args->Cin <= 0 || args->Cout <= 0) return 0;
+    const vf_igemm_args& a = *args;
+    const bool pair = a.Hout == 8 && a.Wout == 8;
+    if (a.Cout % BN != 0 || a.Cin % CK != 0 || (!pair && (a.Hout % TH != 0 || a.Wout % TW != 0)) || a.M % (a.Hout * a.Wout) != 0) return 0;
+    const int S = halo_split_slices(a, pair, 0, true);
+    return S ? (size_t)S * halo_blocks(a, pair) * SPLIT_TILE_BYTES : 0;
+}
+
+int vf_conv3_halo_x3h(const vf_igemm_args* args, void* stream) { return vf_conv3_halo_x3h_ws(args, nullptr, 0, stream); }
+
+int vf_conv3_halo_x3h_ws(const vf_igemm_args* args, void* workspace, size_t workspace_bytes, void* stream) {
     if (!args) return VF_ERR_BAD_ARG;
     const vf_igemm_args& a = *args;
     if (!a.x || !a.w_packed || !a.out || a.M <= 0) return VF_ERR_BAD_ARG;
@@ -755,8 +853,8 @@
     if ((long long)a.Hin * a.Win * a.Cin >= (1ll << 31)) return VF_ERR_UNSUPPORTED;
     if (int st = vf_halo_gn_check(a)) return st;
     hipStream_t s = (hipStream_t)stream;
-    if (pair) return dispatch_pro<false, true>(a, s);
-    return (a.mode == VF_MODE_CONV3_UP2) ? dispatch_pro<true, false>(a, s) : dispatch_pro<false, false>(a, s);
-}
-
-}
+    if (pair) return dispatch_pro<false, true>(a, s, workspace, workspace_bytes);
+    return (a.mode == VF_MODE_CONV3_UP2) ? dispatch_pro<true, false>(a, s, nullptr, 0) : dispatch_pro<false, false>(a, s, nullptr, 0);
+}
+
+}
diff --git a/viewformer_amd/csrc/gemm_bf16.hip b/viewformer_amd/csrc/gemm_bf16.hip
--- a/viewformer_amd/csrc/gemm_bf16.hip
+++ b/viewformer_amd/csrc/gemm_bf16.hip
@@ -389,6 +389,8 @@
 }
 
 int vf_gemm_bf16_g256_launch(const vf_igemm_args& a, hipStream_t stream);
+int vf_gemm_bf16_g64_launch(const vf_igemm_args& a, void* ws, size_t ws_bytes, hipStream_t stream);
+size_t vf_gemm_bf16_g64_workspace_bytes(const vf_igemm_args& a);
 
 extern "C" {
 
@@ -414,7 +416,14 @@
     return vf_last_status();
 }
 
-int vf_gemm_bf16(const vf_igemm_args* args, void* stream) {
+size_t vf_gemm_bf16_workspace_bytes(const vf_igemm_args* args) {
+    if (!args || !args->x || !args->w_packed || !args->out || args->M <= 0 || args->Cin <= 0 || args->Cout <= 0) return 0;
+    return vf_gemm_bf16_g64_workspace_bytes(*args);
+}
+
+int vf_gemm_bf16(const vf_igemm_args* args, void* stream) { return vf_gemm_bf16_ws(args, nullptr, 0, stream); }
+
+int vf_gemm_bf16_ws(const vf_igemm_args* args, void* workspace, size_t workspace_bytes, void* stream) {
     if (!args) return VF_ERR_BAD_ARG;
     const vf_igemm_args& a = *args;
     if (!a.x || !a.w_packed || !a.out || a.M <= 0 || a.Cin <= 0 || a.Cout <= 0) return VF_ERR_BAD_ARG;
@@ -451,6 +460,7 @@
             if (a.epilogue != VF_EPI_GELU_BWD) return VF_ERR_BAD_ARG;
             return vf_gemm_bf16_g256_launch(a, (hipStream_t)stream);
         }
+        if (const int rc = vf_gemm_bf16_g64_launch(a, workspace, workspace_bytes, (hipStream_t)stream); rc != VF_ERR_UNSUPPORTED) return rc;
         if (vf_selected(VF_SEL_GEMM_G256)) {
             const int rc = vf_gemm_bf16_g256_launch(a, (hipStream_t)stream);
             if (rc != VF_ERR_UNSUPPORTED) return rc;
diff --git a/viewformer_amd/csrc/gemm_bf16_g256.hip b/viewformer_amd/csrc/gemm_bf16_g256.hip
--- a/viewformer_amd/csrc/gemm_bf16_g256.hip
+++ b/viewformer_amd/csrc/gemm_bf16_g256.hip
@@ -180,8 +180,9 @@
     }
 }
 
-template <bool O16, bool DROP, int IC>
-__device__ __forceinline__ void g256_tile(const vf_igemm_args& p, unsigned char* smem_b, int m_tile0, int nblk, int tid) {
+template <bool O16, bool DROP, int IC, bool SPLIT = false>
+__device__ __forceinline__ void g256_tile(const vf_igemm_args& p, unsigned char* smem_b, int m_tile0, int nblk, int tid, int st0_ = 0, int nst_ = 0,
+                                          float* __restrict__ part = nullptr) {
     constexpr int TROWS = 2 * IC * 32;
     const int lane = tid & 63;
     const int wave = __builtin_amdgcn_readfirstlane(tid >> 6);
@@ -189,7 +190,8 @@
     const int half = lane >> 5, l31 = lane & 31;
     const int wrow0 = wave_m * (IC * 32);
     const int n_tile0 = nblk * GN;
-    const int nstages = p.Cin / GK;
+    const int st0 = SPLIT ? st0_ : 0;
+    const int nstages = SPLIT ? nst_ : p.Cin / GK;
 
     const bool a_mover = wave * 32 < TROWS;
     const __amdgpu_buffer_rsrc_t a_rsrc = __builtin_amdgcn_make_buffer_rsrc(const_cast<float*>(p.x), 0, 0x7fffffff, 0x00020000);
@@ -209,10 +211,10 @@
         unsigned char* dst = smem_b + (s & 1) * GSTAGE;
         if (IC == 4 || a_mover) {
 #pragma unroll
-            for (int q = 0; q < 4; ++q) bufds16(a_rsrc, dst + (wave * 32 + q * 8) * 128, avoff[q], (unsigned)(s * (GK * 2)));
-        }
-#pragma unroll
-        for (int q = 0; q < 4; ++q) bufds16(w_rsrc, dst + GA_BYTES + wave * 4096 + q * 1024, wvoff + q * 1024, (unsigned)((size_t)s * w_stage_stride));
+            for (int q = 0; q < 4; ++q) bufds16(a_rsrc, dst + (wave * 32 + q * 8) * 128, avoff[q], (unsigned)((st0 + s) * (GK * 2)));
+        }
+#pragma unroll
+        for (int q = 0; q < 4; ++q) bufds16(w_rsrc, dst + GA_BYTES + wave * 4096 + q * 1024, wvoff + q * 1024, (unsigned)((size_t)(st0 + s) * w_stage_stride));
     };
 
     const unsigned a_row_off = (unsigned)((wrow0 + l31) * 128);
@@ -257,6 +259,22 @@
         }
     }
 
+    if constexpr (SPLIT) {
+#pragma unroll
+        for (int j = 0; j < 2; ++j) {
+            const int n = n_tile0 + wave_n * 64 + j * 32 + l31;
+#pragma unroll
+            for (int i = 0; i < IC; ++i) {
+                const int m0 = m_tile0 + wrow0 + i * 32 + 4 * half;
+#pragma unroll
+                for (int r = 0; r < 16; ++r) {
+                    const int m = m0 + (r & 3) + 8 * (r >> 2);
+                    if (m < p.M) part[(size_t)m * p.Cout + n] = acc[i][j][r];
+                }
+            }
+        }
+        return;
+    }
     const bool full = m_tile0 + TROWS <= p.M;
     const bool gelu = p.epilogue == VF_EPI_GELU_ERF;
     if (O16) {
@@ -323,6 +341,113 @@
     }
 }
 
+template <bool O16, bool SPLIT>
+__global__ __launch_bounds__(512, 1) void gemm_bf16_g64_kernel(vf_igemm_args p, float* __restrict__ ws, int slice_stages) {
+    extern __shared__ __attribute__((aligned(16))) unsigned char smem_b[];
+    int mtile, nblk;
+    g256_panel_order(blockIdx.x, (p.M + 63) / 64, p.Cout / GN, mtile, nblk);
+    if constexpr (SPLIT) {
+        const int sl = blockIdx.y;
+        g256_tile<O16, false, 1, true>(p, smem_b, mtile * 64, nblk, threadIdx.x, sl * slice_stages, slice_stages, ws + (size_t)sl * p.M * p.Cout);
+    } else {
+        g256_tile<O16, false, 1>(p, smem_b, mtile * 64, nblk, threadIdx.x);
+    }
+}
+
+template <bool O16>
+__global__ __launch_bounds__(256) void g64_reduce_kernel(vf_igemm_args p, const float* __restrict__ ws, int slices) {
+    const long long quads = (long long)p.M * (p.Cout / 4);
+    const long long slab = (long long)p.M * p.Cout;
+    const bool gelu = p.epilogue == VF_EPI_GELU_ERF;
+    for (long long i = blockIdx.x * (long long)blockDim.x + threadIdx.x; i < quads; i += (long long)gridDim.x * blockDim.x) {
+        const int m = (int)(i / (p.Cout / 4)), n = (int)(i % (p.Cout / 4)) * 4;
+        f32x4 v = *reinterpret_cast<const f32x4*>(ws + (size_t)m * p.Cout + n);
+        for (int s = 1; s < slices; ++s) {
+            const f32x4 t = *reinterpret_cast<const f32x4*>(ws + s * slab + (size_t)m * p.Cout + n);
+#pragma unroll
+            for (int e = 0; e < 4; ++e) v[e] = __fadd_rn(v[e], t[e]);
+        }
+        if (p.bias) {
+#pragma unroll
+            for (int e = 0; e < 4; ++e) v[e] = __fadd_rn(v[e], p.bias[n + e]);
+        }
+        if (gelu) {
+#pragma unroll
+            for (int e = 0; e < 4; ++e) v[e] = vf_gelu_erf_fast(v[e]);
+        }
+        if (O16) {
+            __bf16* o = reinterpret_cast<__bf16*>(p.out) + (size_t)m * p.ldc + n;
+            bf16x2_t lo, hi;
+            lo[0] = (__bf16)v[0]; lo[1] = (__bf16)v[1]; hi[0] = (__bf16)v[2]; hi[1] = (__bf16)v[3];
+            *reinterpret_cast<bf16x2_t*>(o) = lo;
+            *reinterpret_cast<bf16x2_t*>(o + 2) = hi;
+        } else {
+            if (p.res) {
+#pragma unroll
+                for (int e = 0; e < 4; ++e) v[e] = __fadd_rn(v[e], p.res[(size_t)m * p.ldr + n + e]);
+            }
+#pragma unroll
+            for (int e = 0; e < 4; ++e) p.out[(size_t)m * p.ldc + n + e] = v[e];
+        }
+    }
+}
+
+}
+
+struct G64Plan { int take, slices, slice_stages; };
+static G64Plan g64_plan(const vf_igemm_args& a) {
+    G64Plan none{0, 0, 0};
+    const bool a16 = a.reserved0 & 1, o16 = a.reserved0 & 2;
+    if (!vf_latency_selected(VF_LAT_GEMM_ROWS64)) return none;
+    if ((a.reserved0 & ~3) || !a16 || a.batch > 1 || a.mode != VF_MODE_GEMM || a.M < 1 || a.Cout % GN != 0 || a.Cin % (2 * GK) != 0 || (a.lda & 7)) return none;
+    if (a.epilogue != VF_EPI_NONE && a.epilogue != VF_EPI_GELU_ERF) return none;
+    if (a.drop_rate != 0.f || a.out_aux || a.gn_part || a.pro_mean) return none;
+    if (o16 ? (a.res != nullptr || (a.ldc & 1)) : (a.res && a.epilogue == VF_EPI_GELU_ERF)) return none;
+    if ((size_t)a.M * a.lda * 2 >= (1ull << 31) || (size_t)a.Cin * a.Cout * 2 >= (1ull << 31)) return none;
+    const int cus = vf_device_cus();
+    if (cus <= 0) return none;
+    const int nb = a.Cout / GN;
+    const long long today = (a.M >= GM && vf_selected(VF_SEL_GEMM_G256)) ? (long long)((a.M + GM - 1) / GM) * nb
+                                                                        : (long long)((a.M + 127) / 128) * (a.Cout / 128);
+    const long long tiles = (long long)((a.M + 63) / 64) * nb;
+    if (today >= cus || tiles > cus) return none;
+    constexpr int SLICE = 768;
+    int slices = 1;
+    if (vf_latency_selected(VF_LAT_GEMM_SPLITK) && a.Cin % SLICE == 0 && a.Cin / SLICE >= 2 && tiles * (a.Cin / SLICE) <= cus) slices = a.Cin / SLICE;
+    return G64Plan{1, slices, slices > 1 ? SLICE / GK : a.Cin / GK};
+}
+
+size_t vf_gemm_bf16_g64_workspace_bytes(const vf_igemm_args& a) {
+    const G64Plan pl = g64_plan(a);
+    return pl.take && pl.slices > 1 ? (size_t)pl.slices * a.M * a.Cout * sizeof(float) : 0;
+}
+
+int vf_gemm_bf16_g64_launch(const vf_igemm_args& a, void* ws, size_t ws_bytes, hipStream_t stream) {
+    G64Plan pl = g64_plan(a);
+    if (!pl.take) return VF_ERR_UNSUPPORTED;
+    const bool o16 = a.reserved0 & 2;
+    if (pl.slices > 1 && (!ws || ws_bytes < (size_t)pl.slices * a.M * a.Cout * sizeof(float) || (reinterpret_cast<uintptr_t>(ws) & 15))) {
+        pl.slices = 1;
+        pl.slice_stages = a.Cin / GK;
+    }
+    const dim3 g((unsigned)(((a.M + 63) / 64) * (a.Cout / GN)), (unsigned)pl.slices);
+    auto launch = [&](auto kernel, unsigned long long* devs) -> int {
+        if (vf_attr_needed(devs)) {
+            const hipError_t e = hipFuncSetAttribute(reinterpret_cast<const void*>(kernel), hipFuncAttributeMaxDynamicSharedMemorySize, 2 * GSTAGE);
+            if (e != hipSuccess) return (int)e;
+            vf_attr_done(devs);
+        }
+        hipLaunchKernelGGL(kernel, g, dim3(512), (size_t)2 * GSTAGE, stream, a, reinterpret_cast<float*>(ws), pl.slice_stages);
+        return vf_last_status();
+    };
+    static unsigned long long d0 = 0, d1 = 0, d2 = 0;
+    if (pl.slices == 1) return o16 ? launch(gemm_bf16_g64_kernel<true, false>, &d0) : launch(gemm_bf16_g64_kernel<false, false>, &d1);
+    if (const int rc = launch(gemm_bf16_g64_kernel<false, true>, &d2)) return rc;
+    const long long quads = (long long)a.M * (a.Cout / 4);
+    const unsigned blocks = (unsigned)((quads + 255) / 256 > 1024 ? 1024 : (quads + 255) / 256);
+    if (o16) hipLaunchKernelGGL(g64_reduce_kernel<true>, dim3(blocks), dim3(256), 0, stream, a, reinterpret_cast<const float*>(ws), pl.slices);
+    else hipLaunchKernelGGL(g64_reduce_kernel<false>, dim3(blocks), dim3(256), 0, stream, a, reinterpret_cast<const float*>(ws), pl.slices);
+    return vf_last_status();
 }
 
 struct G256Tail { int f_rows, h_rows, ic; };
diff --git a/viewformer_amd/csrc/igemm_f32.hip b/viewformer_amd/csrc/igemm_f32.hip
--- a/viewformer_amd/csrc/igemm_f32.hip
+++ b/viewformer_amd/csrc/igemm_f32.hip
@@ -286,6 +286,20 @@
     return vf_last_status();
 }
 
+int vf_device_cus() {
+    static int cus[64];
+    int d = 0;
+    if (hipGetDevice(&d) != hipSuccess || d < 0 || d >= 64) { (void)hipGetLastError(); return 0; }
+    int c = __atomic_load_n(&cus[d], __ATOMIC_RELAXED);
+    if (c == 0) {
+        int n = 0;
+        c = (hipDeviceGetAttribute(&n, hipDeviceAttributeMultiprocessorCount, d) == hipSuccess && n > 0) ? n : -1;
+        if (c < 0) (void)hipGetLastError();
+        __atomic_store_n(&cus[d], c, __ATOMIC_RELAXED);
+    }
+    return c > 0 ? c : 0;
+}
+
 extern "C" {
 
 int vf_abi_version(void) { return 20; }
@@ -298,6 +312,15 @@
 int vf_selected(int which) {
     if (which < 0 || which >= VF_SEL_COUNT) return VF_ERR_BAD_ARG;
     return __atomic_load_n(&g_vf_select[which], __ATOMIC_RELAXED);
+}
+static int g_vf_latency[VF_LAT_COUNT] = {1, 0, 0};
+int vf_latency_select(int which, int value) {
+    if (which < 0 || which >= VF_LAT_COUNT || (value != 0 && value != 1)) return VF_ERR_BAD_ARG;
+    return __atomic_exchange_n(&g_vf_latency[which], value, __ATOMIC_RELAXED);
+}
+int vf_latency_selected(int which) {
+    if (which < 0 || which >= VF_LAT_COUNT) return VF_ERR_BAD_ARG;
+    return __atomic_load_n(&g_vf_latency[which], __ATOMIC_RELAXED);
 }
 size_t vf_sizeof_igemm_args(void) { return sizeof(vf_igemm_args); }
 size_t vf_sizeof_pack_desc(void) { return sizeof(vf_pack_desc); }
diff --git a/viewformer_amd/csrc/vf_common.h b/viewformer_amd/csrc/vf_common.h
--- a/viewformer_amd/csrc/vf_common.h
+++ b/viewformer_amd/csrc/vf_common.h
@@ -26,6 +26,8 @@
     (void)hipGetDevice(&d);
     __atomic_fetch_or(mask, 1ull << (d & 63), __ATOMIC_RELAXED);
 }
+
+int vf_device_cus();
 
 __device__ __forceinline__ float vf_swish(float v) {
     return v / (1.0f + expf(-v));
diff --git a/viewformer_amd/ops.py b/viewformer_amd/ops.py
--- a/viewformer_amd/ops.py
+++ b/viewformer_amd/ops.py
@@ -329,7 +329,12 @@
         if mode == MODE_GEMM:
             check(lib.vf_gemm_x3h(ctypes.byref(a), _stream()), 'vf_gemm_x3h')
         else:
-            check(lib.vf_conv3_halo_x3h(ctypes.byref(a), _stream()), 'vf_conv3_halo_x3h')
+            nws = int(lib.vf_conv3_halo_x3h_workspace_bytes(ctypes.byref(a)))
+            if nws:
+                ws = torch.empty(nws, dtype=torch.uint8, device=out.device)
+                check(lib.vf_conv3_halo_x3h_ws(ctypes.byref(a), _p(ws), nws, _stream()), 'vf_conv3_halo_x3h_ws')
+            else:
+                check(lib.vf_conv3_halo_x3h(ctypes.byref(a), _stream()), 'vf_conv3_halo_x3h')
         return out
     if x6:
         _chk(w_packed, torch.bfloat16, 'w_packed')
@@ -341,7 +346,12 @@
     if bf16:
         _chk(w_packed, torch.bfloat16, 'w_packed')
         if mode == MODE_GEMM:
-            check(lib.vf_gemm_bf16(ctypes.byref(a), _stream()), 'vf_gemm_bf16')
+            nws = int(lib.vf_gemm_bf16_workspace_bytes(ctypes.byref(a)))
+            if nws:
+                ws = torch.empty(nws, dtype=torch.uint8, device=out.device)
+                check(lib.vf_gemm_bf16_ws(ctypes.byref(a), _p(ws), nws, _stream()), 'vf_gemm_bf16_ws')
+            else:
+                check(lib.vf_gemm_bf16(ctypes.byref(a), _stream()), 'vf_gemm_bf16')
         else:
             check(lib.vf_conv3_halo_bf16(ctypes.byref(a), _stream()), 'vf_conv3_halo_bf16')
         return out
```

Result: no change. 1147, median of 3 (+0.1%).
